# kan-bayashi/espnet

Hardware: AMD Instinct MI355X
Metric: frames/sec, 12L Conformer hybrid CTC/attention training step (B=32 T=1000 d=256 per GPU) (higher is better)
Workload: dtype f32; 1 GPU; BASELINE configs[1]: 12L Conformer enc d=256 h=4 ff=2048 k=31 macaron+cnn rel_pos, 6L Transformer dec, V=5000, fbank B=32 T=1000 L=100, mtlalpha 0.3, lsm 0.1; global_batch=32, frames=1000, parallelism=dp1, optimizer=adam+noam, clip 5.0, launch=hipGraph, wgrad_side_stream=False, optimizer_steps_done=113

## Files before the change

### espnet_amd/csrc/convmod.hip

```cpp
#include <stdlib.h>
#include "common.h"
#include "../../include/espnet_amd.h"

namespace {

constexpr int KMAX = 32;

__device__ __forceinline__ void chan_merge(float& n, float& mean, float& m2, float nb, float mb, float m2b);

template <int NWV, int MODE>
__global__ __launch_bounds__(NWV * 64) void dwconv_lds_kernel(const float* __restrict__ x, const float* __restrict__ w,
                                                              const float* __restrict__ bias, float* __restrict__ y,
                                                              int B, int T, int C, int K, int pad, int flip,
                                                              const float* __restrict__ aglu, int y_bf16,
                                                              float* __restrict__ bn_part) {
  constexpr int TB = NWV * 8;
  constexpr int NR = (TB + KMAX - 1 + NWV - 1) / NWV;
  constexpr int NWL = (64 * KMAX + NWV * 64 - 1) / (NWV * 64);
  __shared__ float xs[(TB + KMAX - 1) * 64];
  __shared__ float wl[64 * KMAX];
  const int lane = threadIdx.x & 63, wave = threadIdx.x >> 6;
  const int c0 = blockIdx.x * 64;
  const int c = min(c0 + lane, C - 1);
  const int nblk = (T + TB - 1) / TB;
// ... 691 lines not shown
  if (gy > total) gy = total;
  if (gy < 1) gy = 1;
  const long tpb = (total + gy - 1) / gy;
  gy = (total + tpb - 1) / tpb;
  hipLaunchKernelGGL(dwconv_bwd_w_kernel, dim3(gx, (unsigned)gy), dim3(WNWV * 64), 0, (hipStream_t)stream, dy, a, dw, db, B,
                     T, C, K, (K - 1) / 2, (int)tpb, 1);
  EAMD_LAUNCH_CHECK();
  return EAMD_OK;
}

static bool bn_shape_ok(int C) { return C >= 4 && C <= 1024 && C % 4 == 0; }
int eamd_bn_nslab(int64_t M, int C) {
  if (!bn_shape_ok(C) || M <= 0) return 0;
  const BnGeom g = bn_geom(C);
  return (int)((M + g.slab_rows - 1) / g.slab_rows);
}

static int bn_stats_impl(const float* x, float* workspace, float* mean, float* rstd, float* running_mean,
                         float* running_var, int64_t* num_batches_tracked, int64_t M, int C, float eps, float momentum, int T,
                         const int32_t* bound, void* stream) {
  if (!x || !workspace || !mean || !rstd || M <= 0 || C <= 0) return EAMD_EINVAL;
  if (bound && (T <= 0 || M % T != 0)) return EAMD_EINVAL;
  if (!bn_shape_ok(C)) return EAMD_EUNSUPPORTED;
  if ((uintptr_t)x & 15) return EAMD_EINVAL;
  hipStream_t s = (hipStream_t)stream;
  const int nslab = eamd_bn_nslab(M, C);
  hipLaunchKernelGGL(bn_partial_kernel, dim3(nslab), dim3(256), 0, s, x, workspace, (long)M, C, T, (const int*)bound);
  EAMD_LAUNCH_CHECK();
  hipLaunchKernelGGL(bn_finalize_kernel, dim3((C + BN_CPB - 1) / BN_CPB), dim3(1024), 0, s, workspace, nslab, C, eps, momentum, mean, rstd,
                     running_mean, running_var, (long long*)num_batches_tracked);
  EAMD_LAUNCH_CHECK();
  return EAMD_OK;
}
int eamd_bn_stats(const float* x, float* workspace, float* mean, float* rstd, float* running_mean,
                  float* running_var, int64_t* num_batches_tracked, int64_t M, int C, float eps, float momentum, void* stream) {
  return bn_stats_impl(x, workspace, mean, rstd, running_mean, running_var, num_batches_tracked, M, C, eps, momentum, 1, nullptr, stream);
}
int eamd_bn_stats_bounded(const float* x, float* workspace, float* mean, float* rstd, float* running_mean,
                          float* running_var, int64_t* num_batches_tracked, int64_t M, int C, float eps, float momentum, int T,
                          const int32_t* bound, void* stream) {
  if (!bound) return EAMD_EINVAL;
  return bn_stats_impl(x, workspace, mean, rstd, running_mean, running_var, num_batches_tracked, M, C, eps, momentum, T, bound, stream);
}

int eamd_bn_finalize(const float* part, int nslab, float* mean, float* rstd, float* running_mean, float* running_var,
                     int64_t* num_batches_tracked, int C, float eps, float momentum, void* stream) {
  if (!part || !mean || !rstd || nslab <= 0 || C <= 0) return EAMD_EINVAL;
  hipLaunchKernelGGL(bn_finalize_kernel, dim3((C + BN_CPB - 1) / BN_CPB), dim3(1024), 0, (hipStream_t)stream, part, nslab, C, eps,
                     momentum, mean, rstd, running_mean, running_var, (long long*)num_batches_tracked);
  EAMD_LAUNCH_CHECK();
  return EAMD_OK;
}

int eamd_bn_apply(const float* x, const float* mean, const float* rstd, const float* gamma, const float* beta,
                  void* y, int64_t M, int C, int act, int y_bf16, void* stream) {
  if (!x || !mean || !rstd || !gamma || !beta || !y || M <= 0 || C <= 0) return EAMD_EINVAL;
  hipLaunchKernelGGL(bn_apply_kernel, dim3(grid_for(M * C)), dim3(256), 0, (hipStream_t)stream, x, mean, rstd, gamma,
                     beta, (float*)y, (long)M, C, act, y_bf16);
  EAMD_LAUNCH_CHECK();
  return EAMD_OK;
}

static int bn_bwd_impl(const float* dy, const float* x, const float* mean, const float* rstd, const float* gamma,
                       const float* beta, float* workspace, float* dx, float* dgamma, float* dbeta, int64_t M, int C,
                       int act, int training, int T, const int32_t* bound, void* stream) {
  if (!dy || !x || !mean || !rstd || !gamma || !beta || !workspace || !dx || !dgamma || !dbeta || M <= 0 || C <= 0)
    return EAMD_EINVAL;
  if (bound && (T <= 0 || M % T != 0)) return EAMD_EINVAL;
  if (!bn_shape_ok(C)) return EAMD_EUNSUPPORTED;
  if (((uintptr_t)x | (uintptr_t)dy | (uintptr_t)mean | (uintptr_t)rstd | (uintptr_t)gamma | (uintptr_t)beta) & 15)
    return EAMD_EINVAL;
  hipStream_t s = (hipStream_t)stream;
  const int nslab = eamd_bn_nslab(M, C);
  float* sums = workspace + (long)nslab * 2 * C;
  hipLaunchKernelGGL(bn_bwd_partial_kernel, dim3(nslab), dim3(256), 0, s, dy, x, mean, rstd, gamma, beta,
                     workspace, (long)M, C, act, T, (const int*)bound);
  EAMD_LAUNCH_CHECK();
  hipLaunchKernelGGL(bn_bwd_finalize_kernel, dim3((C + BN_CPB - 1) / BN_CPB), dim3(1024), 0, s, workspace, nslab, C, sums, dgamma, dbeta);
  EAMD_LAUNCH_CHECK();
  hipLaunchKernelGGL(bn_bwd_apply_kernel, dim3(grid_for(M * C)), dim3(256), 0, s, dy, x, mean, rstd, gamma, beta,
                     sums, dx, (long)M, C, act, training, T, (const int*)bound);
  EAMD_LAUNCH_CHECK();
  return EAMD_OK;
}
int eamd_bn_bwd(const float* dy, const float* x, const float* mean, const float* rstd, const float* gamma,
                const float* beta, float* workspace, float* dx, float* dgamma, float* dbeta, int64_t M, int C,
                int act, int training, void* stream) {
  return bn_bwd_impl(dy, x, mean, rstd, gamma, beta, workspace, dx, dgamma, dbeta, M, C, act, training, 1, nullptr, stream);
}
int eamd_bn_bwd_bounded(const float* dy, const float* x, const float* mean, const float* rstd, const float* gamma,
                        const float* beta, float* workspace, float* dx, float* dgamma, float* dbeta, int64_t M, int C,
                        int act, int training, int T, const int32_t* bound, void* stream) {
  if (!bound) return EAMD_EINVAL;
  return bn_bwd_impl(dy, x, mean, rstd, gamma, beta, workspace, dx, dgamma, dbeta, M, C, act, training, T, bound, stream);
}

static int conv_c1_fwd(const float* x, const float* w, const float* bias, void* y, int B, int T, int F, int C,
                       int y_bf16, int st, int pad, void* stream) {
  if (!x || !w || !bias || !y || B <= 0 || T + 2 * pad < 3 || F + 2 * pad < 3 || C <= 0) return EAMD_EINVAL;
  if (F + 2 * pad > C1_MAXF) return EAMD_EUNSUPPORTED;
  int H = (T + 2 * pad - 3) / st + 1, W = (F + 2 * pad - 3) / st + 1;
  hipStream_t s = (hipStream_t)stream;
  const bool pair = y_bf16 && (C % 2 == 0) && (((uintptr_t)y & 3) == 0);
  const int nthr = pair ? ((C / 2 + 63) / 64) * 64 : 256;
#define EAMD_C1F(ST_, NC_) hipLaunchKernelGGL((conv1_fwd_kernel<ST_, NC_>), dim3(B * H), dim3(min(nthr, 256)), 0, s, x, w, \
                                              bias, (float*)y, B, T, F, H, W, C, y_bf16, pad)
  if (st == 2) { if (pair) EAMD_C1F(2, 2); else EAMD_C1F(2, 1); }
  else         { if (pair) EAMD_C1F(1, 2); else EAMD_C1F(1, 1); }
#undef EAMD_C1F
  EAMD_LAUNCH_CHECK();
  return EAMD_OK;
}
int eamd_conv1_fwd(const float* x, const float* w, const float* bias, void* y, int B, int T, int F, int C,
                   int y_bf16, void* stream) {
  return conv_c1_fwd(x, w, bias, y, B, T, F, C, y_bf16, 2, 0, stream);
}
int eamd_conv3x3_c1_fwd(const float* x, const float* w, const float* bias, void* y, int B, int T, int F, int C,
                        int y_bf16, void* stream) {
  return conv_c1_fwd(x, w, bias, y, B, T, F, C, y_bf16, 1, 1, stream);
}

static void conv_c1_bwd_w_grid(int B, int H, int C, int* gx, int* gy, long* rpb) {
  long nrow = (long)B * H;
  *gx = (C + 255) / 256;
  constexpr int C1W_BLOCKS = 2048;
  long want = C1W_BLOCKS / *gx; if (want < 1) want = 1;
  *rpb = (nrow + want - 1) / want; if (*rpb < 1) *rpb = 1;
  *gy = (int)((nrow + *rpb - 1) / *rpb);
}
static int conv_c1_bwd_w(const void* dy, const float* x, float* dw, float* db, float* workspace, int B, int T, int F,
                         int C, int dy_bf16, int st, int pad, void* stream) {
  if (!dy || !x || !dw || !db || B <= 0 || T + 2 * pad < 3 || F + 2 * pad < 3 || C <= 0) return EAMD_EINVAL;
  if (F + 2 * pad > C1_MAXF) return EAMD_EUNSUPPORTED;
  int H = (T + 2 * pad - 3) / st + 1, W = (F + 2 * pad - 3) / st + 1;
  int gx, gy; long rpb;
  conv_c1_bwd_w_grid(B, H, C, &gx, &gy, &rpb);
  if (!workspace) return EAMD_EINVAL;
  float* part = workspace;
  hipStream_t s = (hipStream_t)stream;
  const bool pair = dy_bf16 && (C % 2 == 0) && (((uintptr_t)dy & 3) == 0);
  const int nthr = pair ? min(256, ((C / 2 + 63) / 64) * 64) : 256;
  if (pair) gx = (C / 2 + nthr - 1) / nthr;
#define EAMD_C1W(ST_, NC_) hipLaunchKernelGGL((conv1_bwd_w_kernel<ST_, NC_>), dim3(gx, gy), dim3(nthr), 0, s, \
                                              (const float*)dy, x, dw, db, part, B, T, F, H, W, C, (int)rpb, dy_bf16, pad)
  if (st == 2) { if (pair) EAMD_C1W(2, 2); else EAMD_C1W(2, 1); }
  else         { if (pair) EAMD_C1W(1, 2); else EAMD_C1W(1, 1); }
#undef EAMD_C1W
  EAMD_LAUNCH_CHECK();
  hipLaunchKernelGGL(conv1_bwd_w_reduce_kernel, dim3((10 * C + 63) / 64, min(16, (gy + 31) / 32)), dim3(256), 0, s, part,
                     gy, C, dw, db);
  EAMD_LAUNCH_CHECK();
  return EAMD_OK;
}
static int64_t conv_c1_ws(int B, int T, int C, int st, int pad) {
  if (B <= 0 || T + 2 * pad < 3 || C <= 0) return 0;
  int H = (T + 2 * pad - 3) / st + 1;
  int gx, gy; long rpb;
  conv_c1_bwd_w_grid(B, H, C, &gx, &gy, &rpb);
  return (int64_t)gy * 10 * C;
}
int64_t eamd_conv1_bwd_w_workspace(int B, int T, int C) { return conv_c1_ws(B, T, C, 2, 0); }
int64_t eamd_conv3x3_c1_bwd_w_workspace(int B, int T, int C) { return conv_c1_ws(B, T, C, 1, 1); }
int eamd_conv1_bwd_w(const void* dy, const float* x, float* dw, float* db, float* workspace, int B, int T, int F,
                     int C, int dy_bf16, void* stream) {
  return conv_c1_bwd_w(dy, x, dw, db, workspace, B, T, F, C, dy_bf16, 2, 0, stream);
}
int eamd_conv3x3_c1_bwd_w(const void* dy, const float* x, float* dw, float* db, float* workspace, int B, int T, int F,
                          int C, int dy_bf16, void* stream) {
  return conv_c1_bwd_w(dy, x, dw, db, workspace, B, T, F, C, dy_bf16, 1, 1, stream);
}

}
```

### espnet_amd/csrc/ctc.hip

```cpp
#include <stdlib.h>
#include <type_traits>
#include "common.h"
#include "../../include/espnet_amd.h"

namespace {

__device__ __forceinline__ float lse2(float a, float b) {
  float m = fmaxf(a, b);
  if (m == -INFINITY) return -INFINITY;
  return m + logf(expf(a - m) + expf(b - m));
}
__device__ __forceinline__ float lse3(float a, float b, float c) {
  float m = fmaxf(fmaxf(a, b), c);
  if (m == -INFINITY) return -INFINITY;
  return m + __logf(__expf(a - m) + __expf(b - m) + __expf(c - m));
}

__global__ __launch_bounds__(64) void ctc_prep_kernel(const long long* __restrict__ ys, int Lmax, int ignore_id,
                                                      int* __restrict__ lab, int* __restrict__ lablen, int B) {
  const int b = blockIdx.x, lane = threadIdx.x;
  int n = 0;
  for (int i0 = 0; i0 < Lmax; i0 += 64) {
    const int i = i0 + lane;
    const long long y = i < Lmax ? ys[(long)b * Lmax + i] : (long long)ignore_id;
// ... 33 lines not shown
      const float4 v = x4[q];
      const float m4 = fmaxf(fmaxf(v.x, v.y), fmaxf(v.z, v.w));
      if (m4 > mx) { se *= expf(mx - m4); mx = m4; }
      se += (expf(v.x - mx) + expf(v.y - mx)) + (expf(v.z - mx) + expf(v.w - mx));
    }
  } else {
    for (int v = threadIdx.x; v < V; v += blockDim.x) {
      const float xv = xr[v];
      if (xv > mx) { se *= expf(mx - xv); mx = xv; }
      se += expf(xv - mx);
    }
  }
  const float mt = mx;
  mx = block_max(mx, red);
  se = block_sum(mt == -INFINITY ? 0.f : se * expf(mt - mx), red);
  const float lse = mx + logf(se);
  if (threadIdx.x == 0) lse_out[(long)ib * T + t] = lse;
  for (int j = 0; j < (kPit ? nsp : 1); ++j) {
    const int r = kPit ? b * nsp + j : b;
    const long lat = kPit ? (long)ib * nsp + j : b;
    const int S = 2 * lablen[r] + 1;
    float* lpr = lp + (lat * T + t) * Smax;
    for (int s = threadIdx.x; s < S; s += blockDim.x) {
      int l = (s & 1) ? lab[(long)r * Lmax + (s >> 1)] : blank;
      if constexpr (kGuardLabels) {
        if (l < 0 || l >= V) { lpr[s] = -INFINITY; continue; }
      }
      lpr[s] = xr[l] - lse;
    }
  }
}

enum { kCtcLoss = 0, kPitAlpha = 1, kPitBeta = 2 };
template <int kMode = kCtcLoss>
__global__ __launch_bounds__(1024) void ctc_alpha_beta_kernel(const float* __restrict__ lp,
                                                              const int* __restrict__ ilen,
                                                              const int* __restrict__ lab,
                                                              const int* __restrict__ lablen, int Lmax,
                                                              float* __restrict__ alpha, float* __restrict__ beta,
                                                              float* __restrict__ nll, int T, int Smax, int blank,
                                                              int nb = 1, int nsp = 1, const long long* __restrict__ perm = nullptr) {
  extern __shared__ float sh[];
  constexpr int PF = 8;
  int b = blockIdx.x, r = b;
  long lat = b, orow = b, nslot = b;
  if constexpr (kMode == kPitAlpha) {
    const int k = blockIdx.x, j = k % nsp, i = k / (nsp * nb);
    b = (k / nsp) % nb; r = b * nsp + j; lat = k; orow = k; nslot = ((long)b * nsp + i) * nsp + j;
  } else if constexpr (kMode == kPitBeta) {
    const int q = blockIdx.x, i = q / nb;
    b = q % nb;
    const int j = (int)perm[(long)b * nsp + i];
    r = b * nsp + j; lat = (long)q * nsp + j; orow = q;
  }
  const int dir = kMode == kCtcLoss ? (int)blockIdx.y : (kMode == kPitAlpha ? 0 : 1);
  const int s = threadIdx.x;
  const int Tb = ilen[b];
  const int L = lablen[r];
  const int S = 2 * L + 1;
  const int W = Smax + 4;
  float* buf0 = sh;
  float* buf1 = sh + W;
  for (int i = threadIdx.x; i < 2 * W; i += blockDim.x) sh[i] = -INFINITY;
  __syncthreads();
  if (Tb <= 0) {
    if (dir == 0 && s == 0) nll[nslot] = (L == 0) ? 0.f : INFINITY;
    return;
  }
  const bool active = s < S;
  const int my = active ? ((s & 1) ? lab[(long)r * Lmax + (s >> 1)] : blank) : blank;
  bool skip = false;
  if (active && (s & 1)) {
    if (dir == 0) skip = (s >= 2) && (lab[(long)r * Lmax + ((s - 2) >> 1)] != my);
    else          skip = (s + 2 < S) && (lab[(long)r * Lmax + ((s + 2) >> 1)] != my);
  }
  const float* lpb = lp + lat * T * Smax;
  float* out = (dir == 0 ? alpha : beta) + orow * T * Smax;

  if (dir == 0) {
    float cur = -INFINITY;
    if (active && s < 2) cur = lpb[s];
    if (active) { buf0[s + 2] = cur; out[s] = cur; }
    __syncthreads();
    float* prev = buf0; float* next = buf1;
    float er[PF];
#pragma unroll
    for (int i = 0; i < PF; ++i) er[i] = (active && 1 + i < Tb) ? lpb[(long)(1 + i) * Smax + s] : 0.f;
    for (int t0 = 1; t0 < Tb; t0 += PF) {
      float en[PF];
#pragma unroll
      for (int i = 0; i < PF; ++i) en[i] = (active && t0 + PF + i < Tb) ? lpb[(long)(t0 + PF + i) * Smax + s] : 0.f;
#pragma unroll
      for (int i = 0; i < PF; ++i) {
        const int t = t0 + i;
        if (t < Tb) {
          if (active) {
            float a = lse3(prev[s + 2], prev[s + 1], skip ? prev[s] : -INFINITY) + er[i];
            next[s + 2] = a;
            out[(long)t * Smax + s] = a;
          }
          __syncthreads();
          float* tmp = prev; prev = next; next = tmp;
        }
      }
#pragma unroll
      for (int i = 0; i < PF; ++i) er[i] = en[i];
    }
    if (s == 0) {
      float a1 = prev[S - 1 + 2];
      float a2 = S >= 2 ? prev[S - 2 + 2] : -INFINITY;
      nll[nslot] = -lse2(a1, a2);
    }
  } else {
    float cur = -INFINITY;
    if (active && s >= S - 2) cur = lpb[(long)(Tb - 1) * Smax + s];
    if (active) { buf0[s + 2] = cur; out[(long)(Tb - 1) * Smax + s] = cur; }
    __syncthreads();
    float* prev = buf0; float* next = buf1;
    float er[PF];
#pragma unroll
    for (int i = 0; i < PF; ++i) er[i] = (active && Tb - 2 - i >= 0) ? lpb[(long)(Tb - 2 - i) * Smax + s] : 0.f;
    for (int t0 = Tb - 2; t0 >= 0; t0 -= PF) {
      float en[PF];
#pragma unroll
      for (int i = 0; i < PF; ++i) en[i] = (active && t0 - PF - i >= 0) ? lpb[(long)(t0 - PF - i) * Smax + s] : 0.f;
#pragma unroll
      for (int i = 0; i < PF; ++i) {
        const int t = t0 - i;
        if (t >= 0) {
          if (active) {
            float a = lse3(prev[s + 2], prev[s + 3], skip ? prev[s + 4] : -INFINITY) + er[i];
            next[s + 2] = a;
            out[(long)t * Smax + s] = a;
          }
          __syncthreads();
          float* tmp = prev; prev = next; next = tmp;
        }
      }
#pragma unroll
      for (int i = 0; i < PF; ++i) er[i] = en[i];
    }
  }
}

template <bool kPit = false>
__global__ __launch_bounds__(256) void ctc_grad_kernel(const float* __restrict__ x, long st, long sb,
                                                       const int* __restrict__ ilen, const int* __restrict__ lab,
                                                       const int* __restrict__ lablen, int Lmax,
                                                       const float* __restrict__ lse, const float* __restrict__ lp,
                                                       const float* __restrict__ alpha,
                                                       const float* __restrict__ beta, const float* __restrict__ nll,
                                                       float* __restrict__ grad, long gst, long gsb, int T, int V,
                                                       int Smax, int blank, float scale, long si = 0, long gsi = 0,
                                                       int nsp = 1, const long long* __restrict__ perm = nullptr) {
  extern __shared__ float occ[];
  const int t = blockIdx.x, b = blockIdx.y;
  const int i = kPit ? (int)blockIdx.z : 0;
  float* gr = grad + t * gst + b * gsb + (kPit ? i * gsi : 0);
  if (t >= ilen[b]) {
    for (int v = threadIdx.x; v < V; v += blockDim.x) gr[v] = 0.f;
    return;
  }
  for (int v = threadIdx.x; v < V; v += blockDim.x) occ[v] = 0.f;
  __syncthreads();
  const long q = kPit ? (long)i * gridDim.y + b : b;
  const int j = kPit ? (int)perm[(long)b * nsp + i] : 0;
  const int r = kPit ? b * nsp + j : b;
  const long lat = kPit ? q * nsp + j : b;
  const int S = 2 * lablen[r] + 1;
  const long base = (lat * T + t) * Smax;
  const long bbase = (q * T + t) * Smax;
  const float nl = nll[kPit ? ((long)b * nsp + i) * nsp + j : b];
  for (int s = threadIdx.x; s < S; s += blockDim.x) {
    int l = (s & 1) ? lab[(long)r * Lmax + (s >> 1)] : blank;
    float g = expf(alpha[base + s] + beta[bbase + s] - lp[base + s] + nl);
    atomicAdd(&occ[l], g);
  }
  __syncthreads();
  const float* xr = x + t * st + b * sb + (kPit ? i * si : 0);
  const float ls = lse[q * T + t];
  for (int v = threadIdx.x; v < V; v += blockDim.x) gr[v] = (expf(xr[v] - ls) - occ[v]) * scale;
}

}

extern "C" {

int64_t eamd_ctc_workspace_bytes(int B, int T, int Lmax) {
  int64_t Smax = 2 * (int64_t)Lmax + 1;
  int64_t n = (int64_t)B * Lmax * 4 + (int64_t)B * 4
              + (int64_t)B * T * 4
              + 3 * (int64_t)B * T * Smax * 4;
  return n + 256;
}

int eamd_ctc_loss(const float* acts, int64_t stride_t, int64_t stride_b, const int64_t* ys_pad,
                  const int32_t* ilens, float* nll, float* grad, int64_t gstride_t, int64_t gstride_b,
                  void* workspace, int B, int T, int V, int Lmax, int blank, int ignore_id, float grad_scale,
                  void* stream) {
  if (!acts || !ys_pad || !ilens || !nll || !workspace || B <= 0 || T <= 0 || V <= 0 || Lmax < 0) return EAMD_EINVAL;
  const int Smax = 2 * Lmax + 1;
  int threads = ((Smax + 63) / 64) * 64;
  if (threads > 1024) return EAMD_EUNSUPPORTED;
  if (grad && (size_t)V * 4 > 64 * 1024) return EAMD_EUNSUPPORTED;
  hipStream_t s = (hipStream_t)stream;
  char* w = (char*)workspace;
  int Lm = Lmax > 0 ? Lmax : 1;
  int* lab = (int*)w; w += (size_t)B * Lm * 4;
  int* lablen = (int*)w; w += (size_t)B * 4;
  w = (char*)(((uintptr_t)w + 15) & ~(uintptr_t)15);
  float* lse = (float*)w; w += (size_t)B * T * 4;
  float* lp = (float*)w; w += (size_t)B * T * Smax * 4;
  float* alpha = (float*)w; w += (size_t)B * T * Smax * 4;
  float* beta = (float*)w;

  hipLaunchKernelGGL(ctc_prep_kernel, dim3(B), dim3(64), 0, s, (const long long*)ys_pad, Lmax, ignore_id, lab, lablen, B);
  EAMD_LAUNCH_CHECK();
  hipLaunchKernelGGL((ctc_lse_gather_kernel<false, false>), dim3(T, B), dim3(256), 0, s, acts, (long)stride_t, (long)stride_b, ilens,
                     lab, lablen, Lm, lse, lp, T, V, Smax, blank, 0L, 1);
  EAMD_LAUNCH_CHECK();
  hipLaunchKernelGGL(ctc_alpha_beta_kernel<kCtcLoss>, dim3(B, 2), dim3(threads), 2 * (Smax + 4) * sizeof(float), s, lp, ilens,
                     lab, lablen, Lm, alpha, beta, nll, T, Smax, blank, 1, 1, nullptr);
  EAMD_LAUNCH_CHECK();
  if (grad) {
    hipLaunchKernelGGL(ctc_grad_kernel<false>, dim3(T, B), dim3(256), (size_t)V * sizeof(float), s, acts, (long)stride_t,
                       (long)stride_b, ilens, lab, lablen, Lm, lse, lp, alpha, beta, nll, grad, (long)gstride_t,
                       (long)gstride_b, T, V, Smax, blank, grad_scale, 0L, 0L, 1, nullptr);
    EAMD_LAUNCH_CHECK();
  }
  return EAMD_OK;
}

}

namespace {
__constant__ int kPitPerm2[2][2] = {{0, 1}, {1, 0}};
__constant__ int kPitPerm3[6][3] = {{0, 1, 2}, {0, 2, 1}, {1, 0, 2}, {1, 2, 0}, {2, 1, 0}, {2, 0, 1}};

template <int NS>
__global__ __launch_bounds__(64) void ctc_pit_select_kernel(const float* __restrict__ nll, long long* __restrict__ perm,
                                                            float* __restrict__ pit, int B) {
  const int b = blockIdx.x * 64 + threadIdx.x;
  if (b >= B) return;
  constexpr int NP = NS == 2 ? 2 : 6;
  const float* n = nll + (long)b * NS * NS;
  const float fb = (float)B;
  float best = 0.f;
  int arg = -1;
  for (int k = 0; k < NP; ++k) {
    float sc = 0.f;
#pragma unroll
    for (int i = 0; i < NS; ++i) {
      const int j = NS == 2 ? kPitPerm2[k][i] : kPitPerm3[k][i];
      const float v = n[i * NS + j] / fb;
      sc = i == 0 ? v : sc + v;
    }
    sc = sc / (float)NS;
    if (arg < 0 || sc < best || (sc != sc && best == best)) { best = sc; arg = k; }
  }
#pragma unroll
  for (int i = 0; i < NS; ++i) perm[(long)b * NS + i] = NS == 2 ? kPitPerm2[arg][i] : kPitPerm3[arg][i];
  pit[b] = best;
}
}

extern "C" {

int64_t eamd_ctc_pit_workspace_bytes(int S, int B, int T, int Lmax) {
  const int64_t Lm = Lmax > 0 ? Lmax : 1;
  const int64_t Smax = 2 * (int64_t)Lmax + 1;
  const int64_t R = (int64_t)B * S;
  return R * Lm * 4 + R * 4 + 16
         + R * T * 4
         + 2 * R * S * T * Smax * 4
         + R * T * Smax * 4
         + 256;
}

int eamd_ctc_pit_loss(const float* acts, const int64_t* ys_pad, const int32_t* ilens, float* nll_pair, int64_t* perm, float* pit,
                      float* grad, void* workspace, int S, int B, int T, int V, int Lmax, int blank, int ignore_id, float grad_scale,
                      void* stream) {
  if (!acts || !ys_pad || !ilens || !nll_pair || !perm || !pit || !workspace || B <= 0 || T <= 0 || V <= 0 || Lmax < 0)
    return EAMD_EINVAL;
  if (S != 2 && S != 3) return EAMD_EUNSUPPORTED;
  const int Smax = 2 * Lmax + 1;
  const int threads = ((Smax + 63) / 64) * 64;
  if (threads > 1024) return EAMD_EUNSUPPORTED;
  if (grad && (size_t)V * 4 > 64 * 1024) return EAMD_EUNSUPPORTED;
  hipStream_t s = (hipStream_t)stream;
  const int Lm = Lmax > 0 ? Lmax : 1;
  const size_t R = (size_t)B * S;
  char* w = (char*)workspace;
  int* lab = (int*)w; w += R * Lm * 4;
  int* lablen = (int*)w; w += R * 4;
  w = (char*)(((uintptr_t)w + 15) & ~(uintptr_t)15);
  float* lse = (float*)w; w += R * T * 4;
  float* lp = (float*)w; w += R * S * T * Smax * 4;
  float* alpha = (float*)w; w += R * S * T * Smax * 4;
  float* beta = (float*)w;
  const long sb = (long)T * V, si = (long)B * T * V;

  hipLaunchKernelGGL(ctc_prep_kernel, dim3(R), dim3(64), 0, s, (const long long*)ys_pad, Lmax, ignore_id, lab, lablen, (int)R);
  EAMD_LAUNCH_CHECK();
  hipLaunchKernelGGL((ctc_lse_gather_kernel<false, false, true>), dim3(T, B, S), dim3(256), 0, s, acts, (long)V, sb, ilens, lab,
                     lablen, Lm, lse, lp, T, V, Smax, blank, si, S);
  EAMD_LAUNCH_CHECK();
  hipLaunchKernelGGL(ctc_alpha_beta_kernel<kPitAlpha>, dim3(R * S), dim3(threads), 2 * (Smax + 4) * sizeof(float), s, lp, ilens,
                     lab, lablen, Lm, alpha, beta, nll_pair, T, Smax, blank, B, S, nullptr);
  EAMD_LAUNCH_CHECK();
  if (S == 2)
    hipLaunchKernelGGL(ctc_pit_select_kernel<2>, dim3((B + 63) / 64), dim3(64), 0, s, nll_pair, (long long*)perm, pit, B);
  else
    hipLaunchKernelGGL(ctc_pit_select_kernel<3>, dim3((B + 63) / 64), dim3(64), 0, s, nll_pair, (long long*)perm, pit, B);
  EAMD_LAUNCH_CHECK();
  if (grad) {
    hipLaunchKernelGGL(ctc_alpha_beta_kernel<kPitBeta>, dim3(R), dim3(threads), 2 * (Smax + 4) * sizeof(float), s, lp, ilens,
                       lab, lablen, Lm, alpha, beta, nll_pair, T, Smax, blank, B, S, (const long long*)perm);
    EAMD_LAUNCH_CHECK();
    hipLaunchKernelGGL(ctc_grad_kernel<true>, dim3(T, B, S), dim3(256), (size_t)V * sizeof(float), s, acts, (long)V, sb, ilens,
                       lab, lablen, Lm, lse, lp, alpha, beta, nll_pair, grad, (long)V, sb, T, V, Smax, blank, grad_scale, si, si,
                       S, (const long long*)perm);
    EAMD_LAUNCH_CHECK();
  }
  return EAMD_OK;
}

}

namespace {
constexpr int kAlignMaxThreads = 1024;

__global__ __launch_bounds__(kAlignMaxThreads) void ctc_viterbi_kernel(const float* __restrict__ lp, const int* __restrict__ ilen,
                                                                        const int* __restrict__ lab, const int* __restrict__ lablen,
                                                                        int Lmax, int Lout, unsigned char* __restrict__ bp,
                                                                        float* __restrict__ score, int* __restrict__ endst,
                                                                        int* __restrict__ states, long long* __restrict__ tokens,
                                                                        int* __restrict__ seg_start, int* __restrict__ seg_end, int T,
                                                                        int Spad, int blank) {
  __shared__ float2 xch[2][kAlignMaxThreads + 1];
  __shared__ float endv[2];
  constexpr int PF = 8;
  const int b = blockIdx.x, tid = threadIdx.x, nt = blockDim.x;
  const int Tb = min(ilen[b], T);
  const int L = lablen[b];
  const int S = 2 * L + 1;
  const int s0 = 4 * tid;
  int* st_b = states + (long)b * T;
  long long* tk_b = tokens + (long)b * T;
  int* ss_b = seg_start + (long)b * Lout;
  int* se_b = seg_end + (long)b * Lout;
  const int* lab_b = lab + (long)b * Lmax;
  for (int t = max(Tb, 0) + tid; t < T; t += nt) { st_b[t] = -1; tk_b[t] = -1; }
  for (int i = L + tid; i < Lout; i += nt) { ss_b[i] = -1; se_b[i] = -1; }
  if (Tb <= 0) {
    if (tid == 0) score[b] = L == 0 ? 0.f : -INFINITY;
    for (int i = tid; i < min(L, Lout); i += nt) { ss_b[i] = -1; se_b[i] = -1; }
    return;
  }
  const bool active = s0 < S;
  unsigned skip = 0;
  if (active) {
#pragma unroll
    for (int k = 0; k < 4; ++k) {
      const int s = s0 + k;
      if ((s & 1) && s >= 3 && s < S) {
        const int y = lab_b[s >> 1];
        if (y != blank && y != lab_b[(s - 2) >> 1]) skip |= 1u << k;
      }
    }
  }
  const float* lpb = lp + (long)b * T * Spad;
  unsigned* bpw = reinterpret_cast<unsigned*>(bp + (long)b * T * Spad);
  const long rw = Spad / 4;
  float d[4];
#pragma unroll
  for (int k = 0; k < 4; ++k) d[k] = (s0 + k < 2 && s0 + k < S) ? lpb[s0 + k] : -INFINITY;
  if (tid == 0) { xch[0][0] = make_float2(-INFINITY, -INFINITY); xch[1][0] = make_float2(-INFINITY, -INFINITY); }
  xch[0][tid + 1] = make_float2(d[2], d[3]);
  __syncthreads();
  int p = 0;
  const float4* lp4 = reinterpret_cast<const float4*>(lpb) + tid;
  float4 er[PF];
// ... 429 lines not shown
```

### espnet_amd/csrc/gemm.hip

```cpp
#include <stdlib.h>
#include "common.h"
#include "../../include/espnet_amd.h"

namespace {

constexpr int BK = 32;
constexpr int NTHREADS = 256;

template <int BM, int BN, int PREC>
struct Smem {
  static constexpr int LDK = PREC ? 40 : 36;
  using elem_t = typename std::conditional<PREC == 1, unsigned short, float>::type;
  elem_t a[2][BM][LDK];
  elem_t b[2][BN][LDK];
  int poff[3][BK];
};

struct RowState {
  int base;
  int ih, jw;
  int ok;
};

__device__ __forceinline__ RowState decompose(const eamd_gather_t& g, int row, int nrows) {
// ... 176 lines not shown
#pragma unroll
      for (int i = 0; i < NIB; ++i) {
        const int n = n0 + b_row[i];
        rb[i] = load_kcontig(B + (long)n * p.ldb, n < p.N, k0 + b_kq[i], p.K, b_vec);
      }
    } else {
#pragma unroll
      for (int i = 0; i < NIB; ++i) {
        const int n = n0 + b_row[i];
        rb[i] = load_kstrided(B + n, p.ldb, n < p.N, k0 + b_kq[i], p.K);
      }
    }
  };

  auto store_tile = [&](int buf) {
#pragma unroll
    for (int i = 0; i < NIA; ++i)
      lds_store4<PREC>(&sm.a[buf][a_row[i]][a_kq[i]], apply_act4(ra[i], p.a_act));
#pragma unroll
    for (int i = 0; i < NIB; ++i)
      lds_store4<PREC>(&sm.b[buf][b_row[i]][b_kq[i]], apply_act4(rb[i], p.b_act));
  };

  f32x4 acc[MT][NT];
#pragma unroll
  for (int i = 0; i < MT; ++i)
#pragma unroll
    for (int j = 0; j < NT; ++j) acc[i][j] = (f32x4){0.f, 0.f, 0.f, 0.f};

  const bool tgat = gat && p.transA;
  if (nkt > 0) {
    if (tgat) {
      fill_poff(kt_begin, kt_begin % 3);
      if (nkt > 1) fill_poff(kt_begin + 1, (kt_begin + 1) % 3);
      __syncthreads();
    }
    load_tile(kt_begin);
    store_tile(0);
    __syncthreads();
  }

  const int fr = lane & 15, fq = lane >> 4;
  for (int it = 0; it < nkt; ++it) {
    const int buf = it & 1;
    const bool more = it + 1 < nkt;
    if (more) {
      if (tgat && it + 2 < nkt) fill_poff(kt_begin + it + 2, (kt_begin + it + 2) % 3);
      load_tile(kt_begin + it + 1);
    }

    if constexpr (PREC == 1) {
      bf16x8 af[MT], bfr[NT];
#pragma unroll
      for (int i = 0; i < MT; ++i)
        af[i] = *reinterpret_cast<const bf16x8*>(&sm.a[buf][wm * WM + i * 16 + fr][fq * 8]);
#pragma unroll
      for (int j = 0; j < NT; ++j)
        bfr[j] = *reinterpret_cast<const bf16x8*>(&sm.b[buf][wn * WN + j * 16 + fr][fq * 8]);
#pragma unroll
      for (int i = 0; i < MT; ++i)
#pragma unroll
        for (int j = 0; j < NT; ++j)
          acc[i][j] = __builtin_amdgcn_mfma_f32_16x16x32_bf16(af[i], bfr[j], acc[i][j], 0, 0, 0);
    } else {
#pragma unroll
      for (int kk = 0; kk < 2; ++kk) {
        f32x4 af[MT], bfr[NT];
#pragma unroll
        for (int i = 0; i < MT; ++i)
          af[i] = *reinterpret_cast<const f32x4*>(&sm.a[buf][wm * WM + i * 16 + fr][kk * 16 + fq * 4]);
#pragma unroll
        for (int j = 0; j < NT; ++j)
          bfr[j] = *reinterpret_cast<const f32x4*>(&sm.b[buf][wn * WN + j * 16 + fr][kk * 16 + fq * 4]);
#pragma unroll
        for (int e = 0; e < 4; ++e)
#pragma unroll
          for (int i = 0; i < MT; ++i)
#pragma unroll
            for (int j = 0; j < NT; ++j)
              acc[i][j] = __builtin_amdgcn_mfma_f32_16x16x4f32(af[i][e], bfr[j][e], acc[i][j], 0, 0, 0);
      }
    }

    if (more) store_tile(buf ^ 1);
    __syncthreads();
  }

  if (do_colsum) {
    const int m = m0 + a_row[0];
    if (m < p.M) atomicAdd(p.colsum + (long)zb * p.M + m, cs_acc * p.alpha);
  }

  const bool lead = split == 0;
#pragma unroll
  for (int i = 0; i < MT; ++i) {
#pragma unroll
    for (int r = 0; r < 4; ++r) {
      const int m = m0 + wm * WM + i * 16 + fq * 4 + r;
      if (m >= p.M) continue;
      long prow = m;
      if (p.cmap.enabled) {
        const eamd_rowmap_t& c = p.cmap;
        int jj = m % c.Wo; int tt = m / c.Wo; int ii = tt % c.Ho; int bb = tt / c.Ho;
        prow = ((long)bb * c.Hc + ii * c.sh + c.oh) * c.Wc + jj * c.sw + c.ow;
      }
#pragma unroll
      for (int j = 0; j < NT; ++j) {
        const int n = n0 + wn * WN + j * 16 + fr;
        if (n >= p.N) continue;
        float v = acc[i][j][r];
        if (p.splitk > 1) {
          if (lead && p.bias) v += p.bias[n];
          v *= p.alpha;
          if (lead && p.R) v += p.R[coff + prow * p.ldr + n];
          atomicAdd(p.C + coff + prow * p.ldc + n, v);
        } else {
          if (p.bias) v += p.bias[n];
          if (p.epilogue == 1) v = v > 0.f ? v : 0.f;
          else if (p.epilogue == 2) v = eamd_swish(v);
          else if (p.epilogue == 3) v = p.aux[coff + prow * p.ldaux + n] > 0.f ? v : 0.f;
          else if (p.epilogue == 4) v *= eamd_dswish(p.aux[coff + prow * p.ldaux + n]);
          else if (p.epilogue == 5) v *= p.aux[coff + prow * p.ldaux + n];
          v *= p.alpha;
          if (p.R) v += p.R[coff + prow * p.ldr + n];
          float* cp = p.C + coff + prow * p.ldc + n;
          if (p.beta != 0.f) v += p.beta * (*cp);
          *cp = v;
        }
      }
    }
  }
}

template <int BM, int BN, int PREC>
int launch(const eamd_gemm_t& p, hipStream_t stream) {
  dim3 grid((p.M + BM - 1) / BM, (p.N + BN - 1) / BN, p.batch1 * p.batch2 * p.splitk);
  size_t smem = sizeof(Smem<BM, BN, PREC>);
  if (smem > 64 * 1024) {
    static const hipError_t attr_err = hipFuncSetAttribute(
        reinterpret_cast<const void*>(&gemm_kernel<BM, BN, PREC>), hipFuncAttributeMaxDynamicSharedMemorySize,
        (int)sizeof(Smem<BM, BN, PREC>));
    if (attr_err != hipSuccess) return (int)attr_err;
  }
  hipLaunchKernelGGL((gemm_kernel<BM, BN, PREC>), grid, dim3(NTHREADS), smem, stream, p);
  EAMD_LAUNCH_CHECK();
  return EAMD_OK;
}

}

int eamd_gemm_bf16_dispatch(const eamd_gemm_t& p, int tile, hipStream_t stream);
int eamd_gemm_f32_dispatch(const eamd_gemm_t& p, int tile, hipStream_t stream);

static int gemm_check(eamd_gemm_t& p, int& tile_out) {
  const bool stats = p.epilogue == 7;
  const bool rowgrad = p.epilogue == 8;
  if (!p.A || !p.B || (!p.C && !p.Cb && !stats)) return EAMD_EINVAL;
  if (stats && (!p.stats.part || !p.stats.zfix || (p.stats.col && !p.stats.zcol))) return EAMD_EINVAL;
  if (rowgrad && !p.stats.rowc) return EAMD_EINVAL;
  if ((stats || rowgrad) && (p.stats.fix < 0 || p.stats.fix >= p.N || (p.tile != 64 && p.tile != 128) || p.splitk > 1 ||
                             p.batch1 * p.batch2 != 1 || p.cmap.enabled || p.gather.enabled || p.Hb || p.drop_p != 0.f ||
                             p.R || p.colsum || p.beta != 0.f))
    return EAMD_EINVAL;
  if (p.in_dtype != 0 && p.in_dtype != 1) return EAMD_EINVAL;
  if (p.in_dtype == 1 && p.precision != 1) return EAMD_EINVAL;
  if (p.in_dtype == 0 && (p.Cb || p.aux_dtype || (!p.C && !stats))) return EAMD_EUNSUPPORTED;
  if (p.M <= 0 || p.N <= 0 || p.K < 0) return EAMD_EINVAL;
  if (p.batch1 <= 0 || p.batch2 <= 0) return EAMD_EINVAL;
  if (p.splitk < 1) p.splitk = 1;
  if (p.splitk > 1 && p.epilogue != 0) return EAMD_EINVAL;
  if (p.epilogue < 0 || p.epilogue > 8) return EAMD_EINVAL;
  if (p.epilogue >= 3 && p.epilogue <= 5 && !p.aux) return EAMD_EINVAL;
  if (p.epilogue == 6 && (!p.Hb || p.drop_p <= 0.f)) return EAMD_EINVAL;
  if (p.precision != 0 && p.precision != 1) return EAMD_EINVAL;
  if ((long)p.batch1 * p.batch2 * p.splitk > 65535) return EAMD_EUNSUPPORTED;

  int tile = p.tile;
  if (tile == 0) {
    long t128 = (long)((p.M + 127) / 128) * ((p.N + 127) / 128) * p.batch1 * p.batch2 * p.splitk;
    if (p.in_dtype == 1) {
      constexpr int T128_KMIN = 320, T128_NMIN = 256;
      tile = (t128 >= 1024 && p.K >= T128_KMIN && p.M >= 2048 && p.N >= T128_NMIN) ? 128 : 64;
    } else {
      tile = (t128 >= (p.precision == 0 ? 240 : 512) && p.M >= 128 && p.N >= 128) ? 128 : 64;
      if (p.precision == 0 && tile == 128 && t128 > 256 && t128 < 400 && p.splitk == 1) tile = 64;
    }
  }
  if (tile != 64 && tile != 128) return EAMD_EINVAL;

  if (p.gather.enabled) {
    const eamd_gather_t& g = p.gather;
    if (g.ntap < 1 || g.ntap > 9 || g.C <= 0 || g.C % BK != 0) return EAMD_EINVAL;
    if (!p.transA) {
      if (p.K != g.ntap * g.C) return EAMD_EINVAL;
    } else {
      if (p.M != g.ntap * g.C) return EAMD_EINVAL;
      if (g.C % tile != 0) return EAMD_EINVAL;
    }
  }
  if ((p.N + tile - 1) / tile > 65535) return EAMD_EUNSUPPORTED;
  if (p.h_dtype != 0 && p.h_dtype != 1) return EAMD_EINVAL;
  if (p.in_dtype == 1 && p.h_dtype != 0) return EAMD_EUNSUPPORTED;
  if (p.in_dtype != 1 && ((p.Hb && !(p.h_dtype == 1 && p.precision == 0)) || (p.drop_p != 0.f && p.precision != 0)))
    return EAMD_EUNSUPPORTED;
  if ((p.a_act > EAMD_ACT_SWISH || p.b_act > EAMD_ACT_SWISH) && (p.in_dtype != 0 || p.precision != 0)) return EAMD_EUNSUPPORTED;
  tile_out = tile;
  return EAMD_OK;
}

extern "C" int eamd_gemm(const eamd_gemm_t* pp, void* stream_) {
  if (!pp) return EAMD_EINVAL;
  eamd_gemm_t p = *pp;
  hipStream_t stream = (hipStream_t)stream_;
  int tile = 0;
  const int chk = gemm_check(p, tile);
  if (chk != EAMD_OK) return chk;
  const bool stats = p.epilogue == 7, rowgrad = p.epilogue == 8;
  if (p.in_dtype == 1) return eamd_gemm_bf16_dispatch(p, tile, stream);

  if (p.precision == 1 && p.gather.enabled && p.transA && !p.Hb && p.drop_p == 0.f) {
    const int rc = eamd_gemm_f32_dispatch(p, tile, stream);
    if (rc != EAMD_EUNSUPPORTED) return rc;
  }
  if (p.precision == 0) {
    const int rc = eamd_gemm_f32_dispatch(p, tile, stream);
    if (rc != EAMD_EUNSUPPORTED) return rc;
    if (p.drop_p != 0.f || p.Hb || p.a_act > EAMD_ACT_SWISH || p.b_act > EAMD_ACT_SWISH) return EAMD_EUNSUPPORTED;
  }
  if (stats || rowgrad) return EAMD_EUNSUPPORTED;
  if (tile == 128) {
    return p.precision ? launch<128, 128, 1>(p, stream) : launch<128, 128, 0>(p, stream);
  }
  return p.precision ? launch<64, 64, 1>(p, stream) : launch<64, 64, 0>(p, stream);
}

int eamd_gemm_f32_multi(const eamd_gemm_t* ps, const int* tiles, int n, hipStream_t stream);

extern "C" int eamd_gemm_multi(const eamd_gemm_t* descs, int n, void* stream) {
  if (!descs || n < 1) return EAMD_EINVAL;
  if (n >= 2 && n <= EAMD_GEMM_MULTI_MAX) {
    eamd_gemm_t ps[EAMD_GEMM_MULTI_MAX];
    int tiles[EAMD_GEMM_MULTI_MAX];
    bool f32 = true;
    for (int i = 0; i < n; ++i) {
      ps[i] = descs[i];
      const int chk = gemm_check(ps[i], tiles[i]);
      if (chk != EAMD_OK) return chk;
      f32 = f32 && ps[i].in_dtype == 0 && ps[i].precision == 0;
    }
    if (f32) {
      const int rc = eamd_gemm_f32_multi(ps, tiles, n, (hipStream_t)stream);
      if (rc != EAMD_EUNSUPPORTED) return rc;
    }
  }
  for (int i = 0; i < n; ++i) {
    const int rc = eamd_gemm(&descs[i], stream);
    if (rc != EAMD_OK) return rc;
  }
  return EAMD_OK;
}

int eamd_gemm_f32_group_count(const eamd_gemm_t& p);
int eamd_gemm_f32_group_launch(const eamd_gemm_t* tab, const int* first, int n, int total, int tile, hipStream_t s);
int eamd_gemm_bf16_group_count(const eamd_gemm_t& p);
int eamd_gemm_bf16_group_launch(const eamd_gemm_t* tab, const int* first, int n, int total, int tile, hipStream_t s);

extern "C" int eamd_gemm_group_plan(const eamd_gemm_t* descs, int n, int32_t* first) {
  if (!descs || !first || n <= 0) return EAMD_EINVAL;
  long total = 0;
  for (int i = 0; i < n; ++i) {
    const eamd_gemm_t& p = descs[i];
    if (!p.A || !p.B || !p.C || p.M <= 0 || p.N <= 0 || p.K <= 0) return EAMD_EINVAL;
    if (p.in_dtype != descs[0].in_dtype || p.precision != descs[0].precision) return EAMD_EINVAL;
    if ((p.tile == 128) != (descs[0].tile == 128)) return EAMD_EINVAL;
    const int c = p.in_dtype == 1 ? eamd_gemm_bf16_group_count(p) : eamd_gemm_f32_group_count(p);
    if (c < 0) return c;
    first[i] = (int32_t)total;
    total += c;
    if (total >= (1L << 30)) return EAMD_EUNSUPPORTED;
  }
  first[n] = (int32_t)total;
  return (int)total;
}

extern "C" int eamd_gemm_group_launch(const eamd_gemm_t* descs_dev, const int32_t* first_dev, int n, int total, int in_dtype,
                                      int tile, void* stream) {
  if (!descs_dev || !first_dev || n <= 0 || total <= 0 || (tile != 64 && tile != 128)) return EAMD_EINVAL;
  return in_dtype == 1 ? eamd_gemm_bf16_group_launch(descs_dev, first_dev, n, total, tile, (hipStream_t)stream)
                       : eamd_gemm_f32_group_launch(descs_dev, first_dev, n, total, tile, (hipStream_t)stream);
}

extern "C" int eamd_abi_version(void) { return 1; }
```

### espnet_amd/csrc/gemm_f32.hip

```cpp
#include <stdlib.h>
#include <type_traits>
#include "common.h"
#include "../../include/espnet_amd.h"

#include "gemm_bf16_common.h"

namespace {

constexpr int FBK = 32;

template <int BM, int BN, bool TA, bool TB>
struct SmemF {
  static constexpr int KPAD_A = BM >= 128 ? 8 : 4, KPAD_B = BN >= 128 ? 8 : 4;
  static constexpr int LDA = TA ? BM + KPAD_A : FBK + 4;
  static constexpr int RA = TA ? FBK : BM;
  static constexpr int LDB = TB ? BN + KPAD_B : FBK + 4;
  static constexpr int RB = TB ? FBK : BN;
  static constexpr int OPS = 2 * (RA * LDA + RB * LDB);
  static constexpr int CT = BM * (BN + 4);
  float ab[OPS > CT ? OPS : CT];
  int poff[8][FBK];
  __device__ float* a(int buf) { return ab + buf * RA * LDA; }
  __device__ float* b(int buf) { return ab + 2 * RA * LDA + buf * RB * LDB; }
};

template <int ACT>
__device__ __forceinline__ float4 act4(float4 v, int act) {
  if constexpr (ACT == 2) return make_float4(eamd_act(v.x, act), eamd_act(v.y, act), eamd_act(v.z, act), eamd_act(v.w, act));
  if (act == EAMD_ACT_SWISH) return make_float4(eamd_swish(v.x), eamd_swish(v.y), eamd_swish(v.z), eamd_swish(v.w));
  return make_float4(fmaxf(v.x, 0.f), fmaxf(v.y, 0.f), fmaxf(v.z, 0.f), fmaxf(v.w, 0.f));
}
__device__ __forceinline__ float4 mask4(float4 v, int nv) {
  return make_float4(nv > 0 ? v.x : 0.f, nv > 1 ? v.y : 0.f, nv > 2 ? v.z : 0.f, nv > 3 ? v.w : 0.f);
}

template <int BM, int BN, bool TA, bool TB, bool GAT, int ACT, bool ROWEPI = false, bool NOPAD = false>
__device__ __forceinline__ void gemm_f32_body(const eamd_gemm_t& p, const int bid, const int nblk, const int zb) {
  constexpr int WM = BM / 2, WN = BN / 2;
  constexpr int MT = WM / 16, NTL = WN / 16;
  constexpr int NCA = BM / 32, NCB = BN / 32;
  constexpr int CPR_A = BM / 4, RPP_A = NT_ / CPR_A;
  constexpr int CPR_B = BN / 4, RPP_B = NT_ / CPR_B;
  using S = SmemF<BM, BN, TA, TB>;
  extern __shared__ __attribute__((aligned(16))) char smem_raw[];
  S& sm = *reinterpret_cast<S*>(smem_raw);

  const int t = threadIdx.x;
  const int lane = t & 63, wave = t >> 6;
  const int wm = wave >> 1, wn = wave & 1;
  const int tiles_n = (p.N + BN - 1) / BN;
  int tile_id, split;
  if (nblk < 0) {
    const int ntile = ((p.M + BM - 1) / BM) * tiles_n;
    const int per = (-nblk) >> 3;
    const int v = (bid & 7) * per + (bid >> 3);
    if (v >= ntile * p.splitk) return;
    split = v / ntile;
    tile_id = v - split * ntile;
  } else if (p.splitk > 1) {
    split = bid % p.splitk;
    tile_id = bid / p.splitk;
  } else {
    split = 0;
    const int ntile = nblk;
    const int id = bid, q = ntile >> 3, r = ntile & 7, xcd = id & 7, j = id >> 3;
    tile_id = (xcd < r ? xcd * (q + 1) : r * (q + 1) + (xcd - r) * q) + j;
  }
  const int tile_m = tile_id / tiles_n, tile_n = tile_id % tiles_n;
  const int m0 = tile_m * BM, n0 = tile_n * BN;
  const int b1 = zb / p.batch2, b2 = zb % p.batch2;
  const float* __restrict__ A = p.A + b1 * p.sA1 + b2 * p.sA2;
  const float* __restrict__ B = p.B + b1 * p.sB1 + b2 * p.sB2;
  const long coff = b1 * p.sC1 + b2 * p.sC2;

  const int nkt_total = (p.K + FBK - 1) / FBK;
  const int per = (nkt_total + p.splitk - 1) / p.splitk;
  const int kt_begin = split * per;
  const int kt_end = min(nkt_total, kt_begin + per);
  const int nkt = kt_end - kt_begin;

  int a_r[NCA], a_c[NCA], b_r[NCB], b_c[NCB];
#pragma unroll
  for (int i = 0; i < NCA; ++i) {
    if constexpr (TA) { a_r[i] = t / CPR_A + RPP_A * i; a_c[i] = t % CPR_A; }
    else              { a_r[i] = t / 8 + 32 * i;        a_c[i] = t % 8; }
  }
#pragma unroll
  for (int i = 0; i < NCB; ++i) {
    if constexpr (TB) { b_r[i] = t / CPR_B + RPP_B * i; b_c[i] = t % CPR_B; }
    else              { b_r[i] = t / 8 + 32 * i;        b_c[i] = t % 8; }
  }
  long a_off[NCA], b_off[NCB];
  if constexpr (!GAT) {
#pragma unroll
    for (int i = 0; i < NCA; ++i) {
      if constexpr (!TA) a_off[i] = (long)min(m0 + a_r[i], p.M - 1) * p.lda + a_c[i] * 4;
      else a_off[i] = (long)a_r[i] * p.lda + min(m0 + a_c[i] * 4, (p.M - 1) & ~3);
    }
  }
#pragma unroll
  for (int i = 0; i < NCB; ++i) {
    if constexpr (!TB) b_off[i] = (long)min(n0 + b_r[i], p.N - 1) * p.ldb + b_c[i] * 4;
    else b_off[i] = (long)b_r[i] * p.ldb + min(n0 + b_c[i] * 4, (p.N - 1) & ~3);
  }
  RowStateB a_rs[NCA];
  unsigned long long dh_pack = 0ull, dw_pack = 0ull;
  int gC = 1, gHin = 0, gWin = 0;
  if constexpr (GAT) {
#pragma unroll
    for (int tp = 0; tp < 9; ++tp) {
      dh_pack |= (unsigned long long)((unsigned)(p.gather.dh[tp] + 8) & 15u) << (4 * tp);
      dw_pack |= (unsigned long long)((unsigned)(p.gather.dw[tp] + 8) & 15u) << (4 * tp);
    }
    gC = p.gather.C; gHin = p.gather.Hin; gWin = p.gather.Win;
  }
  const int pK = p.K;
  const long ldaL = p.lda, ldbL = p.ldb;
  auto tap_dh = [&](int tap) __attribute__((always_inline)) { return (int)((dh_pack >> (4 * tap)) & 15ull) - 8; };
  auto tap_dw = [&](int tap) __attribute__((always_inline)) { return (int)((dw_pack >> (4 * tap)) & 15ull) - 8; };
  auto goff = [&](const RowStateB& rs, int dh, int dw) __attribute__((always_inline)) -> long {
    const int hh = rs.ih + dh, ww = rs.jw + dw;
    const bool ok = rs.ok && hh >= 0 && hh < gHin && ww >= 0 && ww < gWin;
    return ok ? ((long)(rs.base + hh * gWin + ww)) * gC : -1L;
  };
  constexpr bool g_nopad = NOPAD;
  if constexpr (GAT && !TA) {
#pragma unroll
    for (int i = 0; i < NCA; ++i) a_rs[i] = decompose_b(p.gather, m0 + a_r[i], p.M);
  }
  int pr_row = 0, pr_j = 0, pr_i = 0, pr_b = 0;
  if constexpr (GAT && TA) {
    if (t < FBK) {
      pr_row = kt_begin * FBK + t;
      pr_j = pr_row % p.gather.Wo;
      const int tt = pr_row / p.gather.Wo;
      pr_i = tt % p.gather.Ho;
      pr_b = tt / p.gather.Ho;
    }
  }
  constexpr int DEPTH = BM >= 128 ? 2 : 3;
  constexpr int UNROLL = DEPTH % 2 ? 2 * DEPTH : DEPTH;
  float4 ra[DEPTH][NCA], rb[DEPTH][NCB];
  const bool do_colsum = TA && p.colsum != nullptr && !GAT && tile_n == 0;
  float cs[4] = {0.f, 0.f, 0.f, 0.f};

  const int gWo = GAT ? p.gather.Wo : 1, gHo = GAT ? p.gather.Ho : 1, gsh = GAT ? p.gather.sh : 0, gsw = GAT ? p.gather.sw : 0;
  const int ta_tap = (GAT && TA) ? m0 / gC : 0;
  const int ta_dh = tap_dh(ta_tap), ta_dw = tap_dw(ta_tap);
  auto fill_poff = [&](int kt, int slot) __attribute__((always_inline)) {
    if (t < FBK) {
      RowStateB s;
      s.ok = pr_row < pK;
      s.base = pr_b * gHin * gWin; s.ih = pr_i * gsh; s.jw = pr_j * gsw;
      sm.poff[slot][t] = (int)goff(s, ta_dh, ta_dw);
      pr_row += FBK; pr_j += FBK;
      while (pr_j >= gWo) { pr_j -= gWo; ++pr_i; }
      while (pr_i >= gHo) { pr_i -= gHo; ++pr_b; }
    }
  };

  auto load_tile = [&](auto set_c, auto guard_c, int kt) __attribute__((always_inline)) {
    constexpr int SET = decltype(set_c)::value;
    constexpr bool GUARD = decltype(guard_c)::value;
    const int k0 = kt * FBK;
    if constexpr (!TA) {
      if constexpr (!GAT) {
#pragma unroll
        for (int i = 0; i < NCA; ++i) {
          const int kk = (GUARD && k0 + a_c[i] * 4 >= pK) ? -a_c[i] * 4 : k0;
          ra[SET][i] = *reinterpret_cast<const float4*>(A + a_off[i] + kk);
        }
      } else {
        const int tap = k0 / gC, c0 = k0 - tap * gC;
        const int dh = tap_dh(tap), dw = tap_dw(tap);
        const int tappix = dh * gWin + dw;
#pragma unroll
        for (int i = 0; i < NCA; ++i) {
          long off;
          if (g_nopad) off = a_rs[i].ok ? (long)(a_rs[i].base + a_rs[i].ih * gWin + a_rs[i].jw + tappix) * gC : -1L;
          else off = goff(a_rs[i], dh, dw);
          ra[SET][i] = *reinterpret_cast<const float4*>(A + (off >= 0 ? off + c0 + a_c[i] * 4 : 0L));
        }
      }
    } else {
      if constexpr (!GAT) {
#pragma unroll
        for (int i = 0; i < NCA; ++i) {
          const int kk = (GUARD && k0 + a_r[i] >= pK) ? -a_r[i] : k0;
          ra[SET][i] = *reinterpret_cast<const float4*>(A + a_off[i] + (long)kk * ldaL);
        }
      } else {
        const int c = (m0 % gC) + a_c[0] * 4;
        const int slot = kt % 8;
#pragma unroll
        for (int i = 0; i < NCA; ++i) {
          const int off = sm.poff[slot][a_r[i]];
          ra[SET][i] = *reinterpret_cast<const float4*>(A + (off >= 0 ? (long)off + c : 0L));
        }
      }
    }
    if constexpr (!TB) {
#pragma unroll
      for (int i = 0; i < NCB; ++i) {
        const int kk = (GUARD && k0 + b_c[i] * 4 >= pK) ? -b_c[i] * 4 : k0;
        rb[SET][i] = *reinterpret_cast<const float4*>(B + b_off[i] + kk);
      }
    } else {
#pragma unroll
      for (int i = 0; i < NCB; ++i) {
        const int kk = (GUARD && k0 + b_r[i] >= pK) ? -b_r[i] : k0;
        rb[SET][i] = *reinterpret_cast<const float4*>(B + b_off[i] + (long)kk * ldbL);
      }
    }
  };

  auto store_tile = [&](auto set_c, auto guard_c, int buf, int kt) __attribute__((always_inline)) {
    constexpr int SET = decltype(set_c)::value;
    constexpr bool GUARD = decltype(guard_c)::value;
    const int k0 = kt * FBK;
    if constexpr (GAT) {
      int sdh = 0, sdw = 0;
      if constexpr (!TA && !g_nopad) { const int tap = k0 / gC; sdh = tap_dh(tap); sdw = tap_dw(tap); }
#pragma unroll
      for (int i = 0; i < NCA; ++i) {
        bool ok;
        if constexpr (!TA) ok = g_nopad ? a_rs[i].ok != 0 : goff(a_rs[i], sdh, sdw) >= 0;
        else ok = sm.poff[kt % 8][a_r[i]] >= 0;
        ra[SET][i] = mask4(ra[SET][i], ok ? 4 : 0);
      }
    }
    if constexpr (GUARD) {
      if (k0 + FBK > pK) {
        if constexpr (!GAT) {
#pragma unroll
          for (int i = 0; i < NCA; ++i)
            ra[SET][i] = mask4(ra[SET][i], TA ? ((k0 + a_r[i]) < pK ? 4 : 0) : pK - (k0 + a_c[i] * 4));
        }
#pragma unroll
        for (int i = 0; i < NCB; ++i)
          rb[SET][i] = mask4(rb[SET][i], TB ? ((k0 + b_r[i]) < pK ? 4 : 0) : pK - (k0 + b_c[i] * 4));
      }
    }
    float* la = sm.a(buf);
    float* lb = sm.b(buf);
    if constexpr (ACT) {
#pragma unroll
      for (int i = 0; i < NCA; ++i) {
        float4 v = ra[SET][i];
        if (p.a_act != EAMD_ACT_NONE) v = act4<ACT>(v, p.a_act);
        if (do_colsum) { cs[0] += v.x; cs[1] += v.y; cs[2] += v.z; cs[3] += v.w; }
        *reinterpret_cast<float4*>(&la[a_r[i] * S::LDA + a_c[i] * 4]) = v;
        __builtin_amdgcn_sched_barrier(0);
      }
#pragma unroll
      for (int i = 0; i < NCB; ++i) {
        float4 v = rb[SET][i];
        if (p.b_act != EAMD_ACT_NONE) v = act4<ACT>(v, p.b_act);
        *reinterpret_cast<float4*>(&lb[b_r[i] * S::LDB + b_c[i] * 4]) = v;
        __builtin_amdgcn_sched_barrier(0);
      }
    } else {
      if (do_colsum) {
#pragma unroll
        for (int i = 0; i < NCA; ++i) {
          cs[0] += ra[SET][i].x; cs[1] += ra[SET][i].y; cs[2] += ra[SET][i].z; cs[3] += ra[SET][i].w;
        }
      }
#pragma unroll
      for (int i = 0; i < NCA; ++i) *reinterpret_cast<float4*>(&la[a_r[i] * S::LDA + a_c[i] * 4]) = ra[SET][i];
#pragma unroll
      for (int i = 0; i < NCB; ++i) *reinterpret_cast<float4*>(&lb[b_r[i] * S::LDB + b_c[i] * 4]) = rb[SET][i];
    }
  };

  f32x4 acc[MT][NTL];
#pragma unroll
  for (int i = 0; i < MT; ++i)
#pragma unroll
    for (int j = 0; j < NTL; ++j) acc[i][j] = (f32x4){0.f, 0.f, 0.f, 0.f};

  constexpr bool tgat = GAT && TA;
  if (nkt > 0) {
    if (tgat) {
      for (int q = 0; q < DEPTH && q < nkt; ++q) fill_poff(kt_begin + q, (kt_begin + q) % 8);
      __syncthreads();
    }
    load_tile(std::integral_constant<int, 0>{}, std::true_type{}, kt_begin);
    if constexpr (DEPTH == 3) {
      if (nkt > 1) load_tile(std::integral_constant<int, 1>{}, std::true_type{}, kt_begin + 1);
    }
    store_tile(std::integral_constant<int, 0>{}, std::true_type{}, 0, kt_begin);
    __syncthreads();
  }

  const int fr = lane & 15, fq = lane >> 4;
  constexpr int QD = BM >= 128 ? 8 : 16;
  constexpr int NS = FBK / QD, EQ = QD / 4;
  auto read_frags = [&](int buf, int q, float (&af)[MT][EQ], float (&bfr)[NTL][EQ]) __attribute__((always_inline)) {
    const float* la = sm.a(buf);
    const float* lb = sm.b(buf);
#pragma unroll
    for (int i = 0; i < MT; ++i) {
      if constexpr (!TA) {
        const float* src = &la[(wm * WM + i * 16 + fr) * S::LDA + q * QD + fq * EQ];
        if constexpr (EQ == 4) {
          const float4 v = *reinterpret_cast<const float4*>(src);
          af[i][0] = v.x; af[i][1] = v.y; af[i][2] = v.z; af[i][3] = v.w;
        } else {
          const float2 v = *reinterpret_cast<const float2*>(src);
          af[i][0] = v.x; af[i][1] = v.y;
        }
      } else {
#pragma unroll
        for (int e = 0; e < EQ; ++e) af[i][e] = la[(q * QD + fq * EQ + e) * S::LDA + wm * WM + i * 16 + fr];
      }
    }
#pragma unroll
    for (int j = 0; j < NTL; ++j) {
      if constexpr (!TB) {
        const float* src = &lb[(wn * WN + j * 16 + fr) * S::LDB + q * QD + fq * EQ];
        if constexpr (EQ == 4) {
          const float4 v = *reinterpret_cast<const float4*>(src);
          bfr[j][0] = v.x; bfr[j][1] = v.y; bfr[j][2] = v.z; bfr[j][3] = v.w;
        } else {
          const float2 v = *reinterpret_cast<const float2*>(src);
          bfr[j][0] = v.x; bfr[j][1] = v.y;
        }
      } else {
#pragma unroll
        for (int e = 0; e < EQ; ++e) bfr[j][e] = lb[(q * QD + fq * EQ + e) * S::LDB + wn * WN + j * 16 + fr];
      }
    }
  };
  auto mfma_set = [&](const float (&af)[MT][EQ], const float (&bfr)[NTL][EQ]) __attribute__((always_inline)) {
#pragma unroll
    for (int e = 0; e < EQ; ++e)
#pragma unroll
      for (int i = 0; i < MT; ++i)
#pragma unroll
        for (int j = 0; j < NTL; ++j)
          acc[i][j] = __builtin_amdgcn_mfma_f32_16x16x4f32(af[i][e], bfr[j][e], acc[i][j], 0, 0, 0);
  };
  float fa[2][MT][EQ], fb[2][NTL][EQ];
  if (nkt > 0) read_frags(0, 0, fa[0], fb[0]);
  auto phase = [&](auto idx_c, auto guard_c, int it) __attribute__((always_inline)) {
    constexpr int IDX = decltype(idx_c)::value;
    constexpr int PAR = IDX % DEPTH;
    constexpr bool GUARD = decltype(guard_c)::value;
    using load_t = std::integral_constant<int, (PAR + DEPTH - 1) % DEPTH>;
    using other_t = std::integral_constant<int, (PAR + 1) % DEPTH>;
    constexpr int buf = IDX & 1;
    if constexpr (GUARD) {
      if (tgat && it + DEPTH < nkt) fill_poff(kt_begin + it + DEPTH, (kt_begin + it + DEPTH) % 8);
      if (it + DEPTH - 1 < nkt) load_tile(load_t{}, guard_c, kt_begin + it + DEPTH - 1);
    } else {
      if constexpr (tgat) fill_poff(kt_begin + it + DEPTH, (kt_begin + it + DEPTH) % 8);
      load_tile(load_t{}, guard_c, kt_begin + it + DEPTH - 1);
    }
#pragma unroll
    for (int q = 0; q < NS; ++q) {
      if (q + 1 < NS) {
        read_frags(buf, q + 1, fa[(q + 1) & 1], fb[(q + 1) & 1]);
      } else {
        __builtin_amdgcn_sched_barrier(0);
        __syncthreads();
        if constexpr (GUARD) {
          if (it + 1 < nkt) read_frags(buf ^ 1, 0, fa[0], fb[0]);
        } else {
          read_frags(buf ^ 1, 0, fa[0], fb[0]);
        }
#pragma unroll
        for (int e = 0; e < EQ; ++e) {
#pragma unroll
          for (int i = 0; i < MT; ++i) asm volatile("" : "+v"(fa[q & 1][i][e]));
#pragma unroll
          for (int j = 0; j < NTL; ++j) asm volatile("" : "+v"(fb[q & 1][j][e]));
        }
      }
      __builtin_amdgcn_sched_barrier(0);
      if (q == NS - 2) {
        if constexpr (GUARD) {
          if (it + 1 < nkt) store_tile(other_t{}, guard_c, buf ^ 1, kt_begin + it + 1);
        } else {
          store_tile(other_t{}, guard_c, buf ^ 1, kt_begin + it + 1);
        }
        __builtin_amdgcn_sched_barrier(0);
      }
      mfma_set(fa[q & 1], fb[q & 1]);
    }
  };
  using T_ = std::true_type;
  using F_ = std::false_type;
  int it = 0;
  for (; it + UNROLL + DEPTH - 1 < nkt; it += UNROLL) {
    phase(std::integral_constant<int, 0>{}, F_{}, it);
    phase(std::integral_constant<int, 1>{}, F_{}, it + 1);
    if constexpr (UNROLL == 6) {
      phase(std::integral_constant<int, 2>{}, F_{}, it + 2);
      phase(std::integral_constant<int, 3>{}, F_{}, it + 3);
      phase(std::integral_constant<int, 4>{}, F_{}, it + 4);
      phase(std::integral_constant<int, 5>{}, F_{}, it + 5);
    }
  }
  for (; it < nkt; it += UNROLL) {
    phase(std::integral_constant<int, 0>{}, T_{}, it);
    if (it + 1 < nkt) phase(std::integral_constant<int, 1>{}, T_{}, it + 1);
    if constexpr (UNROLL == 6) {
      if (it + 2 < nkt) phase(std::integral_constant<int, 2>{}, T_{}, it + 2);
      if (it + 3 < nkt) phase(std::integral_constant<int, 3>{}, T_{}, it + 3);
      if (it + 4 < nkt) phase(std::integral_constant<int, 4>{}, T_{}, it + 4);
      if (it + 5 < nkt) phase(std::integral_constant<int, 5>{}, T_{}, it + 5);
    }
  }

  __syncthreads();
  if (TA && p.colsum != nullptr && !GAT) {
    float* csl = sm.ab;
    constexpr int NSLOT = NT_ / CPR_A;
    static_assert(NSLOT * BM <= S::OPS, "column-sum slots must fit in the operand buffers");
    __syncthreads();
    if (do_colsum) {
#pragma unroll
      for (int j = 0; j < 4; ++j) csl[(t / CPR_A) * BM + a_c[0] * 4 + j] = cs[j];
    }
    __syncthreads();
    if (do_colsum) {
      for (int i = t; i < BM; i += NT_) {
        const int m = m0 + i;
        float v = 0.f;
#pragma unroll 8
        for (int sl = 0; sl < NSLOT; ++sl) v += csl[sl * BM + i];
        if (m < p.M) atomicAdd(p.colsum + (long)zb * p.M + m, v * p.alpha);
      }
    }
    __syncthreads();
  }

  if (p.splitk > 1) {
    const bool lead = split == 0;
#pragma unroll
    for (int i = 0; i < MT; ++i) {
#pragma unroll
      for (int r = 0; r < 4; ++r) {
        const int m = m0 + wm * WM + i * 16 + fq * 4 + r;
        if (m >= p.M) continue;
        long prow = m;
        if (p.cmap.enabled) {
          const eamd_rowmap_t& c = p.cmap;
          int jj = m % c.Wo; int tt = m / c.Wo; int ii = tt % c.Ho; int bb = tt / c.Ho;
          prow = ((long)bb * c.Hc + ii * c.sh + c.oh) * c.Wc + jj * c.sw + c.ow;
        }
#pragma unroll
        for (int j = 0; j < NTL; ++j) {
          const int n = n0 + wn * WN + j * 16 + fr;
          if (n >= p.N) continue;
          float v = acc[i][j][r];
          if (lead && p.bias) v += p.bias[n];
          v *= p.alpha;
          if (lead && p.R) v += p.R[coff + prow * p.ldr + n];
          atomicAdd(p.C + coff + prow * p.ldc + n, v);
        }
      }
    }
    return;
  }
  store_c_tile<BM, BN, true, ROWEPI>(p, acc, sm.ab, m0, n0, coff);
}

template <int BM, int BN, bool TA, bool TB, bool GAT, int ACT, bool ROWEPI = false, bool NOPAD = false>
__global__ __launch_bounds__(NT_, 2) void gemm_f32_kernel(const eamd_gemm_t p) {
  gemm_f32_body<BM, BN, TA, TB, GAT, ACT, ROWEPI, NOPAD>(p, blockIdx.x, gridDim.x, blockIdx.z);
}

template <int BM, int BN, bool TA, bool TB>
__global__ __launch_bounds__(NT_, 2) void gemm_f32_group_kernel(const eamd_gemm_t* __restrict__ tab,
                                                                const int* __restrict__ first, const int n) {
  int lo = 0, hi = n;
  while (hi - lo > 1) {
    const int mid = (lo + hi) >> 1;
    if (first[mid] <= (int)blockIdx.x) lo = mid; else hi = mid;
  }
  const eamd_gemm_t p = tab[lo];
  gemm_f32_body<BM, BN, TA, TB, false, false>(p, (int)blockIdx.x - first[lo], -(first[lo + 1] - first[lo]), 0);
}

struct MultiF {
  eamd_gemm_t p[EAMD_GEMM_MULTI_MAX];
  int nt[EAMD_GEMM_MULTI_MAX];
  int n;
};

template <int BM, int BN, bool TA, bool TB, bool GAT, bool NOPAD>
__global__ __launch_bounds__(NT_, 2) void gemm_f32_multi_kernel(const MultiF m) {
  const int g = (int)blockIdx.x >> 3;
  const int per = (int)gridDim.x / (8 * m.n);
  const int cls = g / per;
  const int bid = (g - cls * per) * 8 + ((int)blockIdx.x & 7);
  if (bid >= m.nt[cls]) return;
  const eamd_gemm_t p = m.p[cls];
  gemm_f32_body<BM, BN, TA, TB, GAT, false, false, NOPAD>(p, bid, m.nt[cls], 0);
}

template <int BM, int BN, bool TA, bool TB, bool GAT, int ACT, bool NOPAD = false>
int launch_f2(const eamd_gemm_t& p, hipStream_t stream) {
  dim3 grid(((p.M + BM - 1) / BM) * ((p.N + BN - 1) / BN) * p.splitk, 1, p.batch1 * p.batch2);
  constexpr size_t smem = sizeof(SmemF<BM, BN, TA, TB>);
  if (p.epilogue >= 7) {
    if constexpr (!TA && !TB && !GAT && !ACT) {
      if (smem > 64 * 1024) {
        static const hipError_t attr_err_r = hipFuncSetAttribute(
            reinterpret_cast<const void*>(&gemm_f32_kernel<BM, BN, TA, TB, GAT, ACT, true>),
            hipFuncAttributeMaxDynamicSharedMemorySize, (int)smem);
        if (attr_err_r != hipSuccess) return (int)attr_err_r;
      }
      hipLaunchKernelGGL((gemm_f32_kernel<BM, BN, TA, TB, GAT, ACT, true>), grid, dim3(NT_), smem, stream, p);
      EAMD_LAUNCH_CHECK();
      return EAMD_OK;
    } else {
      return EAMD_EUNSUPPORTED;
    }
  }
  if (smem > 64 * 1024) {
    static const hipError_t attr_err = hipFuncSetAttribute(
        reinterpret_cast<const void*>(&gemm_f32_kernel<BM, BN, TA, TB, GAT, ACT, false, NOPAD>),
        hipFuncAttributeMaxDynamicSharedMemorySize, (int)smem);
    if (attr_err != hipSuccess) return (int)attr_err;
  }
  hipLaunchKernelGGL((gemm_f32_kernel<BM, BN, TA, TB, GAT, ACT, false, NOPAD>), grid, dim3(NT_), smem, stream, p);
  EAMD_LAUNCH_CHECK();
  return EAMD_OK;
}

inline bool gather_nopad(const eamd_gather_t& g) {
  for (int tp = 0; tp < g.ntap; ++tp)
    if (g.dh[tp] < 0 || (g.Ho - 1) * g.sh + g.dh[tp] >= g.Hin || g.dw[tp] < 0 || (g.Wo - 1) * g.sw + g.dw[tp] >= g.Win) return false;
  return true;
}

inline bool gather_taps_small(const eamd_gather_t& g) {
  for (int tp = 0; tp < g.ntap; ++tp)
    if (g.dh[tp] < -8 || g.dh[tp] > 7 || g.dw[tp] < -8 || g.dw[tp] > 7) return false;
  return true;
}

template <int BM, int BN, bool TA, bool TB, bool GAT>
int launch_f(const eamd_gemm_t& p, hipStream_t stream) {
  if constexpr (GAT && !TA) {
    if (gather_nopad(p.gather) && p.epilogue < 7) return launch_f2<BM, BN, TA, TB, GAT, 0, true>(p, stream);
  }
  if constexpr (GAT) return launch_f2<BM, BN, TA, TB, GAT, 0>(p, stream);
  else if (p.a_act > EAMD_ACT_SWISH || p.b_act > EAMD_ACT_SWISH) return launch_f2<BM, BN, TA, TB, GAT, 2>(p, stream);
  else if (p.a_act != EAMD_ACT_NONE || p.b_act != EAMD_ACT_NONE) return launch_f2<BM, BN, TA, TB, GAT, 1>(p, stream);
  return launch_f2<BM, BN, TA, TB, GAT, 0>(p, stream);
}

template <int T>
int dispatch_layout_f(const eamd_gemm_t& p, hipStream_t s) {
  if (p.transA) return p.transB ? launch_f<T, T, true, true, false>(p, s) : launch_f<T, T, true, false, false>(p, s);
  return p.transB ? launch_f<T, T, false, true, false>(p, s) : launch_f<T, T, false, false, false>(p, s);
}

bool aligned16f(const void* q) { return (reinterpret_cast<uintptr_t>(q) & 15) == 0; }

}

int eamd_gemm_f32_dispatch(const eamd_gemm_t& p, int tile, hipStream_t stream) {
  if (p.Cb || (p.Hb && !p.h_dtype) || p.aux_dtype || (!p.C && p.epilogue != 7)) return EAMD_EUNSUPPORTED;
  if (p.Hb && p.drop_p <= 0.f) return EAMD_EINVAL;
  if (p.drop_p < 0.f || p.drop_p >= 1.f) return EAMD_EINVAL;
  if (p.drop_p > 0.f && (p.cmap.enabled || p.batch1 * p.batch2 != 1 || p.ldc != p.N || p.splitk > 1)) return EAMD_EINVAL;
  const bool a_ok = aligned16f(p.A) && p.lda % 4 == 0 && p.sA1 % 4 == 0 && p.sA2 % 4 == 0 &&
                    p.lda >= (p.transA ? (p.M + 3) / 4 * 4 : (p.K + 3) / 4 * 4);
  const bool b_ok = aligned16f(p.B) && p.ldb % 4 == 0 && p.sB1 % 4 == 0 && p.sB2 % 4 == 0 &&
                    p.ldb >= (p.transB ? (p.N + 3) / 4 * 4 : (p.K + 3) / 4 * 4);
  if (p.gather.enabled) {
    const eamd_gather_t& g = p.gather;
    if (g.C % FBK != 0 || !p.transB || !aligned16f(p.A) || !b_ok) return EAMD_EUNSUPPORTED;
    if (p.a_act != EAMD_ACT_NONE || p.b_act != EAMD_ACT_NONE) return EAMD_EUNSUPPORTED;
    if (!gather_taps_small(g)) return EAMD_EUNSUPPORTED;
    if (p.transA && g.C % tile != 0) return EAMD_EUNSUPPORTED;
    if (tile == 128)
      return p.transA ? launch_f<128, 128, true, true, true>(p, stream) : launch_f<128, 128, false, true, true>(p, stream);
    return p.transA ? launch_f<64, 64, true, true, true>(p, stream) : launch_f<64, 64, false, true, true>(p, stream);
  }
  if (!a_ok || !b_ok) return EAMD_EUNSUPPORTED;
  return tile == 128 ? dispatch_layout_f<128>(p, stream) : dispatch_layout_f<64>(p, stream);
}

template <bool NOPAD>
static int multi_launch_t(const MultiF& m, int grid, hipStream_t stream) {
  constexpr size_t smem = sizeof(SmemF<128, 128, false, true>);
  static const hipError_t attr_err = hipFuncSetAttribute(
      reinterpret_cast<const void*>(&gemm_f32_multi_kernel<128, 128, false, true, true, NOPAD>),
      hipFuncAttributeMaxDynamicSharedMemorySize, (int)smem);
  if (attr_err != hipSuccess) return (int)attr_err;
  hipLaunchKernelGGL((gemm_f32_multi_kernel<128, 128, false, true, true, NOPAD>), dim3((unsigned)grid), dim3(NT_), smem, stream, m);
  EAMD_LAUNCH_CHECK();
  return EAMD_OK;
}

int eamd_gemm_f32_multi(const eamd_gemm_t* ps, const int* tiles, int n, hipStream_t stream) {
  if (n < 2 || n > EAMD_GEMM_MULTI_MAX) return EAMD_EUNSUPPORTED;
  MultiF m;
  bool nopad = true;
  int maxnt = 0;
  for (int i = 0; i < n; ++i) {
    const eamd_gemm_t& p = ps[i];
    if (tiles[i] != 128 || p.in_dtype != 0 || p.precision != 0) return EAMD_EUNSUPPORTED;
    if (!p.gather.enabled || p.transA || !p.transB || p.splitk != 1 || p.batch1 * p.batch2 != 1) return EAMD_EUNSUPPORTED;
    if (!p.C || p.Cb || p.Hb || p.aux_dtype || p.epilogue > 5 || p.colsum) return EAMD_EUNSUPPORTED;
    if (p.a_act != EAMD_ACT_NONE || p.b_act != EAMD_ACT_NONE || p.drop_p != 0.f) return EAMD_EUNSUPPORTED;
    const bool b_ok = aligned16f(p.B) && p.ldb % 4 == 0 && p.ldb >= (p.N + 3) / 4 * 4;
    if (p.gather.C % FBK != 0 || !aligned16f(p.A) || !b_ok || !gather_taps_small(p.gather)) return EAMD_EUNSUPPORTED;
    const long nt = (long)((p.M + 127) / 128) * ((p.N + 127) / 128);
    if (nt > (1L << 24)) return EAMD_EUNSUPPORTED;
    nopad = nopad && gather_nopad(p.gather);
    m.p[i] = p;
    m.nt[i] = (int)nt;
    maxnt = nt > maxnt ? (int)nt : maxnt;
  }
  for (int i = n; i < EAMD_GEMM_MULTI_MAX; ++i) { m.p[i] = ps[0]; m.nt[i] = 0; }
  m.n = n;
  const int grid = (maxnt + 7) / 8 * 8 * n;
  return nopad ? multi_launch_t<true>(m, grid, stream) : multi_launch_t<false>(m, grid, stream);
}

int eamd_gemm_f32_group_count(const eamd_gemm_t& p) {
  if (p.in_dtype != 0 || p.precision != 0 || !p.transA || !p.transB || !p.C || p.Cb || p.Hb || p.aux || p.R || p.bias)
    return EAMD_EUNSUPPORTED;
  if (p.gather.enabled || p.cmap.enabled || p.epilogue || p.a_act || p.b_act || p.drop_p > 0.f ||
      p.batch1 * p.batch2 != 1 || p.splitk < 1)
    return EAMD_EUNSUPPORTED;
  if (p.splitk == 1 && p.beta != 1.f) return EAMD_EUNSUPPORTED;
  const bool a_ok = aligned16f(p.A) && p.lda % 4 == 0 && p.lda >= (p.M + 3) / 4 * 4;
  const bool b_ok = aligned16f(p.B) && p.ldb % 4 == 0 && p.ldb >= (p.N + 3) / 4 * 4;
  if (!a_ok || !b_ok) return EAMD_EUNSUPPORTED;
  const int T = p.tile == 128 ? 128 : 64;
  const long n = ((long)((p.M + T - 1) / T) * ((p.N + T - 1) / T) * p.splitk + 7) / 8 * 8;
  return n < (1L << 24) ? (int)n : EAMD_EUNSUPPORTED;
}

template <int T>
static int group_launch_t(const eamd_gemm_t* tab_dev, const int* first_dev, int n, int total, hipStream_t stream) {
  constexpr size_t smem = sizeof(SmemF<T, T, true, true>);
  if (smem > 64 * 1024) {
    static const hipError_t attr_err = hipFuncSetAttribute(
        reinterpret_cast<const void*>(&gemm_f32_group_kernel<T, T, true, true>),
        hipFuncAttributeMaxDynamicSharedMemorySize, (int)smem);
    if (attr_err != hipSuccess) return (int)attr_err;
  }
  hipLaunchKernelGGL((gemm_f32_group_kernel<T, T, true, true>), dim3((unsigned)total), dim3(NT_), smem, stream, tab_dev,
                     first_dev, n);
  EAMD_LAUNCH_CHECK();
  return EAMD_OK;
}

int eamd_gemm_f32_group_launch(const eamd_gemm_t* tab_dev, const int* first_dev, int n, int total, int tile, hipStream_t stream) {
  return tile == 128 ? group_launch_t<128>(tab_dev, first_dev, n, total, stream)
                     : group_launch_t<64>(tab_dev, first_dev, n, total, stream);
}
```

### espnet_amd/functional.py

```python
import math

import torch

from . import ops
from .ops import (ACT_NONE, ACT_RELU, ACT_SWISH, EPI_DACT_FACTOR, EPI_MUL_AUX, EPI_MUL_DSWISH, EPI_MUL_RELU_MASK, EPI_NONE,
                  EPI_RELU)


class GradSink:

    on_done = None
    on_use = None

    @staticmethod
    def use(params):
        if GradSink.on_use is not None and torch.is_grad_enabled():
            GradSink.on_use(params)
        return params

    def __init__(self, params):
        self.params = list(params)
        self.ret = [None] * len(self.params)

    def buf(self, i):
# ... 800 lines not shown
            k, v = pre_kv[1].block(pre_kv[2], 0), pre_kv[1].block(pre_kv[2], D)
            dkv_out = pre_kv[1].grad_block(pre_kv[2])
        if P is None:
            P, Pd = again(qu, qv, k, v)
        dqu, dqv, dkk, dv, dp = attn_core_bwd(dctx, P, qu, qv, k, v, p, B, T1, T2, H, dk,
                                              Pd=Pd, attn_drop=(p_att, s_att), dkv_out=dkv_out, dp_out=dp_out,
                                              shift_len=ctx.shift_len)
        if rel:
            wpos = params[10]
            dq = ops.add_cast_colsum2(dqu, dqv, sink.buf(11).view(-1), sink.buf(12).view(-1))
            if dp_out is None:
                ops.linear_bwd_w(ops.to_act(dp), pos2, sink.buf(10))
        else:
            dq = ops.to_act(dqu)
        kv_in = mem2 if cross else xn
        ops.linear_bwd_w(dq, xn, sink.buf(2), db=sink.buf(3))
        dxn = ops.linear_bwd_x(dq, ops.wshadow(wq))
        dmem = None
        if pre_kv is not None:
            dx = _ln_bwd_out(dxn, x2, ln_w, mean, rstd, do, sink.buf(0), sink.buf(1), ctx.prev, (B, T1, D))
            return (dx, None, None, None, None, None, None, None, None, None) + sink.results()
        ops.linear_bwd_w(dkk, kv_in, sink.buf(4), db=sink.buf(5))
        ops.linear_bwd_w(dv, kv_in, sink.buf(6), db=sink.buf(7))
        if cross:
            dmem = ops.linear_bwd_x(dkk, ops.wshadow(wk))
            ops.linear_bwd_x(dv, ops.wshadow(wv), out=dmem, beta=1.0)
            dmem = dmem.view(B, T2, D)
        else:
            ops.linear_bwd_x(dkk, ops.wshadow(wk), out=dxn, beta=1.0)
            ops.linear_bwd_x(dv, ops.wshadow(wv), out=dxn, beta=1.0)
        dx = _ln_bwd_out(dxn, x2, ln_w, mean, rstd, do, sink.buf(0), sink.buf(1), ctx.prev, (B, T1, D))
        return (dx, dmem, None, None, None, None, None, None, None, None) + sink.results()


FUSE_GLU_DWCONV = True


class ConvModuleBlockFn(torch.autograd.Function):
    @staticmethod
    def forward(ctx, x, running_mean, running_var, training, act, eps, bn_eps, bn_momentum, drop, *params):
        p_out, s_out = drop
        ln_w, ln_b, w1, b1, wd, bd_, g, be, w2, b2 = params
        B, T, D = x.shape
        Cc = w2.shape[0]
        K = wd.shape[-1]
        M = B * T
        adt = ops.act_dtype()
        x2 = x.reshape(M, D).contiguous()
        rp = None
        if eps is not None and D == 256 and Cc == 256 and x2.dtype == torch.float32 and adt == torch.float32 \
                and ops.rowproj_ok(M, D, 2 * Cc) and (p_out <= 0.0 or ops.f32_epilogue_drop()):
            w1v, w2v = w1.detach().view(2 * Cc, D), w2.detach().view(Cc, Cc)
            rp = ops.rowproj_images(w1, [(w1v, False), (w1v, True), (w2v, False), (w2v, True)])
        if rp is not None:
            xn = torch.empty_like(x2)
            mean = torch.empty(M, device=x2.device, dtype=torch.float32)
            rstd = torch.empty_like(mean)
            a = ops.rowproj(xn, rp[0], 2 * Cc, bias=b1, ln=(x2, ln_w, ln_b, eps, mean, rstd))
        else:
            xn, mean, rstd = _ln_fwd_in(x2, ln_w, ln_b, eps, adt)
            a = ops.linear_fwd(xn, ops.wshadow(w1).view(2 * Cc, D), b1)
        assert eps is not None or p_out <= 0.0
        tb = ops.time_bound()
        bound = (T, tb) if tb is not None else None
        if bound is not None:
            ops.mask_time(a, T, tb)
        gl = d = bmean = None
        nbt = getattr(running_mean, "_eamd_nbt", None)
        if FUSE_GLU_DWCONV:
            d = ops.dwconv_glu_fwd(a, wd.view(Cc, K), bd_, B, T, Cc, K,
                                   bn=(bn_eps, bn_momentum, running_mean, running_var, nbt) if (training and bound is None) else None)
            if d is not None and training and bound is None:
                d, bmean, brstd = d
        if d is None:
            gl = ops.glu_fwd(a, Cc)
            d = ops.dwconv_fwd(gl, wd.view(Cc, K), bd_, B, T, Cc, K)
        if training:
            if bmean is None:
                bmean, brstd = ops.bn_stats(d, M, Cc, bn_eps, bn_momentum, running_mean, running_var, nbt, bound=bound)
        else:
            bmean = running_mean
            brstd = ops.axpby(running_var, None, 1.0, 0.0)
            brstd = torch.rsqrt_(brstd.add_(bn_eps))
        e = ops.bn_apply(d, bmean, brstd, g, be, M, Cc, act, adt)
        ctx.rp = rp
        if rp is not None:
            out = ops.rowproj(e, rp[2], Cc, bias=b2, R=x2, drop=(p_out, s_out) if p_out > 0.0 else None)
        elif p_out > 0.0 and (ops.fast() or ops.f32_epilogue_drop()):
            out = ops.linear_fwd(e, ops.wshadow(w2).view(Cc, Cc), b2, R=x2, drop=(p_out, s_out))
        elif p_out > 0.0:
            br = ops.linear_fwd(e, ops.wshadow(w2).view(Cc, Cc), b2)
            out = ops.axpby(x2, ops.dropout(br, p_out, s_out), 1.0, 1.0)
        else:
            out = ops.linear_fwd(e, ops.wshadow(w2).view(Cc, Cc), b2, R=x2 if eps is not None else None)
        ctx.save_for_backward(x2, mean, rstd, xn, a, gl, d, bmean, brstd, e)
        ctx.pr = GradSink.use(params)
        ctx.cfg = (B, T, D, Cc, K, act, training, drop)
        ctx.bound = bound
        ctx.prev = _prev_drop(x)
        return _tag_out(out.view(B, T, D), p_out, s_out)

    @staticmethod
    def backward(ctx, dout):
        x2, mean, rstd, xn, a, gl, d, bmean, brstd, e = ctx.saved_tensors
        ln_w, ln_b, w1, b1, wd, bd_, g, be, w2, b2 = ctx.pr
        B, T, D, Cc, K, act, training, (p_out, s_out) = ctx.cfg
        M = B * T
        adt = ops.act_dtype()
        sink = GradSink(ctx.pr)
        do = dout.reshape(M, D).contiguous()
        dob = _grad_in(dout, do, p_out, s_out)
        rp = ctx.rp
        ops.linear_bwd_w(dob, e, sink.buf(8).view(Cc, Cc), db=sink.buf(9))
        if rp is not None:
            de = ops.rowproj(dob, rp[3], Cc)
        else:
            de = ops.linear_bwd_x(dob, ops.wshadow(w2).view(Cc, Cc))
        dd = ops.bn_bwd(de, d, bmean, brstd, g, be, sink.buf(6), sink.buf(7), M, Cc, act, training, bound=ctx.bound)
        if gl is None:
            da = ops.dwconv_glu_bwd_x(dd, wd.view(Cc, K), a, B, T, Cc, K, adt)
            if ctx.bound is not None:
                ops.mask_time(da, T, ctx.bound[1])
            ops.dwconv_glu_bwd_w(dd, a, sink.buf(4).view(Cc, K), sink.buf(5), B, T, Cc, K)
        else:
            dgl = ops.dwconv_bwd_x(dd, wd.view(Cc, K), B, T, Cc, K)
            ops.dwconv_bwd_w(dd, gl, sink.buf(4).view(Cc, K), sink.buf(5), B, T, Cc, K)
            da = ops.glu_bwd(dgl, a, Cc, adt)
            if ctx.bound is not None:
                ops.mask_time(da, T, ctx.bound[1])
        ops.linear_bwd_w(da, xn, sink.buf(2).view(2 * Cc, D), db=sink.buf(3))
        if rp is not None and da.dtype == torch.float32:
            dx = _rp_ln_bwd(da, rp[1], x2, ln_w, mean, rstd, do, sink.buf(0), sink.buf(1), ctx.prev, (B, T, D))
        else:
            dxn = ops.linear_bwd_x(da, ops.wshadow(w1).view(2 * Cc, D))
            dx = _ln_bwd_out(dxn, x2, ln_w, mean, rstd, do, sink.buf(0), sink.buf(1), ctx.prev, (B, T, D))
        return (dx, None, None, None, None, None, None, None, None) + sink.results()


_TAPS_FWD = [(kh, kw) for kh in range(3) for kw in range(3)]
_CLASSES = [((0, 0), [(0, 0), (0, 2), (2, 0), (2, 2)]), ((0, 1), [(0, 1), (2, 1)]),
            ((1, 0), [(1, 0), (1, 2)]), ((1, 1), [(1, 1)])]


def _conv3s2_fwd(y_in, w, b, B, Hi, Wi, Cc, adt):
    Ho, Wo = (Hi - 3) // 2 + 1, (Wi - 3) // 2 + 1
    wf, wd = ops.conv2_weight_prep(w, adt)
    g = ops.make_gather(Cc, _TAPS_FWD, Ho, Wo, Hi, Wi, 2, 2)
    M = B * Ho * Wo
    y = torch.empty(M, Cc, device=y_in.device, dtype=adt)
    ops.gemm(y_in, wf, y, M, Cc, 9 * Cc, 9 * Cc, Cc, Cc, transB=1, bias=b, epilogue=EPI_RELU, gather=g)
    return y, wd, Ho, Wo


def _conv3s2_bwd(dy, y_in, wd, dw_buf, db_buf, B, Hi, Wi, Ho, Wo, Cc, adt):
    dev = dy.device
    M = B * Ho * Wo
    ops.colsum(dy, db_buf)
    dwf = torch.zeros(9 * Cc, Cc, device=dev, dtype=torch.float32)
    g = ops.make_gather(Cc, _TAPS_FWD, Ho, Wo, Hi, Wi, 2, 2)
    f32_big = (not ops.fast()) and Cc % 128 == 0
    tile = 128 if f32_big else 64
    ntile = (9 * Cc // tile) * ((Cc + tile - 1) // tile)
    want = 1024 if ops.fast() else 1008 if f32_big else 2304
    sk = max(2, min(64, (want + ntile - 1) // ntile, max(1, M // 256)))
    ops.gemm(y_in, dy, dwf, 9 * Cc, Cc, M, 9 * Cc, Cc, Cc, transA=1, transB=1, gather=g, splitk=sk, tile=tile)
    ops.conv2_weight_grad(dwf, dw_buf, Cc, Cc)
    dy_in = torch.empty(y_in.shape, device=dev, dtype=adt)
    q0, classes = 0, []
    for (ph, pw), taps in _CLASSES:
        Hc, Wc = (Hi - ph + 1) // 2, (Wi - pw + 1) // 2
        if Hc > 0 and Wc > 0:
            gt = ops.make_gather(Cc, [((ph - kh) // 2, (pw - kw) // 2) for kh, kw in taps], Hc, Wc, Ho, Wo, 1, 1)
            cm = ops.make_rowmap(Hc, Wc, Hi, Wi, 2, ph, 2, pw)
            nt = len(taps)
            ops.gemm(dy, wd, dy_in, B * Hc * Wc, Cc, nt * Cc, nt * Cc, Cc, Cc, transB=1, b_off=q0 * Cc * Cc,
                     gather=gt, cmap=cm, epilogue=EPI_MUL_RELU_MASK, aux=y_in, ldaux=Cc, defer=classes)
        q0 += len(taps)
    ops.gemm_multi(classes)
    return dy_in


def _taps(k):
    return [(kh, kw) for kh in range(k) for kw in range(k)]


def _conv_ks_fwd(y_in, w, b, B, Hi, Wi, Cc, adt, k, st):
    Ho, Wo = (Hi - k) // st + 1, (Wi - k) // st + 1
    KK = k * k
    wf = torch.empty(KK, Cc, Cc, device=y_in.device, dtype=torch.float32)
    ops.permute4(w.contiguous(), wf, (Cc, Cc, KK, 1), (1, Cc, Cc * Cc, 0))
    wd = torch.empty(KK, Cc, Cc, device=y_in.device, dtype=torch.float32)
    ops.permute4(w.contiguous(), wd, (Cc, Cc, KK, 1), (Cc, 1, Cc * Cc, 0))
    wf, wd = ops.to_act(wf), ops.to_act(wd)
    M = B * Ho * Wo
    y32 = torch.empty(M, Cc, device=y_in.device, dtype=torch.float32)
    taps = _taps(k)
    for t0 in range(0, KK, 9):
        ch = taps[t0:t0 + 9]
        g = ops.make_gather(Cc, ch, Ho, Wo, Hi, Wi, st, st)
        ops.gemm(y_in, wf, y32, M, Cc, len(ch) * Cc, len(ch) * Cc, Cc, Cc, transB=1, bias=b if t0 == 0 else None,
                 beta=0.0 if t0 == 0 else 1.0, gather=g, b_off=t0 * Cc * Cc)
    y = ops.dropout(y32, 0.0, 0, act=ACT_RELU, out_dtype=adt)
    return y, wd, Ho, Wo


def _conv_ks_bwd(dy, y_in, wd, dw_buf, db_buf, B, Hi, Wi, Ho, Wo, Cc, adt, k, st):
    dev = dy.device
    M = B * Ho * Wo
    KK = k * k
    taps = _taps(k)
    ops.colsum(dy, db_buf)
    dwf = torch.zeros(KK * Cc, Cc, device=dev, dtype=torch.float32)
    for t0 in range(0, KK, 9):
        ch = taps[t0:t0 + 9]
        g = ops.make_gather(Cc, ch, Ho, Wo, Hi, Wi, st, st)
        ntile = (len(ch) * Cc // 64) * ((Cc + 63) // 64)
        sk = max(2, min(64, (1024 + ntile - 1) // ntile, max(1, M // 256)))
        ops.gemm(y_in, dy, dwf, len(ch) * Cc, Cc, M, len(ch) * Cc, Cc, Cc, transA=1, transB=1, gather=g, splitk=sk, tile=64,
                 c_off=t0 * Cc * Cc)
    ops.permute4(dwf, dw_buf, (KK, Cc, Cc, 1), (1, KK, Cc * KK, 0), accumulate=True)
    dy_in = torch.empty(y_in.shape, device=dev, dtype=adt)
    order, classes = [], []
    for ph in range(st):
        for pw in range(st):
            ct = [(kh, kw) for kh in range(ph, k, st) for kw in range(pw, k, st)]
            classes.append(((ph, pw), ct))
            order += [kh * k + kw for kh, kw in ct]
    wd_cls = wd.index_select(0, torch.tensor(order, device=dev)).contiguous()
    q0, jobs = 0, []
    for (ph, pw), ct in classes:
        Hc, Wc = (Hi - ph + st - 1) // st, (Wi - pw + st - 1) // st
        if Hc > 0 and Wc > 0 and ct:
            gt = ops.make_gather(Cc, [((ph - kh) // st, (pw - kw) // st) for kh, kw in ct], Hc, Wc, Ho, Wo, 1, 1)
            cm = ops.make_rowmap(Hc, Wc, Hi, Wi, st, ph, st, pw)
            nt = len(ct)
            ops.gemm(dy, wd_cls, dy_in, B * Hc * Wc, Cc, nt * Cc, nt * Cc, Cc, Cc, transB=1, b_off=q0 * Cc * Cc,
                     gather=gt, cmap=cm, epilogue=EPI_MUL_RELU_MASK, aux=y_in, ldaux=Cc, defer=jobs)
        q0 += len(ct)
    ops.gemm_multi(jobs)
    return dy_in


class Conv2dSubsamplingFn(torch.autograd.Function):

    @staticmethod
    def forward(ctx, x, xscale, c1_w, c1_b, lin_w, lin_b, *convs):
        B, T, F = x.shape
        Cc = c1_w.shape[0]
        D = lin_w.shape[0]
        H1, W1 = (T - 3) // 2 + 1, (F - 3) // 2 + 1
        adt = ops.act_dtype()
        x = x.contiguous()
        ys = [ops.conv1_fwd(x, c1_w, c1_b, B, T, F, Cc, adt)]
        dims, wds = [(H1, W1)], []
        for i in range(0, len(convs), 2):
            k = convs[i].shape[-1]
            if k == 3:
                y, wd, Ho, Wo = _conv3s2_fwd(ys[-1].view(-1, Cc), convs[i], convs[i + 1], B, dims[-1][0], dims[-1][1], Cc, adt)
            else:
                y, wd, Ho, Wo = _conv_ks_fwd(ys[-1].view(-1, Cc), convs[i], convs[i + 1], B, dims[-1][0], dims[-1][1], Cc,
                                             adt, k, (k + 1) // 2)
            ys.append(y)
            wds.append(wd)
            dims.append((Ho, Wo))
        Hl, Wl = dims[-1]
        assert lin_w.shape[1] == Cc * Wl
        wl = torch.empty(D, Wl * Cc, device=x.device, dtype=torch.float32)
        ops.permute4(lin_w, wl, (D, Cc, Wl, 1), (Wl * Cc, 1, Cc, 0))
        wl = ops.to_act(wl)
        out = ops.linear_fwd(ys[-1].view(B * Hl, Wl * Cc), wl, lin_b, alpha=xscale)
        ctx.save_for_backward(x, wl, *ys, *wds)
        ctx.pr = GradSink.use((c1_w, c1_b, lin_w, lin_b) + tuple(convs))
        ctx.cfg = (B, T, F, Cc, D, dims, xscale)
        ctx.ks = [convs[i].shape[-1] for i in range(0, len(convs), 2)]
        return out.view(B, Hl, D)

    @staticmethod
    def backward(ctx, dout):
        B, T, F, Cc, D, dims, xscale = ctx.cfg
        n = len(dims) - 1
        x, wl = ctx.saved_tensors[:2]
        ys = ctx.saved_tensors[2:3 + n]
        wds = ctx.saved_tensors[3 + n:]
        adt = ops.act_dtype()
        sink = GradSink(ctx.pr)
        dev = x.device
        Hl, Wl = dims[-1]
        dob = ops.to_act(dout.reshape(B * Hl, D).contiguous())
        ylv = ys[-1].view(B * Hl, Wl * Cc)
        dwl = torch.zeros(D, Wl * Cc, device=dev, dtype=torch.float32)
        ops.linear_bwd_w(dob, ylv, dwl, alpha=xscale, db=sink.buf(3))
        ops.permute4(dwl, sink.buf(2), (D, Wl, Cc, 1), (Wl * Cc, 1, Wl, 0), accumulate=True)
        dy = ops.linear_bwd_x(dob, wl, epilogue=EPI_MUL_RELU_MASK, aux=ylv, alpha=xscale, out_dtype=adt)
        dy = dy.view(B * Hl * Wl, Cc)
        for i in range(n - 1, -1, -1):
            (Hi, Wi), (Ho, Wo) = dims[i], dims[i + 1]
            if ctx.ks[i] == 3:
                dy = _conv3s2_bwd(dy, ys[i].view(-1, Cc), wds[i], sink.buf(4 + 2 * i), sink.buf(5 + 2 * i), B, Hi, Wi, Ho,
                                  Wo, Cc, adt)
            else:
                dy = _conv_ks_bwd(dy, ys[i].view(-1, Cc), wds[i], sink.buf(4 + 2 * i), sink.buf(5 + 2 * i), B, Hi, Wi, Ho,
                                  Wo, Cc, adt, ctx.ks[i], (ctx.ks[i] + 1) // 2)
        ops.conv1_bwd_w(dy, x, sink.buf(0), sink.buf(1), B, T, F, Cc)
        return (None, None) + sink.results()


class EmbedPEFn(torch.autograd.Function):
    @staticmethod
    def forward(ctx, tokens, table, pe, scale, pos_offset):
        B, U = tokens.shape
        if U == 1 and not torch.is_grad_enabled():
            return ops.embed_pe(tokens, table, pe, U, scale, pos_offset).view(B, U, table.shape[1])
        tok = tokens.contiguous()
        out = ops.embed_pe(tok, table, pe, U, scale, pos_offset)
        ctx.save_for_backward(tok)
        ctx.pr = GradSink.use((table,))
        ctx.scale = scale
        return out.view(B, U, table.shape[1])

    @staticmethod
    def backward(ctx, dout):
        (tok,) = ctx.saved_tensors
        sink = GradSink(ctx.pr)
        ops.embed_bwd(tok, dout.reshape(-1, dout.shape[-1]).contiguous(), sink.buf(0), ctx.scale)
        return (None,) + sink.results() + (None, None, None)


class PosEncFn(torch.autograd.Function):

    @staticmethod
    def forward(ctx, x, pe, scale):
        B, T, D = x.shape
        ctx.scale = scale
        return ops.posenc(x.reshape(-1, D).contiguous(), pe, T, scale).view(B, T, D)

    @staticmethod
    def backward(ctx, dout):
        return ops.axpby(dout.contiguous(), None, ctx.scale, 0.0), None, None


class ScaledPosEncFn(torch.autograd.Function):

    @staticmethod
    def forward(ctx, x, pe, alpha, scale):
        B, T, D = x.shape
        ctx.save_for_backward(pe)
        ctx.pr = GradSink.use((alpha,))
        ctx.cfg = (T, scale)
        return ops.posenc_scaled(x.reshape(-1, D).contiguous(), pe, alpha.reshape(1), T, scale).view(B, T, D)

    @staticmethod
    def backward(ctx, dout):
        (pe,) = ctx.saved_tensors
        T, scale = ctx.cfg
        sink = GradSink(ctx.pr)
        do = dout.contiguous()
        ops.posenc_scaled_bwd(do.view(-1, do.shape[-1]), pe, sink.buf(0).view(1), T)
        dx = do if scale == 1.0 else ops.axpby(do, None, scale, 0.0)
        res = sink.results()
        return dx, None, res[0], None


class CTCLossFn(torch.autograd.Function):

    @staticmethod
    def forward(ctx, acts, ys_pad, hlens, blank, ignore_id, time_major=False):
        B = acts.shape[1] if time_major else acts.shape[0]
        nll, grad = ops.ctc_loss(acts.contiguous(), ys_pad, hlens, blank, ignore_id, 1.0 / B,
                                 want_grad=acts.requires_grad, time_major=time_major)
        ctx.save_for_backward(grad)
        ctx.nll = nll
        return ops.reduce_sum(nll, 1.0 / B)

    @staticmethod
    def backward(ctx, g):
        (grad,) = ctx.saved_tensors
        return ops.scale_dev(grad, g.contiguous(), 1.0, out=grad), None, None, None, None, None


class CTCRowsLossFn(torch.autograd.Function):

    @staticmethod
    def forward(ctx, acts, ys_pad, hlens, blank, ignore_id):
        B = acts.shape[0]
        nll, grad = ops.ctc_loss(acts.contiguous(), ys_pad, hlens, blank, ignore_id, 1.0 / B, want_grad=acts.requires_grad)
        ctx.save_for_backward(grad)
        return nll / B

    @staticmethod
    def backward(ctx, g):
        (grad,) = ctx.saved_tensors
        return grad * g.view(-1, 1, 1), None, None, None, None


class CTCPITLossFn(torch.autograd.Function):

    @staticmethod
    def forward(ctx, acts, ys_pad, hlens, blank, ignore_id, record=None):
        S, B = acts.shape[:2]
        nll, perm, pit, grad = ops.ctc_pit_loss(acts.contiguous(), ys_pad, hlens, blank, ignore_id, 1.0 / (S * B * B),
                                                want_grad=acts.requires_grad)
        if record is not None:
            record.update(nll_pair=nll, pit=pit)
        ctx.save_for_backward(grad)
        ctx.mark_non_differentiable(perm)
        return ops.reduce_sum(pit, 1.0 / B), perm

    @staticmethod
    def backward(ctx, g, _gp):
        (grad,) = ctx.saved_tensors
        return ops.scale_dev(grad, g.contiguous(), 1.0, out=grad), None, None, None, None, None


class LabelSmoothingLossFn(torch.autograd.Function):

    @staticmethod
    def forward(ctx, logits, target, smoothing, ignore_id, denom):
        V = logits.shape[-1]
        lg = logits.reshape(-1, V).contiguous()
        tg = target.reshape(-1).contiguous()
        loss_rows, correct, grad = ops.lsm_loss(lg, tg, smoothing, 1.0 / denom, ignore_id,
                                                want_grad=logits.requires_grad)
        ctx.save_for_backward(grad)
        ctx.shp = logits.shape
        ctx.mark_non_differentiable(correct)
        return ops.reduce_sum(loss_rows, 1.0 / denom), correct

    @staticmethod
    def backward(ctx, g, _gc):
        (grad,) = ctx.saved_tensors
        return ops.scale_dev(grad, g.contiguous(), 1.0, out=grad).view(ctx.shp), None, None, None, None


class ScaleFn(torch.autograd.Function):

    @staticmethod
    def forward(ctx, x, a):
        ctx.a = a
        return ops.axpby(x.reshape(-1).contiguous(), None, a, 0.0).view(x.shape)

    @staticmethod
    def backward(ctx, g):
        return ops.axpby(g.reshape(-1).contiguous(), None, ctx.a, 0.0).view(g.shape), None


class WeightedSumFn(torch.autograd.Function):

    @staticmethod
    def forward(ctx, a, b, alpha):
        ctx.alpha = alpha
        return ops.axpby(a.reshape(1), b.reshape(1), alpha, 1.0 - alpha).reshape(())

    @staticmethod
    def backward(ctx, g):
        g1 = g.reshape(1).contiguous()
        return (ops.axpby(g1, None, ctx.alpha, 0.0).reshape(()),
                ops.axpby(g1, None, 1.0 - ctx.alpha, 0.0).reshape(()), None)
```

### espnet_amd/ops.py

```python
import ctypes as C
import os
import math

import torch

from . import _lib
from ._lib import GatherT, GemmT, RowMapT, check, ptr, stream_ptr

ACT_NONE, ACT_RELU, ACT_SWISH = 0, 1, 2
EPI_NONE, EPI_RELU, EPI_SWISH, EPI_MUL_RELU_MASK, EPI_MUL_DSWISH, EPI_MUL_AUX, EPI_DACT_FACTOR, EPI_ROW_STATS, EPI_ROW_GRAD = 0, 1, 2, 3, 4, 5, 6, 7, 8

_PRECISIONS = {"fp32": 0, "bf16": 1}
_state = {"precision": 0}


def set_precision(name):
    if name not in _PRECISIONS:
        raise ValueError(f"precision must be one of {list(_PRECISIONS)}")
    _state["precision"] = _PRECISIONS[name]


def get_precision():
    return [k for k, v in _PRECISIONS.items() if v == _state["precision"]][0]


def fast():
    return _state["precision"] == 1


def f32_epilogue_drop():
    return _state["precision"] == 0 and F32_EPILOGUE_DROP


F32_EPILOGUE_DROP = True


def act_dtype():
    return torch.bfloat16 if fast() else torch.float32


def wshadow(p):
    if not fast():
        return p
    sh = getattr(p, "_eamd_bf16", None)
    if sh is not None and getattr(p, "_eamd_bf16_ver", None) == p._version:
        return sh
    if sh is None:
        sh = torch.empty(p.shape, device=p.device, dtype=torch.bfloat16)
        p._eamd_bf16 = sh
    cast_bf16(p.detach().contiguous(), sh)
    p._eamd_bf16_ver = p._version
    return sh


def to_act(x):
    if fast() and x.dtype == torch.float32:
        return cast_bf16(x.contiguous())
    return x


def to_act_shared(x):
    if not (fast() and x.dtype == torch.float32):
        return x
    c = getattr(x, "_eamd_act", None)
    if c is not None and c[1] == x._version and c[0].shape == x.shape:
        return c[0]
    y = cast_bf16(x.contiguous())
    x._eamd_act = (y, x._version)
    return y


def _numel_from(t, off):
    return t.numel() - off


def _span(rows, ld, cols):
    return (rows - 1) * ld + cols if rows > 0 else 0


_time_bound = {"t": None}


def set_time_bound(t):
    if t is not None and not (t.is_cuda and t.dtype == torch.int32 and t.numel() == 1):
        raise _lib.EamdError("time bound: one int32 element on the device")
    _time_bound["t"] = t


def time_bound():
    return _time_bound["t"]


def mask_time(x, T, bound):
    rows = x.numel() // x.shape[-1]
    assert x.is_contiguous() and rows % T == 0 and x.dtype in (torch.float32, torch.bfloat16)
    check(_lib.lib().eamd_mask_time(ptr(x), rows, x.shape[-1], T, ptr(bound), x.dtype == torch.bfloat16,
                                    stream_ptr()), "eamd_mask_time")
    return x


_gemm_record = None


def gemm(A, B, Cm, M, N, K, lda, ldb, ldc, *, transA=0, transB=0, bias=None, aux=None, ldaux=0, R=None,
         ldr=0, batch=(1, 1), sA=(0, 0), sB=(0, 0), sC=(0, 0), alpha=1.0, beta=0.0, a_act=0, b_act=0,
         epilogue=0, splitk=1, tile=0, gather=None, cmap=None, a_off=0, b_off=0, c_off=0, precision=None,
         colsum=None, Cb=None, drop=None, Hb=None, h_act=0, group=False, stats=None, defer=None):
    bf = A.dtype == torch.bfloat16
    if A.dtype != B.dtype or A.dtype not in (torch.float32, torch.bfloat16) or not (A.is_cuda and B.is_cuda):
        raise _lib.EamdError("gemm needs float32 or bfloat16 GPU operands of one dtype")
    if stats is not None:
        assert epilogue in (EPI_ROW_STATS, EPI_ROW_GRAD) and tile in (64, 128) and splitk == 1
        assert (Cm is None and Cb is None) if epilogue == EPI_ROW_STATS else Cm is not None
    c32 = Cm if (Cm is not None and Cm.dtype == torch.float32) else None
    c16 = Cb if Cb is not None else (Cm if (Cm is not None and Cm.dtype == torch.bfloat16) else None)
    if c16 is not None and (c16.dtype != torch.bfloat16 or not bf):
        raise _lib.EamdError("gemm: bf16 outputs need bf16 operands")
    for tt in (R, bias, colsum):
        if tt is not None and tt.dtype != torch.float32:
            raise _lib.EamdError("gemm: bias / residual / colsum must be float32")
    b1, b2 = batch
    if gather is None:
        a_span = _span(K, lda, M) if transA else _span(M, lda, K)
        a_need = a_off + (b1 - 1) * sA[0] + (b2 - 1) * sA[1] + a_span
        if a_need > A.numel():
            raise _lib.EamdError(f"gemm: A too small ({A.numel()} < {a_need})")
    b_span = _span(K, ldb, N) if transB else _span(N, ldb, K)
    b_need = b_off + (b1 - 1) * sB[0] + (b2 - 1) * sB[1] + b_span
    if b_need > B.numel():
        raise _lib.EamdError(f"gemm: B too small ({B.numel()} < {b_need})")
    if cmap is None:
        c_need = c_off + (b1 - 1) * sC[0] + (b2 - 1) * sC[1] + _span(M, ldc, N)
        for ct in (c32, c16):
            if ct is not None and c_need > ct.numel():
                raise _lib.EamdError(f"gemm: C too small ({ct.numel()} < {c_need})")
    if bias is not None and bias.numel() < N:
        raise _lib.EamdError("gemm: bias too small")

    p = GemmT()
    p.A, p.B = ptr(A, a_off), ptr(B, b_off)
    p.C = ptr(c32, c_off) if c32 is not None else None
    p.Cb = ptr(c16, c_off) if c16 is not None else None
    p.bias = ptr(bias)
    p.aux = ptr(aux, c_off) if aux is not None else None
    p.aux_dtype = 1 if (aux is not None and aux.dtype == torch.bfloat16) else 0
    p.R = ptr(R, c_off) if R is not None else None
    if colsum is not None:
        if not transA or gather is not None or colsum.numel() < M * b1 * b2:
            raise _lib.EamdError("gemm: colsum needs transA, no gather and M outputs")
        p.colsum = ptr(colsum)
    p.M, p.N, p.K = M, N, K
    p.transA, p.transB = int(transA), int(transB)
    p.lda, p.ldb, p.ldc, p.ldaux, p.ldr = lda, ldb, ldc, ldaux or ldc, ldr or ldc
    p.batch1, p.batch2 = b1, b2
    p.sA1, p.sA2 = sA
    p.sB1, p.sB2 = sB
    p.sC1, p.sC2 = sC
    p.alpha, p.beta = alpha, beta
    p.a_act, p.b_act, p.epilogue = a_act, b_act, epilogue
    p.splitk = splitk
    p.in_dtype = 1 if bf else 0
    p.precision = 1 if bf else (_state["precision"] if precision is None else precision)
    p.tile = tile
    if stats is not None and epilogue == EPI_ROW_GRAD:
        rowc, col, fix, gscale, scale = stats
        if rowc.dtype != torch.float32 or rowc.numel() < 3 * M or col.dtype != torch.int32 or col.numel() < M or not (0 <= fix < N):
            raise _lib.EamdError("gemm: row-gradient coefficients too small or of the wrong dtype")
        p.stats.rowc, p.stats.col, p.stats.fix, p.stats.gscale, p.stats.scale = ptr(rowc), ptr(col), int(fix), ptr(gscale), float(scale)
    elif stats is not None:
        part, col, zcol, zfix, fix = stats
        tn = (N + tile - 1) // tile
        if part.dtype != torch.float32 or part.numel() < M * tn * 2 or zfix.numel() < M or not (0 <= fix < N) or \
                (col is not None and (col.dtype != torch.int32 or col.numel() < M or zcol is None or zcol.numel() < M)):
            raise _lib.EamdError("gemm: row-statistics buffers too small or of the wrong dtype")
        p.stats.part, p.stats.col, p.stats.zcol, p.stats.zfix, p.stats.fix = ptr(part), ptr(col), ptr(zcol), ptr(zfix), int(fix)
    if gather is not None:
        p.gather = gather
    if cmap is not None:
        p.cmap = cmap
    if drop is not None and drop[0] > 0.0:
        if ldc != N or c_off != 0 or (not bf and p.precision != 0):
            raise _lib.EamdError("gemm: fused dropout needs a contiguous [M, N] result and bf16 or fp32-MFMA operands")
        p.drop_p, p.drop_salt = float(drop[0]), int(drop[1])
        p.drop_step = ptr(rng_state(A.device))
        if Hb is not None:
            if Hb.dtype != (torch.bfloat16 if bf else torch.float32) or Hb.numel() < M * N:
                raise _lib.EamdError("gemm: Hb must be an [M, N] buffer of the operand dtype")
            p.Hb, p.h_act, p.h_dtype = ptr(Hb), h_act, 0 if bf else 1
    if group and _wgroup["on"] and _in_grad_arena(Cm) and _wgroup_accepts(p):
        lo = Cm.data_ptr() + 4 * c_off
        hi = lo + 4 * _span(M, ldc, N)
        nbytes = A.numel() * A.element_size() + B.numel() * B.element_size()
        clash = any(lo < qhi and qlo < hi and (splitk == 1 or qsk == 1) for qlo, qhi, qsk in _wgroup["ranges"])
        if clash or _wgroup["bytes"] + nbytes > GROUP_WGRAD_MAX_BYTES:
            wgrad_group_flush()
        _wgroup["items"].append((p, (A, B, Cm, colsum)))
        _wgroup["ranges"].append((lo, hi, splitk))
        _wgroup["bytes"] += nbytes
        return
    if defer is not None:
        defer.append((p, (A, B, Cm, bias, aux, R, colsum, Cb, Hb, stats)))
        return
    if _gemm_record is not None:
        _gemm_record.append((p, (A, B, Cm, bias, aux, R, colsum, Cb, Hb, stats),
                             lambda sp, p=p: check(_lib.lib().eamd_gemm(C.byref(p), sp), "eamd_gemm")))
    check(_lib.lib().eamd_gemm(C.byref(p), stream_ptr()), "eamd_gemm")


GEMM_MULTI_MAX = 4


def gemm_multi(items):
    L = _lib.lib()
    for i0 in range(0, len(items), GEMM_MULTI_MAX):
        part = items[i0:i0 + GEMM_MULTI_MAX]
        arr = (GemmT * len(part))(*[it[0] for it in part])
        n = len(part)
        if _gemm_record is not None and any(it[0].in_dtype != 0 or it[0].precision != 0 for it in part):
            for p_, keep in part:
                _gemm_record.append((p_, keep, lambda sp, p_=p_: check(L.eamd_gemm(C.byref(p_), sp), "eamd_gemm")))
        elif _gemm_record is not None:
            _gemm_record.append((dict(kind="multi%d" % n, flop=sum(2.0 * it[0].M * it[0].N * it[0].K for it in part)),
                                 (arr, [it[1] for it in part]),
                                 lambda sp, arr=arr, n=n: check(L.eamd_gemm_multi(arr, n, sp), "eamd_gemm_multi")))
        check(L.eamd_gemm_multi(arr, n, stream_ptr()), "eamd_gemm_multi")


GROUP_WGRAD = True
STACK_WGRAD_MAX_ROWS = 64
GROUP_WGRAD_MAX_TILES = 384
GROUP_WGRAD_SK_DIV = 2
GROUP_WGRAD_TILE128_MIN = 100
GROUP_WGRAD_T128_WGS = 96
GROUP_WGRAD_MAX_BYTES = 16 << 30
_wgroup = {"on": False, "items": [], "ranges": [], "bytes": 0, "stack": {}, "pinned": [], "reserve": [], "arenas": {}}


def register_grad_arena(t):
    import weakref
    key = t.untyped_storage().data_ptr()
    _wgroup["arenas"][key] = weakref.ref(t)


def _in_grad_arena(t):
    key = t.untyped_storage().data_ptr()
    ref = _wgroup["arenas"].get(key)
    if ref is None:
        return False
    a = ref()
    if a is None or a.untyped_storage().data_ptr() != key:
        del _wgroup["arenas"][key]
        return False
    return True


def wgrad_group_begin():
    _wgroup["on"] = GROUP_WGRAD
    _wgroup["items"], _wgroup["stack"] = [], {}
    _wgroup["ranges"], _wgroup["bytes"] = [], 0


def _wgroup_accepts(p):
    if ((p.M + 63) // 64) * ((p.N + 63) // 64) > GROUP_WGRAD_MAX_TILES:
        return False
    first = (C.c_int32 * 2)()
    return _lib.lib().eamd_gemm_group_plan(C.byref(p), 1, first) > 0


def _wgroup_staging(nbytes):
    if torch.cuda.is_current_stream_capturing():
        for i, h in enumerate(_wgroup["reserve"]):
            if h.numel() >= nbytes:
                _wgroup["pinned"].append(_wgroup["reserve"].pop(i))
                return _wgroup["pinned"][-1][:nbytes]
        return None
    want = (nbytes + 4095) // 4096 * 4096 * 2
    _wgroup["reserve"] = [h for h in _wgroup["reserve"] if h.numel() >= want]
    while len(_wgroup["reserve"]) < 16:
        _wgroup["reserve"].append(torch.empty(want, dtype=torch.uint8, pin_memory=True))
    return torch.empty(nbytes, dtype=torch.uint8, pin_memory=True)


def wgrad_group_flush():
    stack, _wgroup["stack"] = _wgroup["stack"], {}
    for dW, db, dys, xs in stack.values():
        if len(dys) == 1:
            dyc, xc = dys[0], xs[0]
        else:
            dyc, xc = torch.cat(dys, 0), torch.cat(xs, 0)
        if dyc.shape[0] <= STACK_WGRAD_MAX_ROWS:
            sk = auto_splitk(dyc.shape[1], xc.shape[1], dyc.shape[0])
            gemm(dyc, xc, dW, dyc.shape[1], xc.shape[1], dyc.shape[0], dyc.shape[1], xc.shape[1], xc.shape[1], transA=1,
                 transB=1, splitk=sk, beta=1.0 if sk == 1 else 0.0, colsum=db, group=True)
        else:
            _linear_bwd_w(dyc, xc, dW, db=db)
    items = _wgroup["items"]
    if not items:
        return
    _wgroup["items"], _wgroup["ranges"], _wgroup["bytes"] = [], [], 0
    for tile in (64, 128):
        part = [it for it in items if (128 if it[0].tile == 128 else 64) == tile]
        if part:
            _wgroup_launch(part, tile)


def _wgroup_launch(items, tile):
    L = _lib.lib()

    def separately():
        for p, keep in items:
            if _gemm_record is not None:
                _gemm_record.append((p, keep, lambda sp, p=p: check(L.eamd_gemm(C.byref(p), sp), "eamd_gemm")))
            check(L.eamd_gemm(C.byref(p), stream_ptr()), "eamd_gemm")

    if len(items) == 1:
        return separately()
    n = len(items)
    dev = items[0][1][0].device
    arr = (GemmT * n)(*[it[0] for it in items])
    first = (C.c_int32 * (n + 1))()
    total = L.eamd_gemm_group_plan(arr, n, first)
    check(min(total, 0), "eamd_gemm_group_plan")
    nb_desc, nb_first = C.sizeof(arr), C.sizeof(first)
    host = _wgroup_staging(nb_desc + nb_first)
    if host is None:
        return separately()
    C.memmove(host.data_ptr(), arr, nb_desc)
    C.memmove(host.data_ptr() + nb_desc, first, nb_first)
    tab = torch.empty(nb_desc + nb_first, dtype=torch.uint8, device=dev)
    tab.copy_(host, non_blocking=True)
    in_dtype = int(arr[0].in_dtype)
    args = (ptr(tab), ptr(tab, nb_desc), n, total, in_dtype, tile)
    check(L.eamd_gemm_group_launch(*args, stream_ptr()), "eamd_gemm_group_launch")
    if _gemm_record is not None:
        _gemm_record.append((dict(kind="group%d" % tile, flop=sum(2.0 * it[0].M * it[0].N * it[0].K * it[0].batch1 * it[0].batch2 for it in items)),
                             (tab, [it[1] for it in items]),
                             lambda sp, args=args: check(L.eamd_gemm_group_launch(*args, sp), "eamd_gemm_group_launch")))


def cast_bf16(x, out=None):
    if out is None:
        out = torch.empty(x.shape, device=x.device, dtype=torch.bfloat16)
    assert x.dtype == torch.float32 and x.is_contiguous() and out.numel() == x.numel()
    check(_lib.lib().eamd_cast_bf16(ptr(x), ptr(out), x.numel(), stream_ptr()), "eamd_cast_bf16")
    return out


def auto_splitk(m_out, n_out, k_red):
    tiles = ((m_out + 63) // 64) * ((n_out + 63) // 64)
    if tiles >= 512:
        return 1
    want = 4.0 * (128.0 / tiles) ** 0.5
    s = 1
    while s < want:
        s *= 2
    return max(1, min(s, 64, max(1, k_red // 128)))


LINEAR_ROWS = True
_infer = 0


class inference:

    def __enter__(self):
        global _infer
        _infer += 1

    def __exit__(self, *exc):
        global _infer
        _infer -= 1
        return False


def inference_call(fn):
    import functools

    @functools.wraps(fn)
    def wrapped(*a, **k):
        with inference():
# ... 1366 lines not shown
    check(_lib.lib().eamd_ngram_score_pairs(*_ngram_query_args(lm), V, lm.order, lm.unk, ptr(ctx) if Cw else None, ptr(tok), ptr(lp),
                                            ptr(ctx_new) if Cw else None, n, stream_ptr()), "eamd_ngram_score_pairs")
    return lp, ctx_new


CTC_BEAM_MAX_W, CTC_BEAM_MAX_K, CTC_BEAM_MAX_T = 32, 32, 2048


def ctc_beam_candidates(logp, cand_size):
    B, T, V = logp.shape
    if logp.dtype != torch.float32 or not logp.is_contiguous():
        raise _lib.EamdError("ctc_prefix_beam: contiguous float32 [B, T, V]")
    K = int(cand_size)
    if not 1 <= K <= min(CTC_BEAM_MAX_K, V - 2):
        raise _lib.EamdError("ctc_prefix_beam: 1 <= candidates <= min(%d, V - 2)" % CTC_BEAM_MAX_K)
    rows = B * T
    cval = torch.empty(rows, K, device=logp.device, dtype=torch.float32)
    cidx = torch.empty(rows, K, device=logp.device, dtype=torch.int64)
    cid = torch.empty(rows, K, device=logp.device, dtype=torch.int32)
    check(_lib.lib().eamd_topk_rows_i32(ptr(logp, 1), V, rows, V - 2, K, ptr(cval), ptr(cidx), ptr(cid), stream_ptr()),
          "eamd_topk_rows_i32")
    return cval, cid


def ctc_prefix_beam_search(logp, cval, cid, hlens, beam_size, nbest, penalty=0.0, lm=None, ngram_weight=0.0, ws=None, out=None):
    B, T, V = logp.shape
    K = cval.shape[1]
    assert hlens.dtype == torch.int32 and hlens.numel() == B and hlens.is_contiguous() and hlens.device == logp.device
    assert cval.shape == (B * T, K) and cid.shape == (B * T, K) and cid.dtype == torch.int32
    W = int(beam_size)
    if not (1 <= nbest <= W <= CTC_BEAM_MAX_W and T <= CTC_BEAM_MAX_T):
        raise _lib.EamdError("ctc_prefix_beam: 1 <= nbest <= beam <= %d, T <= %d" % (CTC_BEAM_MAX_W, CTC_BEAM_MAX_T))
    dev = logp.device
    ws_bytes = _lib.lib().eamd_ctc_beam_workspace_bytes(B, T, W)
    if ws is None:
        ws = torch.empty(ws_bytes, device=dev, dtype=torch.uint8)
    if out is None:
        out = torch.empty(B, nbest, 2 + T, device=dev, dtype=torch.int32)
    assert ws.numel() >= ws_bytes and out.shape == (B, nbest, 2 + T) and out.dtype == torch.int32 and out.is_contiguous()
    if lm is not None:
        if lm.uni_tok.device != dev or lm.uni_tok.numel() != V:
            raise _lib.EamdError("ctc_prefix_beam: the n-gram tables on the device of logp, over the same %d tokens" % V)
        tables, order, bos, unk = _ngram_query_args(lm), lm.order, lm.bos, lm.unk
    else:
        tables, order, bos, unk = (None,) * 9 + (0,), 0, 0, 0
    check(_lib.lib().eamd_ctc_prefix_beam(ptr(logp), V, ptr(cval), ptr(cid), ptr(hlens), B, T, V, W, K, int(nbest),
                                          penalty, *tables, order, bos, unk, ngram_weight, ptr(ws),
                                          ws.numel(), ptr(out), stream_ptr()), "eamd_ctc_prefix_beam")
    return out, ws


def ctc_prefix_beam(logp, hlens, beam_size, cand_size, nbest, penalty=0.0, lm=None, ngram_weight=0.0):
    cval, cid = ctc_beam_candidates(logp, cand_size)
    return ctc_prefix_beam_search(logp, cval, cid, hlens, beam_size, nbest, penalty, lm, ngram_weight)[0]


BF_PSD, BF_PSD_BWD, BF_MVDR_BWD, BF_APPLY_BWD = 0, 1, 2, 3
BF_TCHUNK = 64


def _bf_f32(*ts):
    for t in ts:
        if t is not None and (t.dtype != torch.float32 or not t.is_contiguous()):
            raise _lib.EamdError("beamformer kernels take contiguous float32 tensors, complex as a trailing (re, im) axis")


def _bf_workspace(op, S, B, T, Cn, F, device):
    n = _lib.lib().eamd_bf_workspace_bytes(op, S, B, T, Cn, F)
    if n < 0:
        raise _lib.EamdError(f"eamd_bf_workspace_bytes refused S={S} B={B} T={T} C={Cn} F={F} (2 <= C <= 8)")
    return torch.empty(n // 4, device=device, dtype=torch.float32)


def bf_psd(x, z, out=None):
    B, T, Cn, F, two = x.shape
    S, Tm = z.shape[0], z.shape[3]
    assert two == 2 and z.shape == (S, B, Cn, Tm, F) and Tm <= T
    _bf_f32(x, z)
    if out is None:
        out = (torch.empty(S, B, F, Cn, Cn, 2, device=x.device, dtype=torch.float32), torch.empty(B, Cn, F, device=x.device, dtype=torch.float32),
               torch.empty(S, B, F, device=x.device, dtype=torch.float32))
    psd, feat, nrm = out
    assert psd.shape == (S, B, F, Cn, Cn, 2) and feat.shape == (B, Cn, F) and nrm.shape == (S, B, F)
    _bf_f32(psd, feat, nrm)
    ws = _bf_workspace(BF_PSD, S, B, Tm, Cn, F, x.device)
    check(_lib.lib().eamd_bf_psd(ptr(x), ptr(z), ptr(psd), ptr(feat), ptr(nrm), ptr(ws), S, B, T, Tm, Cn, F, stream_ptr()),
          "eamd_bf_psd")
    return psd, feat, nrm


def bf_psd_bwd(x, z, psd, nrm, gpsd, gfeat, out=None):
    B, T, Cn, F, _ = x.shape
    S, Tm = z.shape[0], z.shape[3]
    assert psd.shape == (S, B, F, Cn, Cn, 2) and nrm.shape == (S, B, F)
    assert gpsd is None or gpsd.shape == psd.shape
    assert gfeat is None or gfeat.shape == (B, Cn, F)
    _bf_f32(x, z, psd, nrm, gpsd, gfeat)
    dz = torch.empty_like(z) if out is None else out
    assert dz.shape == z.shape
    _bf_f32(dz)
    ws = _bf_workspace(BF_PSD_BWD, S, B, Tm, Cn, F, x.device)
    check(_lib.lib().eamd_bf_psd_bwd(ptr(x), ptr(z), ptr(psd), ptr(nrm), ptr(gpsd), ptr(gfeat), ptr(dz), ptr(ws), S, B, T, Tm,
                                     Cn, F, stream_ptr()), "eamd_bf_psd_bwd")
    return dz


def bf_mvdr(psd_s, psd_n, u, out=None):
    B, F, Cn = psd_s.shape[:3]
    assert psd_s.shape == (B, F, Cn, Cn, 2) and psd_n.shape == psd_s.shape and u.shape == (B, Cn)
    _bf_f32(psd_s, psd_n, u)
    w = torch.empty(B, F, Cn, 2, device=psd_s.device, dtype=torch.float32) if out is None else out
    assert w.shape == (B, F, Cn, 2)
    _bf_f32(w)
    check(_lib.lib().eamd_bf_mvdr(ptr(psd_s), ptr(psd_n), ptr(u), ptr(w), B, F, Cn, stream_ptr()), "eamd_bf_mvdr")
    return w


def bf_mvdr_bwd(psd_s, psd_n, u, gw, out=None):
    B, F, Cn = psd_s.shape[:3]
    assert psd_n.shape == psd_s.shape and u.shape == (B, Cn) and gw.shape == (B, F, Cn, 2)
    _bf_f32(psd_s, psd_n, u, gw)
    gs, gn, gu = (torch.empty_like(psd_s), torch.empty_like(psd_n), torch.empty_like(u)) if out is None else out
    assert gs.shape == psd_s.shape and gn.shape == psd_s.shape and gu.shape == u.shape
    _bf_f32(gs, gn, gu)
    ws = _bf_workspace(BF_MVDR_BWD, 1, B, 1, Cn, F, u.device)
    check(_lib.lib().eamd_bf_mvdr_bwd(ptr(psd_s), ptr(psd_n), ptr(u), ptr(gw), ptr(gs), ptr(gn), ptr(gu), ptr(ws), B, F, Cn,
                                      stream_ptr()), "eamd_bf_mvdr_bwd")
    return gs, gn, gu


def bf_apply(w, x, out=None):
    B, T, Cn, F, _ = x.shape
    assert w.shape == (B, F, Cn, 2)
    _bf_f32(w, x)
    y = torch.empty(B, T, F, 2, device=x.device, dtype=torch.float32) if out is None else out
    assert y.shape == (B, T, F, 2)
    _bf_f32(y)
    check(_lib.lib().eamd_bf_apply(ptr(w), ptr(x), ptr(y), B, T, Cn, F, stream_ptr()), "eamd_bf_apply")
    return y


def bf_apply_bwd(gy, x, out=None):
    B, T, Cn, F, _ = x.shape
    assert gy.shape == (B, T, F, 2)
    _bf_f32(gy, x)
    gw = torch.empty(B, F, Cn, 2, device=x.device, dtype=torch.float32) if out is None else out
    assert gw.shape == (B, F, Cn, 2)
    _bf_f32(gw)
    ws = _bf_workspace(BF_APPLY_BWD, 1, B, T, Cn, F, x.device)
    check(_lib.lib().eamd_bf_apply_bwd(ptr(gy), ptr(x), ptr(gw), ptr(ws), B, T, Cn, F, stream_ptr()), "eamd_bf_apply_bwd")
    return gw


def ctc_loss(acts_btv, ys_pad, ilens, blank=0, ignore_id=-1, grad_scale=1.0, want_grad=True, time_major=False):
    if time_major:
        T, B, V = acts_btv.shape
        st, sb = B * V, V
    else:
        B, T, V = acts_btv.shape
        st, sb = V, T * V
    L = ys_pad.shape[1]
    assert acts_btv.is_contiguous() and ys_pad.is_contiguous() and ys_pad.dtype == torch.int64
    assert ilens.dtype == torch.int32 and ilens.numel() == B and ys_pad.shape[0] == B
    ws_bytes = _lib.lib().eamd_ctc_workspace_bytes(B, T, L)
    ws = torch.empty(ws_bytes, device=acts_btv.device, dtype=torch.uint8)
    nll = torch.empty(B, device=acts_btv.device, dtype=torch.float32)
    grad = torch.empty_like(acts_btv) if want_grad else None
    check(_lib.lib().eamd_ctc_loss(ptr(acts_btv), st, sb, ptr(ys_pad), ptr(ilens), ptr(nll),
                                   ptr(grad), st, sb, ptr(ws), B, T, V, L, blank, ignore_id,
                                   grad_scale, stream_ptr()), "eamd_ctc_loss")
    return nll, grad


def ctc_pit_loss(acts, ys_pad, ilens, blank=0, ignore_id=-1, grad_scale=1.0, want_grad=True):
    S, B, T, V = acts.shape
    L = ys_pad.shape[2]
    assert acts.is_contiguous() and acts.dtype == torch.float32
    assert ys_pad.is_contiguous() and ys_pad.dtype == torch.int64 and tuple(ys_pad.shape[:2]) == (B, S)
    assert ilens.dtype == torch.int32 and ilens.numel() == B
    dev = acts.device
    ws = torch.empty(_lib.lib().eamd_ctc_pit_workspace_bytes(S, B, T, L), device=dev, dtype=torch.uint8)
    nll = torch.empty(B, S, S, device=dev, dtype=torch.float32)
    perm = torch.empty(B, S, device=dev, dtype=torch.int64)
    pit = torch.empty(B, device=dev, dtype=torch.float32)
    grad = torch.empty_like(acts) if want_grad else None
    check(_lib.lib().eamd_ctc_pit_loss(ptr(acts), ptr(ys_pad), ptr(ilens), ptr(nll), ptr(perm), ptr(pit), ptr(grad), ptr(ws), S, B,
                                       T, V, L, blank, ignore_id, grad_scale, stream_ptr()), "eamd_ctc_pit_loss")
    return nll, perm, pit, grad


def ctc_forced_align(acts, ilens, ys_pad, blank=0, ignore_id=-1, normalized=False, time_major=False):
    if time_major:
        T, B, V = acts.shape
        st, sb = B * V, V
    else:
        B, T, V = acts.shape
        st, sb = V, T * V
    L = ys_pad.shape[1]
    assert acts.is_contiguous() and ys_pad.is_contiguous() and ys_pad.dtype == torch.int64 and acts.dtype == torch.float32
    assert ilens.dtype == torch.int32 and ilens.numel() == B and ys_pad.shape[0] == B
    dev = acts.device
    if L == 0:
        seg = torch.empty(B, 0, device=dev, dtype=torch.int32)
        out = ctc_forced_align(acts, ilens, torch.full((B, 1), ignore_id, device=dev, dtype=torch.int64), blank, ignore_id,
                               normalized, time_major)
        return out[:3] + (seg, seg.clone())
    ws = torch.empty(_lib.lib().eamd_ctc_align_workspace_bytes(B, T, L), device=dev, dtype=torch.uint8)
    score = torch.empty(B, device=dev, dtype=torch.float32)
    states = torch.empty(B, T, device=dev, dtype=torch.int32)
    tokens = torch.empty(B, T, device=dev, dtype=torch.int64)
    seg_start = torch.empty(B, L, device=dev, dtype=torch.int32)
    seg_end = torch.empty(B, L, device=dev, dtype=torch.int32)
    check(_lib.lib().eamd_ctc_forced_align(ptr(acts), st, sb, ptr(ys_pad), ptr(ilens), ptr(score),
                                           ptr(states), ptr(tokens), ptr(seg_start), ptr(seg_end), ptr(ws), B, T, V, L, blank,
                                           ignore_id, bool(normalized), stream_ptr()), "eamd_ctc_forced_align")
    return score, states, tokens, seg_start, seg_end


def maskctc_seed(logits, hlens, thr, K, mask_token, eos, blank=0, Lcap=None):
    B, T, V = logits.shape
    Lcap = T if Lcap is None else int(Lcap)
    assert logits.dtype == torch.float32 and logits.is_contiguous() and hlens.dtype == torch.int32 and hlens.numel() == B
    dev = logits.device
    i32 = lambda *s: torch.empty(*s, device=dev, dtype=torch.int32)
    out = dict(y_in=torch.empty(B, Lcap, device=dev, dtype=torch.int64), tok_p=torch.empty(B, Lcap, device=dev, dtype=torch.float32),
               len=i32(B), nmask=i32(B), niter=i32(B), kper=i32(B), frame_id=i32(B, T),
               frame_p=torch.empty(B, T, device=dev, dtype=torch.float32))
    check(_lib.lib().eamd_maskctc_seed(ptr(logits), ptr(hlens), ptr(out["frame_id"]), ptr(out["frame_p"]), ptr(out["y_in"]),
                                       ptr(out["tok_p"]), ptr(out["len"]), ptr(out["nmask"]), ptr(out["niter"]), ptr(out["kper"]),
                                       B, T, V, Lcap, blank, mask_token, eos, float(thr), int(K), stream_ptr()),
          "eamd_maskctc_seed")
    return out


def maskctc_update(pass_, logits, y_in, lens, niter, kper, mask_token, score=None, arg=None):
    B, L, V = logits.shape
    assert logits.dtype == torch.float32 and logits.is_contiguous() and y_in.dtype == torch.int64 and y_in.stride(1) == 1
    assert y_in.shape[0] == B and y_in.shape[1] >= L
    dev = logits.device
    if score is None:
        score = torch.empty(B, L, device=dev, dtype=torch.float32)
        arg = torch.empty(B, L, device=dev, dtype=torch.int32)
    check(_lib.lib().eamd_maskctc_update(int(pass_), ptr(logits), ptr(y_in), ptr(lens), ptr(niter), ptr(kper), ptr(score), ptr(arg),
                                         B, L, y_in.stride(0), V, mask_token, stream_ptr()), "eamd_maskctc_update")
    return score, arg


def ctc_prefix_score(logp, r_prev, cand, last, olen, blank, eos):
    T, V = logp.shape
    nhyp, ncand = cand.shape
    assert r_prev.shape == (nhyp, T, 2) and cand.dtype == torch.int32 and logp.is_contiguous()
    psi = torch.empty(nhyp, ncand, device=logp.device, dtype=torch.float32)
    r_new = torch.empty(nhyp, ncand, T, 2, device=logp.device, dtype=torch.float32)
    check(_lib.lib().eamd_ctc_prefix_score(ptr(logp), ptr(r_prev.contiguous()), ptr(cand.contiguous()), ptr(last),
                                           ptr(olen), ptr(psi), ptr(r_new), nhyp, ncand, T, V, blank, eos,
                                           stream_ptr()), "eamd_ctc_prefix_score")
    return psi, r_new


def ctc_prefix_score_batch(logp, lens, per_utt, r_prev, cand, last, olen, blank, eos):
    U, Tmax, V = logp.shape
    nhyp, ncand = cand.shape
    assert nhyp == U * per_utt and r_prev.shape == (nhyp, Tmax, 2) and cand.dtype == torch.int32 and logp.is_contiguous()
    assert lens.dtype == torch.int32 and lens.numel() == U
    psi = torch.empty(nhyp, ncand, device=logp.device, dtype=torch.float32)
    r_new = torch.zeros(nhyp, ncand, Tmax, 2, device=logp.device, dtype=torch.float32)
    check(_lib.lib().eamd_ctc_prefix_score_batch(ptr(logp), ptr(lens), U, per_utt, ptr(r_prev.contiguous()), ptr(cand.contiguous()),
                                                 ptr(last), ptr(olen), ptr(psi), ptr(r_new), ncand, Tmax, V, blank, eos,
                                                 stream_ptr()), "eamd_ctc_prefix_score_batch")
    return psi, r_new


def ctc_prefix_psi(logp, lens, per_utt, r_prev, cand, last, olen, blank, eos, olen_dev=None):
    U, Tmax, V = logp.shape
    nhyp, ncand = cand.shape
    assert nhyp == U * per_utt and r_prev.shape == (nhyp, Tmax, 2) and cand.dtype == torch.int32 and logp.is_contiguous()
    psi = torch.empty(nhyp, ncand, device=logp.device, dtype=torch.float32)
    rc = _lib.lib().eamd_ctc_prefix_psi_dyn(ptr(logp), ptr(lens), U, per_utt, ptr(r_prev.contiguous()), ptr(cand.contiguous()), ptr(last),
                                            int(olen), ptr(olen_dev), ptr(psi), ncand, Tmax, V, blank, eos, stream_ptr())
    if rc == _lib.EAMD_EUNSUPPORTED:
        return None
    check(rc, "eamd_ctc_prefix_psi_dyn")
    return psi


def ctc_prefix_state(logp, lens, per_utt, r_prev, parent, tok, last, olen, alive, blank, out=None, olen_dev=None):
    U, Tmax, V = logp.shape
    n = parent.numel()
    r = out if out is not None else torch.empty(n, Tmax, 2, device=logp.device, dtype=torch.float32)
    check(_lib.lib().eamd_ctc_prefix_state_dyn(ptr(logp), ptr(lens), U, per_utt, ptr(r_prev), ptr(parent), ptr(tok), ptr(last), int(olen),
                                               ptr(olen_dev), ptr(alive), ptr(r), Tmax, V, blank, stream_ptr()), "eamd_ctc_prefix_state_dyn")
    return r


def grad_norm(g, ws, out):
    check(_lib.lib().eamd_grad_norm(ptr(g), g.numel(), ptr(ws), ptr(out), stream_ptr()),
          "eamd_grad_norm")


def sched_step(state, gnorm, mode, base_lr, factor, dmodel, warmup, beta1, beta2, max_norm):
    check(_lib.lib().eamd_sched_step(ptr(state), ptr(gnorm), mode, base_lr, factor,
                                     dmodel, warmup, beta1, beta2,
                                     max_norm, stream_ptr()), "eamd_sched_step")


def adam_step(p, g, m, v, state, beta1, beta2, eps, weight_decay, p16=None):
    n = p.numel()
    assert g.numel() == n and m.numel() == n and v.numel() == n and (p16 is None or p16.numel() == n)
    check(_lib.lib().eamd_adam_step(ptr(p), ptr(g), ptr(m), ptr(v), ptr(p16), n, ptr(state), beta1,
                                    beta2, eps, weight_decay, stream_ptr()),
          "eamd_adam_step")


def adadelta_step(p, g, sq, acc, state, rho, weight_decay, p16=None):
    check(_lib.lib().eamd_adadelta_step(ptr(p), ptr(g), ptr(sq), ptr(acc), ptr(p16), p.numel(), ptr(state),
                                        rho, weight_decay, stream_ptr()), "eamd_adadelta_step")


def add_gradient_noise(g, sigma, salt=0x6e6f697365):
    check(_lib.lib().eamd_add_gradient_noise(ptr(g), g.numel(), sigma, ptr(rng_state(g.device)),
                                             salt, stream_ptr()), "eamd_add_gradient_noise")


def make_gather(Cc, taps, Ho, Wo, Hin, Win, sh, sw):
# ... 635 lines not shown
```

### include/espnet_amd.h

```cpp
#ifndef ESPNET_AMD_H_
#define ESPNET_AMD_H_
#include <stdint.h>
#ifdef __cplusplus
extern "C" {
#endif

int eamd_abi_version(void);

typedef struct {
  int32_t enabled;
  int32_t C;
  int32_t ntap;
  int32_t Ho, Wo;
  int32_t Hin, Win;
  int32_t sh, sw;
  int32_t dh[9], dw[9];
} eamd_gather_t;

typedef struct {
  int32_t enabled;
  int32_t Ho, Wo;
  int32_t Hc, Wc;
  int32_t sh, oh, sw, ow;
} eamd_rowmap_t;

typedef struct {
  const float* A; const float* B; float* C;
  const float* bias; const float* aux; const float* R;
  float* colsum;
  int32_t M, N, K;
  int32_t transA, transB;
  int64_t lda, ldb, ldc, ldaux, ldr;
  int32_t batch1, batch2;
  int64_t sA1, sA2, sB1, sB2, sC1, sC2;
  float alpha, beta;
  int32_t a_act, b_act, epilogue;
  int32_t splitk;
  int32_t precision;
  int32_t tile;
  eamd_gather_t gather;
  eamd_rowmap_t cmap;
  void* Cb;
  int32_t in_dtype;
  int32_t aux_dtype;
  float drop_p;
  uint64_t drop_salt;
  const uint64_t* drop_step;
  void* Hb;
  int32_t h_act;
  int32_t h_dtype;
  struct {
    float* part; const int32_t* col; float* zcol; float* zfix; int32_t fix; int32_t reserved;
    const float* rowc; const float* gscale; float scale; int32_t reserved2;
  } stats;
} eamd_gemm_t;

int eamd_gemm(const eamd_gemm_t* p, void* stream);

#define EAMD_GEMM_MULTI_MAX 4
int eamd_gemm_multi(const eamd_gemm_t* descs, int n, void* stream);

int eamd_gemm_group_plan(const eamd_gemm_t* descs, int n, int32_t* first);
int eamd_gemm_group_launch(const eamd_gemm_t* descs_dev, const int32_t* first_dev, int n, int total, int in_dtype, int tile,
                           void* stream);

typedef struct {
  const float* x; const float* w1; const float* b1; const float* w2; const float* b2; const float* R;
  float* out; float* f; float* h;
  int32_t M, D, F, act;
  float alpha;
  float p_in; uint64_t salt_in; float p_out; uint64_t salt_out; const void* drop_step;
  int32_t dtype;
  int32_t hsplit;
  const float* ln_x; const float* ln_w; const float* ln_b; float* ln_mean; float* ln_rstd;
  float ln_eps; int32_t reserved2;
  const float* lnb_x; const float* lnb_gamma; const float* lnb_mean; const float* lnb_rstd; const float* lnb_dres;
  float* lnb_ws; float* lnb_drop_out; uint64_t lnb_drop_salt; float lnb_drop_p; int32_t reserved3;
} eamd_ffn_t;
int eamd_ffn_fwd(const eamd_ffn_t* p, void* stream);
int eamd_ffn_bwd(const eamd_ffn_t* p, void* stream);
typedef struct {
  const float* w1; const float* w2;
  float* fwd_first; float* fwd_second; float* bwd_first; float* bwd_second;
  int32_t D, F;
} eamd_ffn_pack_t;
int eamd_ffn_pack_f32_multi(const eamd_ffn_pack_t* jobs, int njobs, void* stream);

typedef struct {
  const float* a; int64_t lda;
  const float* w; const float* bias;
  const float* R; int64_t ldr;
  float* out; int64_t ldo;
  int32_t M, K, N, a_act;
  float alpha; float p_out; uint64_t salt_out; const void* drop_step;
  const float* ln_x; const float* ln_w; const float* ln_b; float* ln_mean; float* ln_rstd; float ln_eps; float lnb_drop_p;
  const float* a_scale; const float* a_shift; float* a_out;
  const float* lnb_x; const float* lnb_gamma; const float* lnb_mean; const float* lnb_rstd; const float* lnb_dres;
  float* lnb_ws; float* lnb_drop_out; uint64_t lnb_drop_salt;
} eamd_rowproj_t;
typedef struct {
  const float* w; float* image;
  int32_t K, N, ldw, trans;
} eamd_rowproj_pack_t;
int eamd_rowproj(const eamd_rowproj_t* p, void* stream);
int eamd_rowproj_pack_f32(const eamd_rowproj_pack_t* jobs, int njobs, void* stream);
int64_t eamd_rowproj_lnb_workspace(int M);
int eamd_ffn_pack_f32(const float* w1, const float* w2, float* fwd_first, float* fwd_second, float* bwd_first, float* bwd_second,
                      int D, int F, void* stream);
int eamd_ffn_pack_bf16(const void* w1, const void* w2, void* fwd_first, void* fwd_second, void* bwd_first, void* bwd_second,
                       int D, int F, void* stream);

int eamd_layernorm_fwd(const float* x, const float* gamma, const float* beta, float* y, void* y_bf16, float* mean,
                       float* rstd, int rows, int D, float eps, void* stream);
int64_t eamd_layernorm_bwd_workspace(int rows, int D);
typedef struct {
  const float* ws; float* dgamma; float* dbeta;
  int32_t nblk, D;
} eamd_ln_reduce_job_t;
int eamd_layernorm_bwd_reduce(const eamd_ln_reduce_job_t* jobs, int njobs, void* stream);
int eamd_layernorm_bwd(const float* dy, const float* x, const float* gamma, const float* mean,
                       const float* rstd, const float* dres, float* dx, float* dgamma, float* dbeta,
                       float* workspace, int rows, int D, void* stream);
int eamd_layernorm_bwd_drop(const float* dy, const float* x, const float* gamma, const float* mean, const float* rstd,
                            const float* dres, float* dx, void* dx_drop_bf16, float drop_p, const uint64_t* step_dev,
                            uint64_t salt, float* dgamma, float* dbeta, float* workspace, int rows, int D, void* stream);
int eamd_layernorm_bwd_drop_f32(const float* dy, const float* x, const float* gamma, const float* mean, const float* rstd,
                                const float* dres, float* dx, float* dx_drop, float drop_p, const uint64_t* step_dev,
                                uint64_t salt, float* dgamma, float* dbeta, float* workspace, int rows, int D, void* stream);

int eamd_softmax_fwd(const float* ac, const float* bd, const unsigned char* mask, int64_t mask_bstride,
                     int64_t mask_qstride, float* P, void* P_bf16, int nblocks, int B, int T1, int T2, int64_t ld,
                     float scale, void* stream);
int eamd_softmax_bwd(const float* P, const void* P_bf16, float* dP, float* dbd, void* dS_bf16, void* dbd_bf16,
                     int nblocks, int T1, int T2, int64_t ld, float scale, void* stream);

int eamd_attn_fwd(const void* qu, int64_t ldq, const void* qv, int64_t ldqv, const void* k, int64_t ldk, const void* v,
                  int64_t ldv, const void* pos, int64_t ldpos, const unsigned char* mask, int64_t mask_bstride,
                  int64_t mask_qstride, void* P_bf16, int64_t ldp, void* ctx_bf16, int64_t ldc, int B, int H, int T1,
                  int T2, int dk, float scale, void* Pd_bf16, float drop_p, const uint64_t* drop_step, uint64_t drop_salt,
                  const int32_t* shift_len, void* stream);

int eamd_attn_bwd_q(const void* dctx, int64_t ldd, const void* k, int64_t ldk, const void* v, int64_t ldv,
                    const void* P_bf16, int64_t ldp, void* dS_bf16, void* dbd_bf16, void* dq, int64_t ldo, int dq_is_bf16,
                    int B, int H, int T1, int T2, int dk, float scale, float drop_p, const uint64_t* drop_step,
                    uint64_t drop_salt, const int32_t* shift_len, void* stream);

int eamd_attn_fwd_f32(const float* qu, int64_t ldq, const float* qv, int64_t ldqv, const float* k, int64_t ldk,
                      const float* v, int64_t ldv, const float* pos, int64_t ldpos, const unsigned char* mask,
                      int64_t mask_bstride, int64_t mask_qstride, float* P, int64_t ldp, float* ctx, int64_t ldc, int B,
                      int H, int T1, int T2, int dk, float scale, float* Pd, float drop_p, const uint64_t* drop_step,
                      uint64_t drop_salt, const int32_t* shift_len, void* stream);
int eamd_attn_bwd_q_f32(const float* dctx, int64_t ldd, const float* k, int64_t ldk, const float* v, int64_t ldv,
                        const float* P, int64_t ldp, float* dS, float* dbd, float* dq, int64_t ldo, int B, int H, int T1,
                        int T2, int dk, float scale, float drop_p, const uint64_t* drop_step, uint64_t drop_salt,
                        const int32_t* shift_len, void* stream);

int eamd_attn_bwd_kv_f32(const float* Pd, const float* dS, const float* dbd, int64_t ldp, const float* dctx, int64_t ldd,
                         const float* qu, int64_t ldq, const float* qv, int64_t ldqv, float* dv, float* dk_out, int64_t ldo,
                         float* dpos, int64_t ldpos, int B, int H, int T1, int T2, int dk, void* stream);

int eamd_attn_bwd_kv(const void* Pd_bf16, const void* dS_bf16, int64_t ldp, const void* dctx, int64_t ldd, const void* qu,
                     int64_t ldq, void* dv, void* dk_out, int64_t ldo, int B, int H, int T1, int T2, int dk, void* stream);

int eamd_lsm_loss(const float* logits, const int64_t* target, float* loss_rows, float* correct_rows,
                  float* grad, int rows, int V, int ignore_id, float smoothing, float inv_denom,
                  void* stream);
int eamd_argmax_rows(const float* x, int64_t ld, int32_t* out, int rows, int V, void* stream);
int eamd_reduce_sum(const float* in, int64_t n, float* out, float scale, void* stream);
int eamd_log_softmax_rows(const float* x, float* y, int rows, int V, void* stream);
int eamd_transducer_expand_rows(const float* logits, int64_t ld, int n, int V, int k, const float* lm, const int32_t* lm_row,
                                const int32_t* pairs, int g, float* rec, float* pair_out, void* stream);
int eamd_beam_finish(const float* top_s, const int64_t* top_i, int n, int beam, int V, int W, int L, int step, int eos,
                     const int64_t* maxlen, int ns, int nf, const float* sc_in, const float* const* logps, const float* c_local,
                     int64_t ldc, int full_mode, const int64_t* ids, int ncand, const int64_t* yseq_in, float* sc_out,
                     int64_t* yseq_out, float* hyp_out, int64_t* hyp_i, int64_t* tok_i, int64_t* pos, float* rec, void* stream);
int eamd_linear_rows_f32(const float* x, const float* W, const float* bias, const float* R, float* y, int M, int N, int K,
                         int a_act, int act, float alpha, int64_t ldx, int64_t ldr, void* stream);
int eamd_linear_rows_ln_f32(const float* x, const float* gamma, const float* beta, float eps, const float* W, const float* bias,
                            const float* R, float* y, int M, int N, int K, int act, float alpha, int64_t ldx, int64_t ldr,
                            int64_t ldy, void* stream);
int eamd_decode_self_attn_dyn(const float* qkv, int64_t ldq, float* kcache, float* vcache, const int32_t* slot_at, int Lcap, int pos,
                              const int32_t* pos_dev, int n, int H, int D, float* ctx, void* stream);
int eamd_beam_slots_dyn(const int32_t* slot_in, int32_t* slot_out, const int64_t* hyp, int n, int Lcap, int pos, const int32_t* pos_dev,
                        void* stream);
int eamd_decode_src_attn(const float* q, int64_t ldq, const float* kmem, const float* vmem, int64_t ldkv, const uint8_t* mask, int nutt,
                         int g, int T, int H, int D, float* ctx, void* stream);
int eamd_decode_src_attn_group(const float* q, int64_t ldq, const float* kmem, const float* vmem, int64_t ldkv, const uint8_t* mask, int nutt,
                         int g, int T, int H, int D, float* ctx, void* stream);
int64_t eamd_decode_src_attn_split_workspace(int nutt, int g, int H, int splits);
int eamd_decode_src_attn_split(const float* q, int64_t ldq, const float* kmem, const float* vmem, int64_t ldkv, const uint8_t* mask,
                               int nutt, int g, int T, int H, int D, int splits, float* ws, float* ctx, void* stream);
int eamd_weighted_sum(const float* const* logps, const float* weights, int nf, int64_t numel, float* out, void* stream);
int eamd_beam_select(const float* pre, const int64_t* ids, const float* psi, const float* c_s, const float* hyp, float w_ctc,
                     int nutt, int beam, int P, int V, float* c_local, float* top_s, int64_t* top_i, void* stream);
int eamd_topk_rows_i32(const float* x, int64_t ld, int rows, int n, int k, float* vals, int64_t* idx, int32_t* idx32, void* stream);
int eamd_copy_jobs(const void* const* src, void* const* dst, const int64_t* nbytes, int njobs, void* stream);
int eamd_weighted_topk_rows(const float* const* logps, const float* weights, int nf, int rows, int n, int k, int extra, float* pre,
                            float* vals, int64_t* idx, int32_t* idx32, void* stream);
int eamd_beam_step_dyn(const float* pre, const int64_t* ids, const float* psi, const float* c_s, const float* hyp, float w_ctc, int nutt,
                       int beam, int P, int V, int W, int L, int step, int eos, const int64_t* maxlen, int ns, int nf, const float* sc_in,
                       const float* const* logps, const int64_t* yseq_in, float* c_local, float* sc_out, int64_t* yseq_out, float* hyp_out,
                       int64_t* hyp_i, int64_t* tok_i, int32_t* tok32, float* cs_out, float* rec, const int32_t* step_dev, int32_t* step_out,
                       int ring, const int32_t* slot_in, int32_t* slot_out, int Lcap, void* stream);

int eamd_axpby(const float* x, const float* y, float* out, int64_t n, float a, float b, void* stream);
int eamd_cast_bf16(const float* x, void* y_bf16, int64_t n, void* stream);
int eamd_scale_dev(const float* x, const float* scale_dev, float* out, int64_t n, float extra, void* stream);
int eamd_act_fwd(const float* x, float* y, int64_t n, int act, void* stream);
int eamd_act_bwd(const float* dy, const float* x, float* dx, int64_t n, int act, void* stream);
int eamd_glu_fwd(const float* x, float* y, int64_t rows, int C, void* stream);
int eamd_glu_bwd(const float* dy, const float* x, float* dx, void* dx_bf16, int64_t rows, int C, void* stream);
int eamd_add_bias2(const void* q, int64_t ldq, const float* u, const float* v, void* qu, void* qv, int64_t rows, int D,
                   int bf16, void* stream);
int eamd_add_cast_bf16(const float* a, const float* b, void* out_bf16, int64_t rows, int cols, int64_t ld_out,
                       void* stream);
int eamd_add_block_f32(const float* a, const float* b, float* out, int64_t rows, int cols, int64_t ld_out, void* stream);
int eamd_add_cast_colsum2(const float* a, const float* b, void* out_bf16, int64_t ld_out, float* suma, float* sumb,
                          int64_t rows, int D, void* stream);
int eamd_add_colsum2_f32(const float* a, const float* b, float* out, int64_t ld_out, float* suma, float* sumb, int64_t rows,
                         int D, void* stream);
int eamd_colsum(const void* x, int64_t ld, float* out, int64_t rows, int D, float scale, int x_bf16, void* stream);
int eamd_embed_pe_dyn(const int64_t* tok, int64_t ldt, const float* table, const float* pe, float* out, int64_t rows, int U, int D,
                      float scale, int pos_offset, const int32_t* pos_dev, void* stream);
int eamd_embed_bwd(const int64_t* tok, const float* dout, float* dtable, int64_t rows, int D, float scale,
                   int64_t pad_idx, void* stream);
int eamd_posenc(const float* x, const float* pe, float* out, int64_t rows, int T, int D, float scale,
                void* stream);
int eamd_posenc_scaled(const float* x, const float* pe, const float* alpha, float* out, int64_t rows, int T, int D,
                       float scale, void* stream);
int eamd_posenc_scaled_bwd(const float* dout, const float* pe, float* dalpha, int64_t rows, int T, int D,
                           void* stream);
int eamd_permute4(const float* src, float* dst, int d0, int d1, int d2, int d3, int64_t s0, int64_t s1,
                  int64_t s2, int64_t s3, int accumulate, void* stream);
int eamd_dropout(const void* x, void* y, int64_t n, float p, const uint64_t* step_dev, uint64_t salt, int act,
                 int in_bf16, int out_bf16, void* stream);
int eamd_rng_advance(uint64_t* step_dev, void* stream);

int eamd_dwconv_fwd(const float* x, const float* w, const float* bias, float* y, int B, int T, int C, int K,
                    void* stream);
int eamd_dwconv_bwd_x(const float* dy, const float* w, float* dx, int B, int T, int C, int K, void* stream);
int eamd_dwconv_bwd_w(const float* dy, const float* x, float* dw, float* db, int B, int T, int C, int K,
                      void* stream);
int eamd_dwconv_glu_fwd(const float* a, const float* w, const float* bias, float* y, float* bn_part, int B, int T, int C, int K,
                        void* stream);
int eamd_dwconv_glu_bwd_x(const float* dy, const float* w, const float* a, void* da, int da_bf16, int B, int T, int C, int K,
                          void* stream);
int eamd_dwconv_glu_bwd_w(const float* dy, const float* a, float* dw, float* db, int B, int T, int C, int K, void* stream);
int eamd_bn_nslab(int64_t M, int C);
int eamd_bn_stats(const float* x, float* workspace, float* mean, float* rstd, float* running_mean,
                  float* running_var, int64_t* num_batches_tracked, int64_t M, int C, float eps, float momentum, void* stream);
int eamd_bn_finalize(const float* part, int nslab, float* mean, float* rstd, float* running_mean, float* running_var,
                     int64_t* num_batches_tracked, int C, float eps, float momentum, void* stream);
int eamd_bn_apply(const float* x, const float* mean, const float* rstd, const float* gamma, const float* beta,
                  void* y, int64_t M, int C, int act, int y_bf16, void* stream);
int eamd_bn_stats_bounded(const float* x, float* workspace, float* mean, float* rstd, float* running_mean,
                          float* running_var, int64_t* num_batches_tracked, int64_t M, int C, float eps, float momentum, int T,
                          const int32_t* bound, void* stream);
int eamd_bn_bwd_bounded(const float* dy, const float* x, const float* mean, const float* rstd, const float* gamma,
                        const float* beta, float* workspace, float* dx, float* dgamma, float* dbeta, int64_t M, int C,
                        int act, int training, int T, const int32_t* bound, void* stream);
int eamd_mask_time(void* x, int64_t rows, int C, int T, const int32_t* bound, int is_bf16, void* stream);
int eamd_bn_bwd(const float* dy, const float* x, const float* mean, const float* rstd, const float* gamma,
                const float* beta, float* workspace, float* dx, float* dgamma, float* dbeta, int64_t M, int C,
                int act, int training, void* stream);
int eamd_conv1_fwd(const float* x, const float* w, const float* bias, void* y, int B, int T, int F, int C,
                   int y_bf16, void* stream);
int64_t eamd_conv1_bwd_w_workspace(int B, int T, int C);
int eamd_conv1_bwd_w(const void* dy, const float* x, float* dw, float* db, float* workspace, int B, int T, int F,
                     int C, int dy_bf16, void* stream);

int64_t eamd_ctc_workspace_bytes(int B, int T, int Lmax);
int eamd_ctc_loss(const float* acts, int64_t stride_t, int64_t stride_b, const int64_t* ys_pad,
                  const int32_t* ilens, float* nll, float* grad, int64_t gstride_t, int64_t gstride_b,
                  void* workspace, int B, int T, int V, int Lmax, int blank, int ignore_id, float grad_scale,
                  void* stream);

int64_t eamd_ctc_pit_workspace_bytes(int S, int B, int T, int Lmax);
int eamd_ctc_pit_loss(const float* acts, const int64_t* ys_pad, const int32_t* ilens, float* nll_pair, int64_t* perm, float* pit,
                      float* grad, void* workspace, int S, int B, int T, int V, int Lmax, int blank, int ignore_id, float grad_scale,
                      void* stream);

int64_t eamd_ctc_align_workspace_bytes(int B, int T, int Lmax);
int eamd_ctc_forced_align(const float* acts, int64_t stride_t, int64_t stride_b, const int64_t* ys_pad, const int32_t* ilens,
                          float* score, int32_t* states, int64_t* tokens, int32_t* seg_start, int32_t* seg_end, void* workspace,
                          int B, int T, int V, int Lmax, int blank, int ignore_id, int normalized, void* stream);

int eamd_ctc_prefix_score(const float* logp, const float* r_prev, const int32_t* cand, const int32_t* last,
                          const int32_t* olen, float* psi, float* r_new, int nhyp, int ncand, int T, int V,
                          int blank, int eos, void* stream);

int eamd_ctc_prefix_score_batch(const float* logp, const int32_t* lens, int nutt, int per_utt, const float* r_prev,
                                const int32_t* cand, const int32_t* last, const int32_t* olen, float* psi, float* r_new,
                                int ncand, int Tmax, int V, int blank, int eos, void* stream);
int eamd_ctc_prefix_psi_dyn(const float* logp, const int32_t* lens, int nutt, int per_utt, const float* r_prev, const int32_t* cand,
                            const int32_t* last, int olen, const int32_t* olen_dev, float* psi, int ncand, int Tmax, int V, int blank,
                            int eos, void* stream);
int eamd_ctc_prefix_state_dyn(const float* logp, const int32_t* lens, int nutt, int per_utt, const float* r_prev, const int64_t* parent,
                              const int64_t* tok, const int32_t* last, int olen, const int32_t* olen_dev, const float* alive, float* r_out,
                              int Tmax, int V, int blank, void* stream);

int eamd_specaug(const float* x, float* y, const int32_t* lens, const int32_t* center, const int32_t* warped,
                 const int32_t* fpos, const int32_t* flen, int nf, const int32_t* tpos, const int32_t* tlen, int nt, int B,
                 int T, int F, void* stream);
int eamd_global_mvn(const float* x, float* y, const int32_t* lens, const float* mean, const float* stdv, int B, int T,
                    int F, void* stream);
int eamd_utterance_mvn(const float* x, float* y, const int32_t* lens, float* workspace, int norm_means, int norm_vars,
                       float eps, int B, int T, int F, void* stream);

int eamd_reflect_pad(const float* x, int64_t ldx, float* y, int64_t ldy, int B, int L, int pad, void* stream);
int eamd_logmel(const float* spec, int64_t ld, int64_t rows_per_utt, const float* melmat, const int32_t* lo,
                const int32_t* hi, const int32_t* flens, float* out, int B, int T, int F, int M, float log_scale,
                int power_input, void* stream);

int eamd_ft_logmel_fwd(const float* spec, const float* melmat, const int32_t* lo, const int32_t* hi, const int32_t* lens,
                       float* out, int B, int T, int F, int M, void* stream);
int eamd_ft_logmel_bwd(const float* spec, const float* g, const float* melmat, const int32_t* lo, const int32_t* hi,
                       const int32_t* mlo, const int32_t* mhi, const int32_t* lens, float* gspec, int B, int T, int F, int M,
                       void* stream);
int eamd_ft_mvn_fwd(const float* x, float* y, const int32_t* lens, const float* bias, const float* scale, float* workspace,
                    int apply_utt, int norm_means, int norm_vars, float eps, int B, int T, int M, void* stream);
int eamd_ft_mvn_bwd(const float* gy, float* gx, const int32_t* lens, const float* scale, float* workspace, int apply_utt,
                    int B, int T, int M, void* stream);

int eamd_lstm_cell_fwd(const float* gates, const float* c_prev, const float* h_prev, const uint8_t* live, float* h,
                       float* c, float* y, float* acts, int B, int H, void* stream);
int eamd_lstm_cell_bwd(const float* dy, const float* dh, const float* dc, const float* acts, const float* c_prev,
                       const float* c, const uint8_t* live, float* dgates, float* dc_prev, float* dh_pass, int B, int H,
                       void* stream);
int eamd_lstm_step_fwd(const float* gx, const float* w_hh, const float* b_hh, const float* h_prev, const float* c_prev,
                       const uint8_t* live, float* h, float* c, float* y, float* acts, int B, int H, void* stream);
int eamd_lstm_step_bwd(const float* dy, const float* dgates_next, const float* w_t, const float* dh_pass_in, const float* dc,
                       const float* acts, const float* c_prev, const float* c, const uint8_t* live, float* dgates,
                       float* dc_prev, float* dh_pass, int B, int H, void* stream);
typedef struct {
  const float* gx;
  const float* w_hh;
  const float* b_hh;
  const uint8_t* live;
  float* h_out;
  float* c_out;
  float* y;
  float* acts;
  int32_t reverse;
  int32_t reserved;
} eamd_lstm_seq_fwd_t;
typedef struct {
  const float* dy;
  const float* w_t;
  const float* acts;
  const float* c_out;
  const uint8_t* live;
  float* dgates;
  int32_t reverse;
  int32_t reserved;
} eamd_lstm_seq_bwd_t;
int64_t eamd_lstm_seq_sync_bytes(void);
int eamd_lstm_seq_fwd(const eamd_lstm_seq_fwd_t* jobs, int njobs, int T, int B, int H, void* sync_ws, void* stream);
int eamd_lstm_seq_bwd(const eamd_lstm_seq_bwd_t* jobs, int njobs, int T, int B, int H, void* sync_ws, void* stream);
int eamd_lstm_seq_status(const void* sync_ws, void* stream);
int eamd_lstm_seq_status_merge(const void* sync_ws, void* sticky, void* stream);
int eamd_gru_cell_fwd(const float* gx, const float* gh, const float* h_prev, const uint8_t* live, float* h, float* y,
                      float* acts, int B, int H, void* stream);
int eamd_gru_cell_bwd(const float* dy, const float* dh, const float* acts, const float* h_prev, const uint8_t* live,
                      float* dgx, float* dgh, float* dh_direct, int B, int H, void* stream);
int eamd_maxpool2x2_fwd(const float* x, float* y, uint8_t* idx, int B, int H, int W, int C, void* stream);
int eamd_maxpool2x2_bwd(const float* dy, const uint8_t* idx, float* dx, int B, int H, int W, int C, void* stream);
int eamd_mask_rows(const float* x, const uint8_t* keep, float* y, int64_t rows, int D, void* stream);
int eamd_unfold1d(const void* x, void* col, int B, int T, int C, int k, int bf16, void* stream);
int eamd_fold1d(const float* dcol, float* dx, int B, int T, int C, int k, void* stream);
int eamd_conv3x3_c1_fwd(const float* x, const float* w, const float* bias, void* y, int B, int T, int F, int C,
                        int y_bf16, void* stream);
int64_t eamd_conv3x3_c1_bwd_w_workspace(int B, int T, int C);
int eamd_conv3x3_c1_bwd_w(const void* dy, const float* x, float* dw, float* db, float* workspace, int B, int T, int F,
                          int C, int dy_bf16, void* stream);
int eamd_conv3x3_c1_bwd_x(const void* dy, const float* w, float* dx, int B, int T, int F, int C, int dy_bf16, void* stream);
int eamd_attloc_fwd(const float* att_prev, const float* conv_w, const float* w_att, const float* pre_enc,
                    const float* dec_proj, const float* gvec, const float* gb, const int32_t* lens, const float* enc_h,
                    float scaling, float* e, float* th, float* conv, float* w, float* ctx, int B, int T, int A, int C,
                    int K, int R, int E, void* stream);
int eamd_attloc_bwd_energy(const float* dctx, const float* dw_ext, const float* w, const float* enc_h, const float* th,
                           const float* gvec, float scaling, float* de, float* d_enc_h, float* df, float* dgvec,
                           float* dgb, float* d_dec_proj, int B, int T, int A, int E, void* stream);
int64_t eamd_attloc_bwd_workspace(int B, int T, int A, int C);
int eamd_attloc_bwd_energy_conv(const float* dctx, const float* dw_ext, const float* w, const float* enc_h, const float* th,
                                const float* gvec, float scaling, const float* conv, const float* w_att, float* de,
                                float* d_enc_h, float* df, float* dconv, float* dgvec, float* dgb, float* d_dec_proj,
                                float* dw_att, float* workspace, int accumulate, int B, int T, int A, int C, int E,
                                void* stream);
int eamd_att_dot_energy_fwd(const float* k, const float* q, const int32_t* lens, float* e, int B, int T, int A,
                            void* stream);
int eamd_att_dot_energy_bwd(const float* de, const float* k, const float* q, float* dk, float* dq, int B, int T, int A,
                            void* stream);
int eamd_att_ctx_fwd(const float* e, const float* v, float scaling, float* w, float* ctx, int B, int T, int E,
                     void* stream);
int eamd_att_ctx_bwd(const float* dctx, const float* dw_ext, const float* w, const float* v, float scaling, float* de,
                     float* d_v, float* dsum, int B, int T, int E, void* stream);
int eamd_attloc_bwd_conv(const float* dconv, const float* conv_w, const float* att_prev, float* d_prev, float* dconv_w,
                         int B, int T, int C, int K, int R, void* stream);
int eamd_attloc_convmax_fwd(const float* att_prev, const float* conv_w, float* pooled, int32_t* idx, int B, int T, int C,
                            int K, void* stream);
int eamd_attloc_convmax_bwd(const float* dpool, const float* pooled, const int32_t* idx, const float* att_prev,
                            const float* conv_w, float* d_prev, float* dconv_w, int B, int T, int C, int K, void* stream);

int eamd_joint_fwd(const float* enc, const float* dec, float* out, void* out_bf16, int B, int T, int U, int J, int act,
                   void* stream);
int eamd_joint_bwd(const float* dh, const float* enc, const float* dec, float* d_enc, float* d_dec, int B, int T, int U,
                   int J, int act, void* stream);
int64_t eamd_rnnt_workspace(int B, int T, int U);
int eamd_rnnt_loss(const float* logits, const int32_t* labels, const int32_t* tlens, const int32_t* ulens,
                   float* workspace, float* loss, float* grad, int B, int T, int U, int V, int blank,
                   const float* gscale_dev, float scale, void* stream);
int eamd_rnnt_grad(const float* logits, const int32_t* labels, const int32_t* tlens, const int32_t* ulens,
                   const float* workspace, float* grad, int B, int T, int U, int V, int blank, const float* gscale_dev,
                   float scale, void* stream);
int eamd_rnnt_node_stats(const float* logits_rows, const int32_t* labels, float* workspace, int64_t node0, int64_t nrows,
                         int B, int T, int U, int V, int blank, void* stream);
int eamd_rnnt_alpha_beta(float* workspace, const int32_t* tlens, const int32_t* ulens, float* loss, int B, int T, int U,
                         void* stream);
int eamd_rnnt_node_stats_part(const float* part, const float* zlab, const float* zblank, float* workspace, int64_t node0,
                              int64_t nrows, int tiles_n, int B, int T, int U, void* stream);
int eamd_rnnt_row_coef(const int32_t* labels, const int32_t* tlens, const int32_t* ulens, const float* workspace, float* rowc,
                       int32_t* col, int64_t node0, int64_t nrows, int B, int T, int U, void* stream);
int eamd_rnnt_node_grad(const float* logits_rows, float* grad_rows, void* grad_rows_bf16, const int32_t* labels,
                        const int32_t* tlens, const int32_t* ulens, const float* workspace, int64_t node0, int64_t nrows,
                        int B, int T, int U, int V, int blank, const float* gscale_dev, float scale, void* stream);
int eamd_rnnt_greedy_part_floats(int B, int V);
int eamd_rnnt_greedy_joint(const float* enc_proj, const float* d, const float* w_out, const float* b_out, float* part, int B, int T,
                           int J, int V, int act, int t, const int32_t* t_dev, void* stream);
// ... 78 lines not shown
```

Baseline: 1.123 million frames/s.

## Fuse conv1 weight-gradient into conv2 dgrad GEMM and defer CTC gradient to backward

```diff
diff --git a/espnet_amd/csrc/convmod.hip b/espnet_amd/csrc/convmod.hip
--- a/espnet_amd/csrc/convmod.hip
+++ b/espnet_amd/csrc/convmod.hip
@@ -867,6 +867,14 @@
   EAMD_LAUNCH_CHECK();
   return EAMD_OK;
 }
+}
+int eamd_conv1_bwd_w_reduce(const float* part, int nslab, int C, float* dw, float* db, hipStream_t stream) {
+  hipLaunchKernelGGL(conv1_bwd_w_reduce_kernel, dim3((10 * C + 63) / 64, min(16, (nslab + 31) / 32)), dim3(256), 0, stream, part,
+                     nslab, C, dw, db);
+  EAMD_LAUNCH_CHECK();
+  return EAMD_OK;
+}
+extern "C" {
 static int64_t conv_c1_ws(int B, int T, int C, int st, int pad) {
   if (B <= 0 || T + 2 * pad < 3 || C <= 0) return 0;
   int H = (T + 2 * pad - 3) / st + 1;
diff --git a/espnet_amd/csrc/ctc.hip b/espnet_amd/csrc/ctc.hip
--- a/espnet_amd/csrc/ctc.hip
+++ b/espnet_amd/csrc/ctc.hip
@@ -209,7 +209,8 @@
                                                        const float* __restrict__ beta, const float* __restrict__ nll,
                                                        float* __restrict__ grad, long gst, long gsb, int T, int V,
                                                        int Smax, int blank, float scale, long si = 0, long gsi = 0,
-                                                       int nsp = 1, const long long* __restrict__ perm = nullptr) {
+                                                       int nsp = 1, const long long* __restrict__ perm = nullptr,
+                                                       const float* __restrict__ gscale = nullptr) {
   extern __shared__ float occ[];
   const int t = blockIdx.x, b = blockIdx.y;
   const int i = kPit ? (int)blockIdx.z : 0;
@@ -236,7 +237,28 @@
   __syncthreads();
   const float* xr = x + t * st + b * sb + (kPit ? i * si : 0);
   const float ls = lse[q * T + t];
+  if (gscale) {
+    const float gs = gscale[0];
+    for (int v = threadIdx.x; v < V; v += blockDim.x) gr[v] = ((expf(xr[v] - ls) - occ[v]) * scale) * gs;
+    return;
+  }
   for (int v = threadIdx.x; v < V; v += blockDim.x) gr[v] = (expf(xr[v] - ls) - occ[v]) * scale;
+}
+
+struct CtcWs { int* lab; int* lablen; float* lse; float* lp; float* alpha; float* beta; int Lm; };
+inline CtcWs ctc_ws_carve(void* workspace, int B, int T, int Lmax) {
+  CtcWs r;
+  const int Smax = 2 * Lmax + 1;
+  char* w = (char*)workspace;
+  r.Lm = Lmax > 0 ? Lmax : 1;
+  r.lab = (int*)w; w += (size_t)B * r.Lm * 4;
+  r.lablen = (int*)w; w += (size_t)B * 4;
+  w = (char*)(((uintptr_t)w + 15) & ~(uintptr_t)15);
+  r.lse = (float*)w; w += (size_t)B * T * 4;
+  r.lp = (float*)w; w += (size_t)B * T * Smax * 4;
+  r.alpha = (float*)w; w += (size_t)B * T * Smax * 4;
+  r.beta = (float*)w;
+  return r;
 }
 
 }
@@ -261,15 +283,10 @@
   if (threads > 1024) return EAMD_EUNSUPPORTED;
   if (grad && (size_t)V * 4 > 64 * 1024) return EAMD_EUNSUPPORTED;
   hipStream_t s = (hipStream_t)stream;
-  char* w = (char*)workspace;
-  int Lm = Lmax > 0 ? Lmax : 1;
-  int* lab = (int*)w; w += (size_t)B * Lm * 4;
-  int* lablen = (int*)w; w += (size_t)B * 4;
-  w = (char*)(((uintptr_t)w + 15) & ~(uintptr_t)15);
-  float* lse = (float*)w; w += (size_t)B * T * 4;
-  float* lp = (float*)w; w += (size_t)B * T * Smax * 4;
-  float* alpha = (float*)w; w += (size_t)B * T * Smax * 4;
-  float* beta = (float*)w;
+  const CtcWs ws = ctc_ws_carve(workspace, B, T, Lmax);
+  int* lab = ws.lab; int* lablen = ws.lablen;
+  float* lse = ws.lse; float* lp = ws.lp; float* alpha = ws.alpha; float* beta = ws.beta;
+  const int Lm = ws.Lm;
 
   hipLaunchKernelGGL(ctc_prep_kernel, dim3(B), dim3(64), 0, s, (const long long*)ys_pad, Lmax, ignore_id, lab, lablen, B);
   EAMD_LAUNCH_CHECK();
@@ -285,6 +302,23 @@
                        (long)gstride_b, T, V, Smax, blank, grad_scale, 0L, 0L, 1, nullptr);
     EAMD_LAUNCH_CHECK();
   }
+  return EAMD_OK;
+}
+
+
+int eamd_ctc_grad(const float* acts, int64_t stride_t, int64_t stride_b, const int32_t* ilens, const float* nll, float* grad,
+                  int64_t gstride_t, int64_t gstride_b, const void* workspace, int B, int T, int V, int Lmax, int blank,
+                  float grad_scale, const float* gscale_dev, void* stream) {
+  if (!acts || !ilens || !nll || !grad || !workspace || B <= 0 || T <= 0 || V <= 0 || Lmax < 0) return EAMD_EINVAL;
+  const int Smax = 2 * Lmax + 1;
+  if (((Smax + 63) / 64) * 64 > 1024) return EAMD_EUNSUPPORTED;
+  if ((size_t)V * 4 > 64 * 1024) return EAMD_EUNSUPPORTED;
+  const CtcWs ws = ctc_ws_carve((void*)workspace, B, T, Lmax);
+  hipLaunchKernelGGL(ctc_grad_kernel<false>, dim3(T, B), dim3(256), (size_t)V * sizeof(float), (hipStream_t)stream, acts,
+                     (long)stride_t, (long)stride_b, ilens, ws.lab, ws.lablen, ws.Lm, ws.lse, ws.lp, ws.alpha, ws.beta, nll, grad,
+                     (long)gstride_t, (long)gstride_b, T, V, Smax, blank, grad_scale, 0L, 0L, 1, (const long long*)nullptr,
+                     gscale_dev);
+  EAMD_LAUNCH_CHECK();
   return EAMD_OK;
 }
 
diff --git a/espnet_amd/csrc/gemm.hip b/espnet_amd/csrc/gemm.hip
--- a/espnet_amd/csrc/gemm.hip
+++ b/espnet_amd/csrc/gemm.hip
@@ -352,10 +352,11 @@
 int eamd_gemm_bf16_dispatch(const eamd_gemm_t& p, int tile, hipStream_t stream);
 int eamd_gemm_f32_dispatch(const eamd_gemm_t& p, int tile, hipStream_t stream);
 
-static int gemm_check(eamd_gemm_t& p, int& tile_out) {
+static int gemm_check(eamd_gemm_t& p, int& tile_out, const bool no_c = false) {
   const bool stats = p.epilogue == 7;
+  const bool no_result = stats || no_c;
   const bool rowgrad = p.epilogue == 8;
-  if (!p.A || !p.B || (!p.C && !p.Cb && !stats)) return EAMD_EINVAL;
+  if (!p.A || !p.B || (!p.C && !p.Cb && !no_result)) return EAMD_EINVAL;
   if (stats && (!p.stats.part || !p.stats.zfix || (p.stats.col && !p.stats.zcol))) return EAMD_EINVAL;
   if (rowgrad && !p.stats.rowc) return EAMD_EINVAL;
   if ((stats || rowgrad) && (p.stats.fix < 0 || p.stats.fix >= p.N || (p.tile != 64 && p.tile != 128) || p.splitk > 1 ||
@@ -364,7 +365,7 @@
     return EAMD_EINVAL;
   if (p.in_dtype != 0 && p.in_dtype != 1) return EAMD_EINVAL;
   if (p.in_dtype == 1 && p.precision != 1) return EAMD_EINVAL;
-  if (p.in_dtype == 0 && (p.Cb || p.aux_dtype || (!p.C && !stats))) return EAMD_EUNSUPPORTED;
+  if (p.in_dtype == 0 && (p.Cb || p.aux_dtype || (!p.C && !no_result))) return EAMD_EUNSUPPORTED;
   if (p.M <= 0 || p.N <= 0 || p.K < 0) return EAMD_EINVAL;
   if (p.batch1 <= 0 || p.batch2 <= 0) return EAMD_EINVAL;
   if (p.splitk < 1) p.splitk = 1;
@@ -398,6 +399,9 @@
       if (g.C % tile != 0) return EAMD_EINVAL;
     }
   }
+  if (p.colsum && p.gather.enabled &&
+      (!p.transA || !p.transB || p.in_dtype != 0 || p.batch1 * p.batch2 != 1 || p.a_act != EAMD_ACT_NONE || p.b_act != EAMD_ACT_NONE))
+    return EAMD_EUNSUPPORTED;
   if ((p.N + tile - 1) / tile > 65535) return EAMD_EUNSUPPORTED;
   if (p.h_dtype != 0 && p.h_dtype != 1) return EAMD_EINVAL;
   if (p.in_dtype == 1 && p.h_dtype != 0) return EAMD_EUNSUPPORTED;
@@ -428,6 +432,7 @@
     if (p.drop_p != 0.f || p.Hb || p.a_act > EAMD_ACT_SWISH || p.b_act > EAMD_ACT_SWISH) return EAMD_EUNSUPPORTED;
   }
   if (stats || rowgrad) return EAMD_EUNSUPPORTED;
+  if (p.colsum && p.gather.enabled) return EAMD_EUNSUPPORTED;
   if (tile == 128) {
     return p.precision ? launch<128, 128, 1>(p, stream) : launch<128, 128, 0>(p, stream);
   }
@@ -458,6 +463,26 @@
     if (rc != EAMD_OK) return rc;
   }
   return EAMD_OK;
+}
+
+int eamd_gemm_f32_conv1w(const eamd_gemm_t* ps, const int* tiles, int n, const float* x, int T, int F, float* part, int* nslab,
+                         hipStream_t stream);
+int eamd_conv1_bwd_w_reduce(const float* part, int nslab, int C, float* dw, float* db, hipStream_t stream);
+
+extern "C" int eamd_conv2_bwd_x_conv1_bwd_w(const eamd_gemm_t* descs, int n, const float* x, int T, int F, float* part,
+                                            float* dw, float* db, void* stream) {
+  if (!descs || n < 1 || n > EAMD_GEMM_MULTI_MAX || !x || !part || !dw || !db || T < 3 || F < 3) return EAMD_EINVAL;
+  eamd_gemm_t ps[EAMD_GEMM_MULTI_MAX];
+  int tiles[EAMD_GEMM_MULTI_MAX];
+  for (int i = 0; i < n; ++i) {
+    ps[i] = descs[i];
+    const int chk = gemm_check(ps[i], tiles[i], true);
+    if (chk != EAMD_OK) return chk;
+  }
+  int nslab = 0;
+  const int rc = eamd_gemm_f32_conv1w(ps, tiles, n, x, T, F, part, &nslab, (hipStream_t)stream);
+  if (rc != EAMD_OK) return rc;
+  return eamd_conv1_bwd_w_reduce(part, nslab, ps[0].N, dw, db, (hipStream_t)stream);
 }
 
 int eamd_gemm_f32_group_count(const eamd_gemm_t& p);
diff --git a/espnet_amd/csrc/gemm_f32.hip b/espnet_amd/csrc/gemm_f32.hip
--- a/espnet_amd/csrc/gemm_f32.hip
+++ b/espnet_amd/csrc/gemm_f32.hip
@@ -34,8 +34,104 @@
   return make_float4(nv > 0 ? v.x : 0.f, nv > 1 ? v.y : 0.f, nv > 2 ? v.z : 0.f, nv > 3 ? v.w : 0.f);
 }
 
-template <int BM, int BN, bool TA, bool TB, bool GAT, int ACT, bool ROWEPI = false, bool NOPAD = false>
-__device__ __forceinline__ void gemm_f32_body(const eamd_gemm_t& p, const int bid, const int nblk, const int zb) {
+struct Conv1W {
+  const float* x;
+  float* part;
+  int T, F;
+  int slab0[EAMD_GEMM_MULTI_MAX];
+};
+
+__device__ __forceinline__ void conv1w_tile(const eamd_gemm_t& p, f32x4 (&acc)[4][4], float* cl, float* patch, int m0, int n0,
+                                            const Conv1W& cw, int slab) {
+  constexpr int BM = 128, BN = 128, WM = 64, WN = 64, MT = 4, NTL = 4, LDC = BN + 4;
+  const int t = threadIdx.x;
+  const int lane = t & 63, wave = t >> 6;
+  const int wm = wave >> 1, wn = wave & 1;
+  const int fr = lane & 15, fq = lane >> 4;
+  int* rowp = reinterpret_cast<int*>(patch + BM * 9);
+  float xv[9];
+  int prow = -1;
+#pragma unroll
+  for (int k = 0; k < 9; ++k) xv[k] = 0.f;
+  if (t < BM && m0 + t < p.M) {
+    const int m = m0 + t;
+    const eamd_rowmap_t& c = p.cmap;
+    const int jj = m % c.Wo, tt = m / c.Wo, ii = tt % c.Ho, bb = tt / c.Ho;
+    const int hi = ii * c.sh + c.oh, wi = jj * c.sw + c.ow;
+    prow = (bb * c.Hc + hi) * c.Wc + wi;
+    const float* xp = cw.x + ((long)bb * cw.T + 2 * hi) * cw.F + 2 * wi;
+#pragma unroll
+    for (int kh = 0; kh < 3; ++kh)
+#pragma unroll
+      for (int kw = 0; kw < 3; ++kw) xv[kh * 3 + kw] = xp[kh * cw.F + kw];
+  }
+#pragma unroll
+  for (int i = 0; i < MT; ++i)
+#pragma unroll
+    for (int j = 0; j < NTL; ++j)
+#pragma unroll
+      for (int r = 0; r < 4; ++r)
+        cl[(wm * WM + i * 16 + fq * 4 + r) * LDC + wn * WN + j * 16 + fr] = acc[i][j][r];
+  if (t < BM) {
+#pragma unroll
+    for (int k = 0; k < 9; ++k) patch[t * 9 + k] = xv[k];
+    rowp[t] = prow;
+  }
+  __syncthreads();
+
+  const int c4 = t & 31, r0 = t >> 5;
+  const int n = n0 + c4 * 4;
+  float db[4] = {0.f, 0.f, 0.f, 0.f}, dw[4][9];
+#pragma unroll
+  for (int e = 0; e < 4; ++e)
+#pragma unroll
+    for (int k = 0; k < 9; ++k) dw[e][k] = 0.f;
+#pragma unroll 1
+  for (int g0 = 0; g0 < BM / 8; g0 += 4) {
+    float4 a32[4];
+    int pr[4];
+#pragma unroll
+    for (int q = 0; q < 4; ++q) {
+      pr[q] = rowp[r0 + (g0 + q) * 8];
+      a32[q] = *reinterpret_cast<const float4*>(p.aux + (long)max(pr[q], 0) * p.ldaux + n);
+    }
+#pragma unroll
+    for (int q = 0; q < 4; ++q) {
+      const int rr = r0 + (g0 + q) * 8;
+      const float4 a4 = *reinterpret_cast<const float4*>(&cl[rr * LDC + c4 * 4]);
+      const bool ok = pr[q] >= 0;
+      const float g[4] = {ok && a32[q].x > 0.f ? a4.x : 0.f, ok && a32[q].y > 0.f ? a4.y : 0.f,
+                          ok && a32[q].z > 0.f ? a4.z : 0.f, ok && a32[q].w > 0.f ? a4.w : 0.f};
+      float xr[9];
+#pragma unroll
+      for (int k = 0; k < 9; ++k) xr[k] = patch[rr * 9 + k];
+#pragma unroll
+      for (int e = 0; e < 4; ++e) {
+        db[e] += g[e];
+#pragma unroll
+        for (int k = 0; k < 9; ++k) dw[e][k] += g[e] * xr[k];
+      }
+    }
+  }
+  __syncthreads();
+  float* red = cl;
+#pragma unroll
+  for (int k = 0; k < 9; ++k)
+    *reinterpret_cast<float4*>(&red[(r0 * 10 + k) * BN + c4 * 4]) = make_float4(dw[0][k], dw[1][k], dw[2][k], dw[3][k]);
+  *reinterpret_cast<float4*>(&red[(r0 * 10 + 9) * BN + c4 * 4]) = make_float4(db[0], db[1], db[2], db[3]);
+  __syncthreads();
+  float* out = cw.part + (long)slab * 10 * p.N + n0;
+  for (int idx = t; idx < 10 * BN; idx += NT_) {
+    float v = 0.f;
+#pragma unroll
+    for (int g = 0; g < NT_ / 32; ++g) v += red[g * 10 * BN + idx];
+    out[(long)(idx / BN) * p.N + (idx % BN)] = v;
+  }
+}
+
+template <int BM, int BN, bool TA, bool TB, bool GAT, int ACT, bool ROWEPI = false, bool NOPAD = false, bool C1W = false>
+__device__ __forceinline__ void gemm_f32_body(const eamd_gemm_t& p, const int bid, const int nblk, const int zb,
+                                              const Conv1W* cw = nullptr, const int slab0 = 0) {
   constexpr int WM = BM / 2, WN = BN / 2;
   constexpr int MT = WM / 16, NTL = WN / 16;
   constexpr int NCA = BM / 32, NCB = BN / 32;
@@ -142,6 +238,7 @@
   constexpr int UNROLL = DEPTH % 2 ? 2 * DEPTH : DEPTH;
   float4 ra[DEPTH][NCA], rb[DEPTH][NCB];
   const bool do_colsum = TA && p.colsum != nullptr && !GAT && tile_n == 0;
+  const bool do_bsum = TA && TB && GAT && p.colsum != nullptr && tile_m == 0;
   float cs[4] = {0.f, 0.f, 0.f, 0.f};
 
   const int gWo = GAT ? p.gather.Wo : 1, gHo = GAT ? p.gather.Ho : 1, gsh = GAT ? p.gather.sh : 0, gsw = GAT ? p.gather.sw : 0;
@@ -270,6 +367,14 @@
       for (int i = 0; i < NCA; ++i) *reinterpret_cast<float4*>(&la[a_r[i] * S::LDA + a_c[i] * 4]) = ra[SET][i];
 #pragma unroll
       for (int i = 0; i < NCB; ++i) *reinterpret_cast<float4*>(&lb[b_r[i] * S::LDB + b_c[i] * 4]) = rb[SET][i];
+      if constexpr (TA && TB && GAT) {
+        if (do_bsum) {
+#pragma unroll
+          for (int i = 0; i < NCB; ++i) {
+            cs[0] += rb[SET][i].x; cs[1] += rb[SET][i].y; cs[2] += rb[SET][i].z; cs[3] += rb[SET][i].w;
+          }
+        }
+      }
     }
   };
 
@@ -435,7 +540,34 @@
     }
     __syncthreads();
   }
-
+  if constexpr (TA && TB && GAT) {
+    if (p.colsum != nullptr) {
+      float* csl = sm.ab;
+      constexpr int NSLOT = NT_ / CPR_B;
+      static_assert(NSLOT * BN <= S::OPS, "column-sum slots must fit in the operand buffers");
+      if (do_bsum) {
+#pragma unroll
+        for (int j = 0; j < 4; ++j) csl[(t / CPR_B) * BN + b_c[0] * 4 + j] = cs[j];
+      }
+      __syncthreads();
+      if (do_bsum) {
+        for (int i = t; i < BN; i += NT_) {
+          const int n = n0 + i;
+          float v = 0.f;
+#pragma unroll 8
+          for (int sl = 0; sl < NSLOT; ++sl) v += csl[sl * BN + i];
+          if (n < p.N) atomicAdd(p.colsum + n, v * p.alpha);
+        }
+      }
+      __syncthreads();
+    }
+  }
+
+  if constexpr (C1W) {
+    static_assert(BM == 128 && BN == 128 && !TA && !ROWEPI, "the conv1 weight-gradient epilogue is written for the 128 tile");
+    conv1w_tile(p, acc, sm.ab, reinterpret_cast<float*>(smem_raw + sizeof(S)), m0, n0, *cw, slab0 + tile_m);
+    return;
+  }
   if (p.splitk > 1) {
     const bool lead = split == 0;
 #pragma unroll
@@ -500,6 +632,18 @@
   const eamd_gemm_t p = m.p[cls];
   gemm_f32_body<BM, BN, TA, TB, GAT, false, false, NOPAD>(p, bid, m.nt[cls], 0);
 }
+
+template <bool NOPAD>
+__global__ __launch_bounds__(NT_, 2) void gemm_f32_multi_c1w_kernel(const MultiF m, const Conv1W cw) {
+  const int g = (int)blockIdx.x >> 3;
+  const int per = (int)gridDim.x / (8 * m.n);
+  const int cls = g / per;
+  const int bid = (g - cls * per) * 8 + ((int)blockIdx.x & 7);
+  if (bid >= m.nt[cls]) return;
+  const eamd_gemm_t p = m.p[cls];
+  gemm_f32_body<128, 128, false, true, true, 0, false, NOPAD, true>(p, bid, m.nt[cls], 0, &cw, cw.slab0[cls]);
+}
+constexpr size_t C1W_SMEM = sizeof(SmemF<128, 128, false, true>) + (128 * 9 + 128) * sizeof(float);
 
 template <int BM, int BN, bool TA, bool TB, bool GAT, int ACT, bool NOPAD = false>
 int launch_f2(const eamd_gemm_t& p, hipStream_t stream) {
@@ -625,6 +769,59 @@
   return nopad ? multi_launch_t<true>(m, grid, stream) : multi_launch_t<false>(m, grid, stream);
 }
 
+template <bool NOPAD>
+static int c1w_launch_t(const MultiF& m, const Conv1W& cw, int grid, hipStream_t stream) {
+  static const hipError_t attr_err = hipFuncSetAttribute(reinterpret_cast<const void*>(&gemm_f32_multi_c1w_kernel<NOPAD>),
+                                                         hipFuncAttributeMaxDynamicSharedMemorySize, (int)C1W_SMEM);
+  if (attr_err != hipSuccess) return (int)attr_err;
+  hipLaunchKernelGGL(gemm_f32_multi_c1w_kernel<NOPAD>, dim3((unsigned)grid), dim3(NT_), C1W_SMEM, stream, m, cw);
+  EAMD_LAUNCH_CHECK();
+  return EAMD_OK;
+}
+
+int eamd_gemm_f32_conv1w(const eamd_gemm_t* ps, const int* tiles, int n, const float* x, int T, int F, float* part, int* nslab,
+                         hipStream_t stream) {
+  if (n < 1 || n > EAMD_GEMM_MULTI_MAX) return EAMD_EUNSUPPORTED;
+  MultiF m;
+  Conv1W cw;
+  cw.x = x; cw.part = part; cw.T = T; cw.F = F;
+  const int H1 = (T - 3) / 2 + 1, W1 = (F - 3) / 2 + 1;
+  int maxnt = 0;
+  bool nopad = true;
+  long slabs = 0, nimg = -1;
+  for (int i = 0; i < n; ++i) {
+    const eamd_gemm_t& p = ps[i];
+    if (tiles[i] != 128 || p.in_dtype != 0 || p.precision != 0) return EAMD_EUNSUPPORTED;
+    if (!p.gather.enabled || p.transA || !p.transB || p.splitk != 1 || p.batch1 * p.batch2 != 1) return EAMD_EUNSUPPORTED;
+    if (p.Cb || p.Hb || p.aux_dtype || p.epilogue != 3 || !p.aux || p.colsum || p.bias || p.R) return EAMD_EUNSUPPORTED;
+    if (p.a_act != EAMD_ACT_NONE || p.b_act != EAMD_ACT_NONE || p.drop_p != 0.f || p.alpha != 1.f || p.beta != 0.f)
+      return EAMD_EUNSUPPORTED;
+    const bool b_ok = aligned16f(p.B) && p.ldb % 4 == 0 && p.ldb >= (p.N + 3) / 4 * 4;
+    if (p.gather.C % FBK != 0 || !aligned16f(p.A) || !b_ok || !gather_taps_small(p.gather)) return EAMD_EUNSUPPORTED;
+    nopad = nopad && gather_nopad(p.gather);
+    if (p.N % 128 != 0 || p.N != ps[0].N || !aligned16f(p.aux) || p.ldaux % 4 != 0 || p.ldaux < p.N) return EAMD_EUNSUPPORTED;
+    const eamd_rowmap_t& c = p.cmap;
+    if (!c.enabled || c.Hc != H1 || c.Wc != W1 || c.Ho < 1 || c.Wo < 1 || c.sh < 1 || c.sw < 1 || c.oh < 0 || c.ow < 0 ||
+        (long)(c.Ho - 1) * c.sh + c.oh >= H1 || (long)(c.Wo - 1) * c.sw + c.ow >= W1 || p.M % (c.Ho * c.Wo) != 0)
+      return EAMD_EUNSUPPORTED;
+    const long b = p.M / (c.Ho * c.Wo);
+    if ((nimg >= 0 && b != nimg) || b * H1 * W1 >= (1L << 31)) return EAMD_EUNSUPPORTED;
+    nimg = b;
+    const long rt = (p.M + 127) / 128, nt = rt * (p.N / 128);
+    if (nt > (1L << 24)) return EAMD_EUNSUPPORTED;
+    m.p[i] = p;
+    m.nt[i] = (int)nt;
+    cw.slab0[i] = (int)slabs;
+    slabs += rt;
+    maxnt = nt > maxnt ? (int)nt : maxnt;
+  }
+  for (int i = n; i < EAMD_GEMM_MULTI_MAX; ++i) { m.p[i] = ps[0]; m.nt[i] = 0; cw.slab0[i] = 0; }
+  m.n = n;
+  *nslab = (int)slabs;
+  const int grid = (maxnt + 7) / 8 * 8 * n;
+  return nopad ? c1w_launch_t<true>(m, cw, grid, stream) : c1w_launch_t<false>(m, cw, grid, stream);
+}
+
 int eamd_gemm_f32_group_count(const eamd_gemm_t& p) {
   if (p.in_dtype != 0 || p.precision != 0 || !p.transA || !p.transB || !p.C || p.Cb || p.Hb || p.aux || p.R || p.bias)
     return EAMD_EUNSUPPORTED;
diff --git a/espnet_amd/functional.py b/espnet_amd/functional.py
--- a/espnet_amd/functional.py
+++ b/espnet_amd/functional.py
@@ -976,10 +976,15 @@
     return y, wd, Ho, Wo
 
 
-def _conv3s2_bwd(dy, y_in, wd, dw_buf, db_buf, B, Hi, Wi, Ho, Wo, Cc, adt):
+FUSE_CONV1_WGRAD = True
+
+
+def _conv3s2_bwd_w(dy, y_in, dw_buf, db_buf, B, Hi, Wi, Ho, Wo, Cc):
     dev = dy.device
     M = B * Ho * Wo
-    ops.colsum(dy, db_buf)
+    bsum = not ops.fast() and dy.dtype == torch.float32 and y_in.dtype == torch.float32
+    if not bsum:
+        ops.colsum(dy, db_buf)
     dwf = torch.zeros(9 * Cc, Cc, device=dev, dtype=torch.float32)
     g = ops.make_gather(Cc, _TAPS_FWD, Ho, Wo, Hi, Wi, 2, 2)
     f32_big = (not ops.fast()) and Cc % 128 == 0
@@ -987,9 +992,12 @@
     ntile = (9 * Cc // tile) * ((Cc + tile - 1) // tile)
     want = 1024 if ops.fast() else 1008 if f32_big else 2304
     sk = max(2, min(64, (want + ntile - 1) // ntile, max(1, M // 256)))
-    ops.gemm(y_in, dy, dwf, 9 * Cc, Cc, M, 9 * Cc, Cc, Cc, transA=1, transB=1, gather=g, splitk=sk, tile=tile)
+    ops.gemm(y_in, dy, dwf, 9 * Cc, Cc, M, 9 * Cc, Cc, Cc, transA=1, transB=1, gather=g, splitk=sk, tile=tile,
+             colsum=db_buf if bsum else None)
     ops.conv2_weight_grad(dwf, dw_buf, Cc, Cc)
-    dy_in = torch.empty(y_in.shape, device=dev, dtype=adt)
+
+
+def _conv3s2_dx_classes(dy, y_in, wd, dy_in, B, Hi, Wi, Ho, Wo, Cc, tile=0):
     q0, classes = 0, []
     for (ph, pw), taps in _CLASSES:
         Hc, Wc = (Hi - ph + 1) // 2, (Wi - pw + 1) // 2
@@ -998,10 +1006,25 @@
             cm = ops.make_rowmap(Hc, Wc, Hi, Wi, 2, ph, 2, pw)
             nt = len(taps)
             ops.gemm(dy, wd, dy_in, B * Hc * Wc, Cc, nt * Cc, nt * Cc, Cc, Cc, transB=1, b_off=q0 * Cc * Cc,
-                     gather=gt, cmap=cm, epilogue=EPI_MUL_RELU_MASK, aux=y_in, ldaux=Cc, defer=classes)
+                     gather=gt, cmap=cm, epilogue=EPI_MUL_RELU_MASK, aux=y_in, ldaux=Cc, defer=classes, tile=tile)
         q0 += len(taps)
-    ops.gemm_multi(classes)
+    return classes
+
+
+def _conv3s2_bwd(dy, y_in, wd, dw_buf, db_buf, B, Hi, Wi, Ho, Wo, Cc, adt):
+    _conv3s2_bwd_w(dy, y_in, dw_buf, db_buf, B, Hi, Wi, Ho, Wo, Cc)
+    dy_in = torch.empty(y_in.shape, device=dy.device, dtype=adt)
+    ops.gemm_multi(_conv3s2_dx_classes(dy, y_in, wd, dy_in, B, Hi, Wi, Ho, Wo, Cc))
     return dy_in
+
+
+def _conv1w_fusable(y_in, Cc):
+    return FUSE_CONV1_WGRAD and not ops.fast() and y_in.dtype == torch.float32 and Cc % 128 == 0
+
+
+def _conv3s2_bwd_conv1w(dy, y_in, wd, dw_buf, db_buf, B, Hi, Wi, Ho, Wo, Cc, x, dw1_buf, db1_buf):
+    _conv3s2_bwd_w(dy, y_in, dw_buf, db_buf, B, Hi, Wi, Ho, Wo, Cc)
+    ops.conv2_bwd_x_conv1_bwd_w(_conv3s2_dx_classes(dy, y_in, wd, None, B, Hi, Wi, Ho, Wo, Cc, tile=128), x, dw1_buf, db1_buf)
 
 
 def _taps(k):
@@ -1119,6 +1142,10 @@
         dy = dy.view(B * Hl * Wl, Cc)
         for i in range(n - 1, -1, -1):
             (Hi, Wi), (Ho, Wo) = dims[i], dims[i + 1]
+            if i == 0 and ctx.ks[i] == 3 and _conv1w_fusable(ys[0], Cc):
+                _conv3s2_bwd_conv1w(dy, ys[0].view(-1, Cc), wds[0], sink.buf(4), sink.buf(5), B, Hi, Wi, Ho, Wo, Cc, x,
+                                    sink.buf(0), sink.buf(1))
+                return (None, None) + sink.results()
             if ctx.ks[i] == 3:
                 dy = _conv3s2_bwd(dy, ys[i].view(-1, Cc), wds[i], sink.buf(4 + 2 * i), sink.buf(5 + 2 * i), B, Hi, Wi, Ho,
                                   Wo, Cc, adt)
@@ -1190,16 +1217,20 @@
     @staticmethod
     def forward(ctx, acts, ys_pad, hlens, blank, ignore_id, time_major=False):
         B = acts.shape[1] if time_major else acts.shape[0]
-        nll, grad = ops.ctc_loss(acts.contiguous(), ys_pad, hlens, blank, ignore_id, 1.0 / B,
-                                 want_grad=acts.requires_grad, time_major=time_major)
-        ctx.save_for_backward(grad)
+        acts = acts.contiguous()
+        nll, _, ws = ops.ctc_loss(acts, ys_pad, hlens, blank, ignore_id, 1.0 / B, want_grad=False, time_major=time_major,
+                                  keep_workspace=True)
+        ctx.save_for_backward(acts, nll, hlens, ws)
         ctx.nll = nll
+        ctx.cfg = (ys_pad.shape[1], blank, 1.0 / B, time_major)
         return ops.reduce_sum(nll, 1.0 / B)
 
     @staticmethod
     def backward(ctx, g):
-        (grad,) = ctx.saved_tensors
-        return ops.scale_dev(grad, g.contiguous(), 1.0, out=grad), None, None, None, None, None
+        acts, nll, hlens, ws = ctx.saved_tensors
+        L, blank, scale, time_major = ctx.cfg
+        grad = ops.ctc_grad(acts, hlens, nll, ws, L, blank, scale, gscale=g.contiguous().view(1), time_major=time_major)
+        return grad, None, None, None, None, None
 
 
 class CTCRowsLossFn(torch.autograd.Function):
diff --git a/espnet_amd/ops.py b/espnet_amd/ops.py
--- a/espnet_amd/ops.py
+++ b/espnet_amd/ops.py
@@ -146,8 +146,11 @@
     p.aux_dtype = 1 if (aux is not None and aux.dtype == torch.bfloat16) else 0
     p.R = ptr(R, c_off) if R is not None else None
     if colsum is not None:
-        if not transA or gather is not None or colsum.numel() < M * b1 * b2:
-            raise _lib.EamdError("gemm: colsum needs transA, no gather and M outputs")
+        if gather is not None:
+            if not (transA and transB) or bf or (b1, b2) != (1, 1) or colsum.numel() < N:
+                raise _lib.EamdError("gemm: colsum with a gather needs transA, transB, float32 operands and N outputs")
+        elif not transA or colsum.numel() < M * b1 * b2:
+            raise _lib.EamdError("gemm: colsum needs transA and M outputs")
         p.colsum = ptr(colsum)
     p.M, p.N, p.K = M, N, K
     p.transA, p.transB = int(transA), int(transB)
@@ -226,6 +229,26 @@
         check(L.eamd_gemm_multi(arr, n, stream_ptr()), "eamd_gemm_multi")
 
 
+def conv2_bwd_x_conv1_bwd_w(items, x, dw, db):
+    L = _lib.lib()
+    n = len(items)
+    Bn, T, F = x.shape
+    H1, W1 = (T - 3) // 2 + 1, (F - 3) // 2 + 1
+    Cc = items[0][0].N
+    assert 1 <= n <= GEMM_MULTI_MAX and x.is_contiguous() and x.dtype == torch.float32
+    assert dw.dtype == torch.float32 and db.dtype == torch.float32 and dw.numel() >= 9 * Cc and db.numel() >= Cc
+    for p_, keep in items:
+        assert p_.M == Bn * p_.cmap.Ho * p_.cmap.Wo and keep[4] is not None and keep[4].numel() >= Bn * H1 * W1 * p_.ldaux
+    arr = (GemmT * n)(*[it[0] for it in items])
+    part = torch.empty(sum((it[0].M + 127) // 128 for it in items) * 10 * Cc, device=x.device, dtype=torch.float32)
+    args = (arr, n, ptr(x), T, F, ptr(part), ptr(dw), ptr(db))
+    if _gemm_record is not None:
+        _gemm_record.append((dict(kind="multi%d_c1w" % n, flop=sum(2.0 * it[0].M * it[0].N * it[0].K for it in items)),
+                             (arr, [it[1] for it in items], x, part, dw, db),
+                             lambda sp, args=args: check(L.eamd_conv2_bwd_x_conv1_bwd_w(*args, sp), "eamd_conv2_bwd_x_conv1_bwd_w")))
+    check(L.eamd_conv2_bwd_x_conv1_bwd_w(*args, stream_ptr()), "eamd_conv2_bwd_x_conv1_bwd_w")
+
+
 GROUP_WGRAD = True
 STACK_WGRAD_MAX_ROWS = 64
 GROUP_WGRAD_MAX_TILES = 384
@@ -1898,7 +1921,8 @@
     return gw
 
 
-def ctc_loss(acts_btv, ys_pad, ilens, blank=0, ignore_id=-1, grad_scale=1.0, want_grad=True, time_major=False):
+def ctc_loss(acts_btv, ys_pad, ilens, blank=0, ignore_id=-1, grad_scale=1.0, want_grad=True, time_major=False,
+             keep_workspace=False):
     if time_major:
         T, B, V = acts_btv.shape
         st, sb = B * V, V
@@ -1915,7 +1939,26 @@
     check(_lib.lib().eamd_ctc_loss(ptr(acts_btv), st, sb, ptr(ys_pad), ptr(ilens), ptr(nll),
                                    ptr(grad), st, sb, ptr(ws), B, T, V, L, blank, ignore_id,
                                    grad_scale, stream_ptr()), "eamd_ctc_loss")
+    if keep_workspace:
+        return nll, grad, ws
     return nll, grad
+
+
+def ctc_grad(acts_btv, ilens, nll, ws, L, blank=0, grad_scale=1.0, gscale=None, time_major=False):
+    if time_major:
+        T, B, V = acts_btv.shape
+        st, sb = B * V, V
+    else:
+        B, T, V = acts_btv.shape
+        st, sb = V, T * V
+    L_ = _lib.lib()
+    assert acts_btv.is_contiguous() and acts_btv.dtype == torch.float32 and ilens.dtype == torch.int32 and ilens.numel() == B
+    assert nll.dtype == torch.float32 and nll.numel() == B and ws.numel() >= L_.eamd_ctc_workspace_bytes(B, T, L)
+    assert gscale is None or (gscale.dtype == torch.float32 and gscale.numel() == 1)
+    grad = torch.empty_like(acts_btv)
+    check(L_.eamd_ctc_grad(ptr(acts_btv), st, sb, ptr(ilens), ptr(nll), ptr(grad), st, sb, ptr(ws), B, T, V, L, blank,
+                           grad_scale, ptr(gscale), stream_ptr()), "eamd_ctc_grad")
+    return grad
 
 
 def ctc_pit_loss(acts, ys_pad, ilens, blank=0, ignore_id=-1, grad_scale=1.0, want_grad=True):
diff --git a/include/espnet_amd.h b/include/espnet_amd.h
--- a/include/espnet_amd.h
+++ b/include/espnet_amd.h
@@ -59,6 +59,9 @@
 
 #define EAMD_GEMM_MULTI_MAX 4
 int eamd_gemm_multi(const eamd_gemm_t* descs, int n, void* stream);
+
+int eamd_conv2_bwd_x_conv1_bwd_w(const eamd_gemm_t* descs, int n, const float* x, int T, int F, float* part, float* dw,
+                                 float* db, void* stream);
 
 int eamd_gemm_group_plan(const eamd_gemm_t* descs, int n, int32_t* first);
 int eamd_gemm_group_launch(const eamd_gemm_t* descs_dev, const int32_t* first_dev, int n, int total, int in_dtype, int tile,
@@ -274,6 +277,9 @@
                   const int32_t* ilens, float* nll, float* grad, int64_t gstride_t, int64_t gstride_b,
                   void* workspace, int B, int T, int V, int Lmax, int blank, int ignore_id, float grad_scale,
                   void* stream);
+int eamd_ctc_grad(const float* acts, int64_t stride_t, int64_t stride_b, const int32_t* ilens, const float* nll, float* grad,
+                  int64_t gstride_t, int64_t gstride_b, const void* workspace, int B, int T, int V, int Lmax, int blank,
+                  float grad_scale, const float* gscale_dev, void* stream);
 
 int64_t eamd_ctc_pit_workspace_bytes(int S, int B, int T, int Lmax);
 int eamd_ctc_pit_loss(const float* acts, const int64_t* ys_pad, const int32_t* ilens, float* nll_pair, int64_t* perm, float* pit,
```

Result: faster. 1.138 million frames/s (median of 6 runs) (+1.3%).
